# cloudflare/zkp-ecdsa

Hardware: NVIDIA H100
Metric: ZKAttest proofs/sec (higher is better)
Workload: dtype u256/u258 (32-bit limbs, Montgomery)

## Files before the change

zkp_ecdsa_b200/csrc/zk_curves.cuh:

```cuda
#pragma once
#include "zk_field.cuh"

namespace zk {

#define WEI_PT P256Pt
#define WEI_AFF P256Aff
#define WEI_JAC P256Jac
#define WEI_F P256p
#define WEI_FN(n) p256_##n
#define WEI_B_MONT ZK_P256_B_MONT
#define WEI_GX_MONT ZK_P256_GX_MONT
#define WEI_GY_MONT ZK_P256_GY_MONT
#include "zk_weier.inc"
#undef WEI_PT
#undef WEI_AFF
#undef WEI_JAC
#undef WEI_F
#undef WEI_FN
#undef WEI_B_MONT
#undef WEI_GX_MONT
#undef WEI_GY_MONT

#if defined(ZKA_PG_WAR256)
#define WEI_PT WarPt
#define WEI_AFF WarAff
#define WEI_JAC WarJac
#define WEI_F Warp
#define WEI_FN(n) war_##n
#define WEI_B_MONT ZK_WAR_B_MONT
#define WEI_GX_MONT ZK_WAR_GX_MONT
#define WEI_GY_MONT ZK_WAR_GY_MONT
#include "zk_weier.inc"
#undef WEI_PT
#undef WEI_AFF
#undef WEI_JAC
#undef WEI_F
#undef WEI_FN
#undef WEI_B_MONT
#undef WEI_GX_MONT
#undef WEI_GY_MONT

enum : int { PGL = 8 };
using PGp = Warp;
using FpPG = FpWar;
using TomPt = WarPt;
using TomPre = WarAff;
using TompMsm = Warp;
using TompCommit = Warp;
ZK_HD void tom_set_identity(TomPt& p) { war_set_identity(p); }
ZK_HD void tom_from_affine(TomPt& p, const uint32_t* x, const uint32_t* y) {
  copy_n<8>(p.x, x);
  copy_n<8>(p.y, y);
  Warp::set_one(p.z);
}
ZK_HD void tom_set_generator(TomPt& p) {
  WarAff g;
  war_set_generator(g);
  war_from_affine(p, g);
}
ZK_HD bool tom_on_curve(const uint32_t* x, const uint32_t* y) { return war_on_curve(x, y); }
ZK_HD void tom_add(TomPt& r, const TomPt& p, const TomPt& q) { war_add(r, p, q); }
template <bool kNeedT, class F = Warp>
ZK_HD void tom_madd(TomPt& r, const TomPt& p, const TomPre& q) { war_madd(r, p, q); }
ZK_HD void tom_dbl(TomPt& r, const TomPt& p) { war_dbl(r, p); }
ZK_HD void tom_neg(TomPt& r, const TomPt& p) {
  copy_n<8>(r.x, p.x);
  Warp::neg(r.y, p.y);
  copy_n<8>(r.z, p.z);
}
ZK_HD void pg_dbl_n(TomPt& p, int c) { war_dbl_n(p, c); }
ZK_HD void pg_pre_neg(TomPre& q) { Warp::neg(q.y, q.y); }
ZK_HD bool pg_is_identity(const TomPt& p) { return war_is_identity(p); }
ZK_HD void pg_fixed_to_msm(TomPt&) {}
#else
struct TomPt {
  uint32_t x[9], y[9], t[9], z[9];
};
struct TomPre {
  uint32_t x[9], y[9], k[9];
};

ZK_HD void tom_const(uint32_t* r, int which) {
  constexpr uint32_t sa[9] = ZK_TOM_SQRTA_MONT;
  constexpr uint32_t isa[9] = ZK_TOM_INVSQRTA_MONT;
  constexpr uint32_t d1[9] = ZK_TOM_D1_MONT;
  constexpr uint32_t gx[9] = ZK_TOM_GX1_MONT;
  constexpr uint32_t gy[9] = ZK_TOM_GY_MONT;
  constexpr uint32_t s2[9] = ZK_TOM_SQRTND1_MONT;
  constexpr uint32_t is2[9] = ZK_TOM_INVSQRTND1_MONT;
  constexpr uint32_t dd2[9] = ZK_TOM_2D2_MONT;
  constexpr uint32_t isd[9] = ZK_TOM_INVSQRTND_MONT;
#pragma unroll
  for (int i = 0; i < 9; i++)
    r[i] = which == 0 ? sa[i] : which == 1 ? isa[i] : which == 2 ? d1[i] : which == 3 ? gx[i] : which == 4 ? gy[i]
           : which == 5 ? s2[i] : which == 6 ? is2[i] : which == 7 ? dd2[i] : isd[i];
}
enum { TOM_SQRTA = 0, TOM_INVSQRTA = 1, TOM_D1 = 2, TOM_GX1 = 3, TOM_GY = 4, TOM_SQRTND1 = 5, TOM_INVSQRTND1 = 6,
       TOM_2D2 = 7, TOM_INVSQRTND = 8 };

struct TompInl : Tomp {
  ZK_HD static void mul(uint32_t* r, const uint32_t* a, const uint32_t* b) {
#if defined(__CUDA_ARCH__) && !defined(ZKA_NO_PTX_MUL)
    ptx::tom_mul_body(r, a, b);
#else
    Tomp::mul(r, a, b);
#endif
  }
  ZK_HD static void sqr(uint32_t* r, const uint32_t* a) { mul(r, a, a); }
};
#if defined(ZKA_COMMIT_INLINE)
using TompCommit = TompInl;
#else
using TompCommit = Tomp;
#endif
#if defined(ZKA_MSM_INLINE)
using TompMsm = TompInl;
#else
using TompMsm = Tomp;
#endif

template <bool kNeedT, class F = Tomp>
ZK_HD void tom2_madd(TomPt& r, const TomPt& p, const TomPre& q) {
  uint32_t A[9], B[9], C[9], D[9], E[9], Fv[9], G[9], H[9];
  F::sub(A, p.y, p.x);
  F::mul(A, A, q.x);
  F::add(B, p.y, p.x);
  F::mul(B, B, q.y);
  F::mul(C, p.t, q.k);
  F::add(D, p.z, p.z);
  F::sub(E, B, A);
  F::sub(Fv, D, C);
  F::add(G, D, C);
  F::add(H, B, A);
  F::mul(r.x, E, Fv);
  F::mul(r.y, G, H);
  if (kNeedT) F::mul(r.t, E, H);
  F::mul(r.z, Fv, G);
}

ZK_HD void tom_set_identity(TomPt& p) {
  zero_n<9>(p.x);
  Tomp::set_one(p.y);
  zero_n<9>(p.t);
  Tomp::set_one(p.z);
}
ZK_HD void tom_from_affine(TomPt& p, const uint32_t* x1, const uint32_t* y) {
  copy_n<9>(p.x, x1);
  copy_n<9>(p.y, y);
  Tomp::mul(p.t, x1, y);
  Tomp::set_one(p.z);
}
ZK_HD void tom_set_generator(TomPt& p) {
  uint32_t gx[9], gy[9];
  tom_const(gx, TOM_GX1);
  tom_const(gy, TOM_GY);
  tom_from_affine(p, gx, gy);
}
ZK_HD bool tom_on_curve(const uint32_t* x1, const uint32_t* y) {
  using F = Tomp;
  uint32_t xx[9], yy[9], l[9], r[9], d1[9], one[9];
  F::sqr(xx, x1);
  F::sqr(yy, y);
  F::add(l, xx, yy);
  F::mul(r, xx, yy);
  tom_const(d1, TOM_D1);
  F::mul(r, r, d1);
  F::set_one(one);
  F::add(r, r, one);
  uint32_t d[9], o[9];
  F::sub(d, l, r);
  zero_n<9>(o);
  o[0] = 1;
  F::mul(d, d, o);
  uint32_t nz = 0, np = 0;
#pragma unroll
  for (int i = 0; i < 9; i++) { nz |= d[i]; np |= d[i] ^ FpTom::p(i); }
  return nz == 0 || np == 0;
}

ZK_HD void tom_add(TomPt& r, const TomPt& p, const TomPt& q) {
  using F = Tomp;
  uint32_t A[9], B[9], C[9], D[9], E[9], Fv[9], G[9], H[9], d1[9];
  tom_const(d1, TOM_D1);
  F::mul(A, p.x, q.x);
  F::mul(B, p.y, q.y);
  F::mul(C, p.t, q.t);
  F::mul(C, C, d1);
  F::mul(D, p.z, q.z);
  F::add(E, p.x, p.y);
  F::add(H, q.x, q.y);
  F::mul(E, E, H);
  F::sub(E, E, A);
  F::sub(E, E, B);
  F::sub(Fv, D, C);
  F::add(G, D, C);
  F::sub(H, B, A);
  F::mul(r.x, E, Fv);
  F::mul(r.y, G, H);
  F::mul(r.t, E, H);
  F::mul(r.z, Fv, G);
}
template <bool kNeedT, class F = Tomp>
ZK_HD void tom_madd(TomPt& r, const TomPt& p, const TomPre& q) {
  uint32_t A[9], B[9], C[9], E[9], Fv[9], G[9], H[9];
  F::mul(A, p.x, q.x);
  F::mul(B, p.y, q.y);
  F::mul(C, p.t, q.k);
  F::add(E, p.x, p.y);
  F::add(H, q.x, q.y);
  F::mul(E, E, H);
  F::sub(E, E, A);
  F::sub(E, E, B);
  F::sub(Fv, p.z, C);
  F::add(G, p.z, C);
  F::sub(H, B, A);
  F::mul(r.x, E, Fv);
  F::mul(r.y, G, H);
  if (kNeedT) F::mul(r.t, E, H);
  F::mul(r.z, Fv, G);
}
ZK_HD void tom_dbl(TomPt& r, const TomPt& p) {
  using F = Tomp;
  uint32_t A[9], B[9], C[9], E[9], G[9], Fv[9], H[9];
  F::sqr(A, p.x);
  F::sqr(B, p.y);
  F::sqr(C, p.z);
  F::add(C, C, C);
  F::add(E, p.x, p.y);
  F::sqr(E, E);
  F::sub(E, E, A);
  F::sub(E, E, B);
  F::add(G, A, B);
  F::sub(Fv, G, C);
  F::sub(H, A, B);
  F::mul(r.x, E, Fv);
  F::mul(r.y, G, H);
  F::mul(r.t, E, H);
  F::mul(r.z, Fv, G);
}
ZK_HD void tom_neg(TomPt& r, const TomPt& p) {
  Tomp::neg(r.x, p.x);
  copy_n<9>(r.y, p.y);
  Tomp::neg(r.t, p.t);
  copy_n<9>(r.z, p.z);
}


enum : int { PGL = 9 };
using PGp = Tomp;
using FpPG = FpTom;
ZK_HD void pg_dbl_n(TomPt& p, int c) {
  for (int i = 0; i < c; i++) tom_dbl(p, p);
}
ZK_HD void pg_pre_neg(TomPre& q) {
  Tomp::neg(q.x, q.x);
  Tomp::neg(q.k, q.k);
}
ZK_HD bool pg_is_identity(const TomPt& p) { return Tomp::is_zero(p.x) && Tomp::eq(p.y, p.z); }
ZK_HD void pg_fixed_to_msm(TomPt& f) {
  uint32_t cw[9], X[9], Y[9], Tt[9], Zp[9], c1[9];
  tom_const(c1, TOM_INVSQRTND1);
  Tomp::mul(cw, f.x, c1);
  Tomp::mul(X, cw, f.y);
  Tomp::sqr(Y, f.z);
  Tomp::mul(Tt, cw, f.z);
  Tomp::mul(Zp, f.z, f.y);
  copy_n<9>(f.x, X); copy_n<9>(f.y, Y); copy_n<9>(f.t, Tt); copy_n<9>(f.z, Zp);
}
#endif

}
```

zkp_ecdsa_b200/csrc/zk_ops.cuh:

```cuda
#pragma once
#include "zk_curves.cuh"
#include "zk_layout.h"
#include "zk_sha256.cuh"

namespace zk {

#if defined(__CUDA_ARCH__)
#define ZK_SET_STATUS(ptr, code) atomicCAS((int*)(ptr), 0, (int)(code))
#define ZK_SET_STATUS_OVER(ptr, code, over) \
  do {                                      \
    atomicCAS((int*)(ptr), 0, (int)(code)); \
    atomicCAS((int*)(ptr), (int)(over), (int)(code)); \
  } while (0)
#else
#define ZK_SET_STATUS_OVER(ptr, code, over)              \
  do {                                                   \
    if (*(ptr) == 0 || *(ptr) == (over)) *(ptr) = (code); \
  } while (0)
#define ZK_SET_STATUS(ptr, code) \
  do {                           \
    if (*(ptr) == 0) *(ptr) = (code); \
  } while (0)
#endif

template <int N>
ZK_HD void ld(uint32_t* r, const uint32_t* p) {
#pragma unroll
  for (int i = 0; i < N; i++) r[i] = p[i];
}
template <int N>
ZK_HD void st(uint32_t* p, const uint32_t* r) {
#pragma unroll
  for (int i = 0; i < N; i++) p[i] = r[i];
}

enum : int {
  P256_PROJ_WORDS = 24,
  P256_AFF_WORDS = 16,
#if defined(ZKA_PG_WAR256)
  TOM_PROJ_WORDS = 24,
  TOM_AFF_WORDS = 16,
  TOM_PRE_WORDS = 16,
#else
  TOM_PROJ_WORDS = 28,
  TOM_AFF_WORDS = 18,
  TOM_PRE_WORDS = 32,
#endif
  NORM_CHUNK_MAX = 64,
};


#if defined(ZKA_PG_WAR256)
ZK_HD void tom_st_xyz(uint32_t* m, const uint32_t* x, const uint32_t* y, const uint32_t* z) {
  st<8>(m, x); st<8>(m + 8, y); st<8>(m + 16, z);
}
ZK_HD void tom_ld_xyz(uint32_t* x, uint32_t* y, uint32_t* z, const uint32_t* m) {
  ld<8>(x, m); ld<8>(y, m + 8); ld<8>(z, m + 16);
}
ZK_HD void tom_ld_pre(TomPre& q, const uint32_t* m) { ld<8>(q.x, m); ld<8>(q.y, m + 8); }
#else
ZK_HD void tom_st_xyz(uint32_t* m, const uint32_t* x, const uint32_t* y, const uint32_t* z) {
  uint32_t w[28];
#pragma unroll
  for (int i = 0; i < 9; i++) { w[i] = x[i]; w[9 + i] = y[i]; w[18 + i] = z[i]; }
  w[27] = 0;
#if defined(__CUDA_ARCH__)
  uint4* v = reinterpret_cast<uint4*>(m);
#pragma unroll
  for (int i = 0; i < 7; i++) v[i] = make_uint4(w[4 * i], w[4 * i + 1], w[4 * i + 2], w[4 * i + 3]);
#else
  for (int i = 0; i < 28; i++) m[i] = w[i];
#endif
}
ZK_HD void tom_ld_xyz(uint32_t* x, uint32_t* y, uint32_t* z, const uint32_t* m) {
  uint32_t w[28];
#if defined(__CUDA_ARCH__)
  const uint4* v = reinterpret_cast<const uint4*>(m);
#pragma unroll
  for (int i = 0; i < 7; i++) {
    const uint4 u = v[i];
    w[4 * i] = u.x; w[4 * i + 1] = u.y; w[4 * i + 2] = u.z; w[4 * i + 3] = u.w;
  }
#else
  for (int i = 0; i < 28; i++) w[i] = m[i];
#endif
#pragma unroll
  for (int i = 0; i < 9; i++) { x[i] = w[i]; y[i] = w[9 + i]; z[i] = w[18 + i]; }
}

ZK_HD void tom2_pre_neg(TomPre& q, bool neg) {
  uint32_t nk[9];
  Tomp::neg(nk, q.k);
#pragma unroll
  for (int i = 0; i < 9; i++) {
    const uint32_t a = q.x[i], b = q.y[i];
    q.x[i] = neg ? b : a;
    q.y[i] = neg ? a : b;
    q.k[i] = neg ? nk[i] : q.k[i];
  }
}
ZK_HD void tom_ld_pre(TomPre& q, const uint32_t* m) {
#if defined(__CUDA_ARCH__)
  const uint4* v = reinterpret_cast<const uint4*>(m);
  uint32_t w[32];
#pragma unroll
  for (int i = 0; i < 7; i++) {
    uint4 u = __ldg(v + i);
    w[4 * i] = u.x; w[4 * i + 1] = u.y; w[4 * i + 2] = u.z; w[4 * i + 3] = u.w;
  }
#pragma unroll
  for (int i = 0; i < 9; i++) { q.x[i] = w[i]; q.y[i] = w[9 + i]; q.k[i] = w[18 + i]; }
#else
  ld<9>(q.x, m); ld<9>(q.y, m + 9); ld<9>(q.k, m + 18);
#endif
}

#endif

ZK_HD void ld4(uint32_t* w, const void* p) {
#if defined(__CUDA_ARCH__)
  const uint4 u = *reinterpret_cast<const uint4*>(p);
  w[0] = u.x; w[1] = u.y; w[2] = u.z; w[3] = u.w;
#else
  const uint32_t* q = reinterpret_cast<const uint32_t*>(p);
  for (int i = 0; i < 4; i++) w[i] = q[i];
#endif
}
ZK_HD void st4(void* p, const uint32_t* w) {
#if defined(__CUDA_ARCH__)
  *reinterpret_cast<uint4*>(p) = make_uint4(w[0], w[1], w[2], w[3]);
#else
  uint32_t* q = reinterpret_cast<uint32_t*>(p);
  for (int i = 0; i < 4; i++) q[i] = w[i];
#endif
}
ZK_HD void ld8v(uint32_t* r, const uint32_t* p) { ld4(r, p); ld4(r + 4, p + 4); }
ZK_HD void st8v(uint32_t* p, const uint32_t* r) { st4(p, r); st4(p + 4, r + 4); }
ZK_HD bool aligned16(const void* p) { return ((size_t)p & 15) == 0; }

template <int N, int CB>
ZK_HD uint32_t enc_byte(int i, uint32_t tag, const uint32_t* x, const uint32_t* y) {
  if (i == 0) return tag;
  if (i >= 1 + 2 * CB) return 0u;
  const uint32_t* c = i <= CB ? x : y;
  const int pos = CB - 1 - (i <= CB ? i - 1 : i - 1 - CB);
  return (pos >> 2) < N ? ((c[pos >> 2] >> (8 * (pos & 3))) & 0xffu) : 0u;
}
template <int N, int CB>
ZK_HD void store_point_words(uint8_t* o, uint32_t tag, const uint32_t* x, const uint32_t* y) {
  uint32_t w[BSTRIDE / 4];
#pragma unroll
  for (int j = 0; j < BSTRIDE / 4; j++)
    w[j] = enc_byte<N, CB>(4 * j, tag, x, y) | (enc_byte<N, CB>(4 * j + 1, tag, x, y) << 8) |
           (enc_byte<N, CB>(4 * j + 2, tag, x, y) << 16) | (enc_byte<N, CB>(4 * j + 3, tag, x, y) << 24);
  if (aligned16(o)) {
#pragma unroll
    for (int j = 0; j < BSTRIDE / 16; j++) st4(o + 16 * j, w + 4 * j);
  } else {
    uint32_t* ow = reinterpret_cast<uint32_t*>(o);
#pragma unroll
    for (int j = 0; j < BSTRIDE / 4; j++) ow[j] = w[j];
  }
}

ZK_HD uint32_t digit4(const uint32_t* k, int j) { return (k[j >> 3] >> (4 * (j & 7))) & 15u; }
ZK_HD uint32_t digit8(const uint32_t* k, int j) { return (k[j >> 2] >> (8 * (j & 3))) & 255u; }
ZK_HD uint32_t digit_w(const uint32_t* k, int pos, int w) {
  int wi = pos >> 5, sh = pos & 31;
  uint64_t v = k[wi];
  if (wi + 1 < 8) v |= (uint64_t)k[wi + 1] << 32;
  return (uint32_t)(v >> sh) & ((1u << w) - 1u);
}

ZK_HD int fb_entries(int w) { return (1 << (w - 1)) + 1; }
ZK_HD int fb_windows(int w) { return (256 + w) / w; }
ZK_HD uint32_t signed_digit(const uint32_t* k, int j, int w, uint32_t& carry, bool& neg) {
  const int pos = j * w;
  uint32_t d = carry;
  if (pos < 256) d += digit_w(k, pos, (256 - pos) < w ? (256 - pos) : w);
  const uint32_t half = 1u << (w - 1);
  neg = d > half;
  carry = neg ? 1u : 0u;
  return neg ? (1u << w) - d : d;
}

ZK_HD uint32_t bswap32(uint32_t x) {
#if defined(__CUDA_ARCH__)
  return __byte_perm(x, 0u, 0x0123);
#else
  return (x >> 24) | ((x >> 8) & 0xff00u) | ((x << 8) & 0xff0000u) | (x << 24);
#endif
}
ZK_HD void tape_draw(uint32_t* r, const uint8_t* tape, int draw) {
  const uint8_t* p = tape + 32 * (size_t)draw;
#if defined(__CUDA_ARCH__)
  if (aligned16(p)) {
    const uint4 a = __ldg(reinterpret_cast<const uint4*>(p)), b = __ldg(reinterpret_cast<const uint4*>(p) + 1);
    r[7] = bswap32(a.x); r[6] = bswap32(a.y); r[5] = bswap32(a.z); r[4] = bswap32(a.w);
    r[3] = bswap32(b.x); r[2] = bswap32(b.y); r[1] = bswap32(b.z); r[0] = bswap32(b.w);
    return;
  }
#endif
#pragma unroll
  for (int i = 0; i < 8; i++) {
    const uint8_t* q = p + 28 - 4 * i;
    r[i] = ((uint32_t)q[0] << 24) | ((uint32_t)q[1] << 16) | ((uint32_t)q[2] << 8) | (uint32_t)q[3];
  }
}

#define WEI_PT P256Pt
#define WEI_AFF P256Aff
#define WEI_JAC P256Jac
#define WEI_F P256p
#define WEI_FN(n) p256_##n
#define WEI_T(n) P256##n
#include "zk_weier_ops.inc"
#undef WEI_PT
#undef WEI_AFF
#undef WEI_JAC
#undef WEI_F
#undef WEI_FN
#undef WEI_T

enum : int { KEY_W_MIN = 5, KEY_W_MAX = 8, KEY_CAP = 52 * 17 };
ZK_HD int key_window_bits(uint32_t count, uint32_t B, uint32_t uses) {
  int best = KEY_W_MIN;
  uint64_t best_cost = ~0ull;
  for (int w = KEY_W_MIN; w <= KEY_W_MAX; w++) {
    const uint64_t nwin = (uint64_t)fb_windows(w), ne = (uint64_t)fb_entries(w);
    if (w > KEY_W_MIN && (uint64_t)count * nwin * ne > (uint64_t)B * KEY_CAP) break;
    const uint64_t cost = nwin * ((uint64_t)count * (ne - 1) * 2 + (uint64_t)B * uses);
    if (cost < best_cost) { best_cost = cost; best = w; }
  }
  return best;
}
ZK_HD size_t key_table_words(int w) { return (size_t)fb_windows(w) * fb_entries(w) * P256_AFF_WORDS; }

enum : int { RT_W = 5, RT_NWIN = 52, RT_ROW = 16, RT_ENTRIES = RT_NWIN * RT_ROW };
struct P256RowsSignedTask {
  const uint32_t* pows;
// ... 35 lines not shown
ZK_HD int item_gpart_of_job(int j) {
  if (j < 6) return j;
  if (j < 30) {
    const int m = (j - 6) / 6, u = (j - 6) % 6;
    return 6 + 5 * m + (u < 4 ? u : u - 1);
  }
  return 26 + ((j - 30) >> 1);
}
ZK_HD int item_job_of_gpart(int g) {
  if (g < 6) return g;
  if (g < 26) {
    const int m = (g - 6) / 5, u = (g - 6) % 5;
    return 6 + 6 * m + (u < 4 ? u : 5);
  }
  return 30 + 2 * (g - 26);
}
#if defined(ZKA_PG_WAR256)
#include "zk_ops_war.cuh"
#else
struct TomPowsTask {
  const uint32_t* base_aff;
  uint32_t* pows;
  int nbase, nwin, w;
  ZK_HD void operator()(int t) const {
    uint32_t x[9], y[9];
    ld<9>(x, base_aff + (size_t)t * TOM_AFF_WORDS);
    ld<9>(y, base_aff + (size_t)t * TOM_AFF_WORDS + 9);
    TomPt p;
    tom_from_affine(p, x, y);
    for (int j = 0; j < nwin; j++) {
      uint32_t* o = pows + ((size_t)t * nwin + j) * 36;
      st<9>(o, p.x); st<9>(o + 9, p.y); st<9>(o + 18, p.t); st<9>(o + 27, p.z);
      for (int k = 0; k < w; k++) tom_dbl(p, p);
    }
  }
};
struct TomRowsTask {
  const uint32_t* pows;
  uint32_t* rows;
  int w;
  ZK_HD void operator()(int t) const {
    TomPt p, acc;
    const uint32_t* s = pows + (size_t)t * 36;
    ld<9>(p.x, s); ld<9>(p.y, s + 9); ld<9>(p.t, s + 18); ld<9>(p.z, s + 27);
    tom_set_identity(acc);
    const int ne = fb_entries(w);
    uint32_t* out = rows + (size_t)t * ne * TOM_PROJ_WORDS;
    for (int d = 0; d < ne; d++) {
      uint32_t* o = out + (size_t)d * TOM_PROJ_WORDS;
      tom_st_xyz(o, acc.x, acc.y, acc.z);
      tom_add(acc, acc, p);
    }
  }
};
struct TomRowsHiTask {
  const uint32_t* pows;
  uint32_t* hi;
  uint32_t* rows;
  int w;
  ZK_HD void operator()(int t) const {
    TomPt p, acc;
    const uint32_t* s = pows + (size_t)t * 36;
    ld<9>(p.x, s); ld<9>(p.y, s + 9); ld<9>(p.t, s + 18); ld<9>(p.z, s + 27);
    for (int k = 0; k < 8; k++) tom_dbl(p, p);
    tom_set_identity(acc);
    const int nh = 1 << (w - 9);
    for (int m = 0; m < nh; m++) {
      uint32_t* o = hi + ((size_t)t * nh + m) * 36;
      st<9>(o, acc.x); st<9>(o + 9, acc.y); st<9>(o + 18, acc.t); st<9>(o + 27, acc.z);
      tom_add(acc, acc, p);
    }
    tom_st_xyz(rows + ((size_t)t * fb_entries(w) + ((size_t)1 << (w - 1))) * TOM_PROJ_WORDS, acc.x, acc.y, acc.z);
  }
};
struct TomRowsLoTask {
  const uint32_t* pows;
  const uint32_t* hi;
  uint32_t* rows;
  int w;
  ZK_HD void operator()(int t) const {
    const int nh = 1 << (w - 9);
    const int j = t / nh, m = t % nh;
    TomPt p, acc;
    const uint32_t* s = pows + (size_t)j * 36;
    ld<9>(p.x, s); ld<9>(p.y, s + 9); ld<9>(p.t, s + 18); ld<9>(p.z, s + 27);
    const uint32_t* h = hi + (size_t)t * 36;
    ld<9>(acc.x, h); ld<9>(acc.y, h + 9); ld<9>(acc.t, h + 18); ld<9>(acc.z, h + 27);
    uint32_t* out = rows + ((size_t)j * fb_entries(w) + ((size_t)m << 8)) * TOM_PROJ_WORDS;
    for (int d = 0; d < 256; d++) {
      uint32_t* o = out + (size_t)d * TOM_PROJ_WORDS;
      tom_st_xyz(o, acc.x, acc.y, acc.z);
      tom_add(acc, acc, p);
    }
  }
};
struct TomTabE2Task {
  const uint32_t* proj;
  uint32_t* pre;
  int count;
  ZK_HD void operator()(int t) const {
    using F = Tomp;
    constexpr int CH = 16;
    const int lo = t * CH;
    int n = count - lo;
    if (n > CH) n = CH;
    if (n <= 0) return;
    uint32_t pf[CH][9];
    uint32_t acc[9], y[9], z[9], den[9];
    F::set_one(acc);
    for (int k = 0; k < n; k++) {
      const uint32_t* src = proj + (size_t)(lo + k) * TOM_PROJ_WORDS;
      uint32_t xx[9];
      tom_ld_xyz(xx, y, z, src);
      F::mul(den, y, z);
      F::mul(acc, acc, den);
      copy_n<9>(pf[k], acc);
    }
    uint32_t inv[9], s2[9], dd2[9];
    F::inv(inv, acc);
    tom_const(s2, TOM_SQRTND1);
    tom_const(dd2, TOM_2D2);
    for (int k = n - 1; k >= 0; k--) {
      const uint32_t* src = proj + (size_t)(lo + k) * TOM_PROJ_WORDS;
      uint32_t x[9], di[9], w[9], v[9], kk[9], ym[9], yp[9];
      tom_ld_xyz(x, y, z, src);
      F::mul(den, y, z);
      if (k > 0) F::mul(di, inv, pf[k - 1]); else copy_n<9>(di, inv);
      F::mul(inv, inv, den);
      F::mul(w, x, y);
      F::mul(w, w, di);
      F::mul(w, w, s2);
      F::sqr(v, z);
      F::mul(v, v, di);
      F::mul(kk, w, v);
      F::mul(kk, kk, dd2);
      F::sub(ym, v, w);
      F::add(yp, v, w);
      F::reduce(ym); F::reduce(yp); F::reduce(kk);
      uint32_t* o = pre + (size_t)(lo + k) * TOM_PRE_WORDS;
      st<9>(o, ym); st<9>(o + 9, yp); st<9>(o + 18, kk);
      for (int i = 27; i < 32; i++) o[i] = 0;
    }
  }
};

struct TomNormTask {
  const uint32_t* proj;
  uint32_t* aff;
  uint8_t* bytes;
  int count;
  int chunk;
  int e2;
  int aff_mod, aff_lim;
  ZK_HD static void canon2p(uint32_t* r) {
    uint32_t t[9], p2[9];
#pragma unroll
    for (int i = 0; i < 9; i++) p2[i] = (FpTom::p(i) << 1) | (i > 0 ? (FpTom::p(i - 1) >> 31) : 0u);
    uint32_t br = sub_n<9>(t, r, p2);
    csel_n<9>(r, br == 0, t, r);
    br = sub_p<FpTom>(t, r);
    csel_n<9>(r, br == 0, t, r);
  }
  ZK_HD void operator()(int t) const {
    using F = Tomp;
    const int lo = t * chunk;
    int n = count - lo;
    if (n > chunk) n = chunk;
    if (n <= 0) return;
    uint32_t pre[NORM_CHUNK_MAX][9];
    uint32_t acc[9], z[9], v[9], den[9];
    F::set_one(acc);
    for (int k = 0; k < n; k++) {
      const uint32_t* src = proj + (size_t)(lo + k) * TOM_PROJ_WORDS;
      uint32_t xx[9];
      tom_ld_xyz(xx, v, z, src);
      if (e2) F::mul(den, z, v); else copy_n<9>(den, z);
      F::mul(acc, acc, den);
      copy_n<9>(pre[k], acc);
    }
    uint32_t inv[9], isa[9], is2[9], isd[9], one_plain[9];
    F::inv(inv, acc);
    tom_const(isa, TOM_INVSQRTA);
    tom_const(is2, TOM_INVSQRTND1);
    tom_const(isd, TOM_INVSQRTND);
    zero_n<9>(one_plain);
    one_plain[0] = 1;
    for (int k = n - 1; k >= 0; k--) {
      const uint32_t* src = proj + (size_t)(lo + k) * TOM_PROJ_WORDS;
      uint32_t X[9], Y[9], di[9];
      tom_ld_xyz(X, Y, z, src);
      if (e2) F::mul(den, z, Y); else copy_n<9>(den, z);
      if (k > 0) F::mul(di, inv, pre[k - 1]); else copy_n<9>(di, inv);
      F::mul(inv, inv, den);
      if (bytes) {
        uint32_t Dp[9], cx[9], cy[9];
        F::mul(Dp, di, one_plain);
        if (e2) {
          F::mul(cx, X, Y);
          F::mul(cx, cx, isd);
          F::mul(cx, cx, Dp);
          F::sqr(cy, z);
          F::mul(cy, cy, Dp);
        } else {
          F::mul(cx, X, isa);
          F::mul(cx, cx, Dp);
          F::mul(cy, Y, Dp);
        }
        canon2p(cx);
        canon2p(cy);
        store_point_words<9, 33>(bytes + (size_t)(lo + k) * BSTRIDE, 0x04u, cx, cy);
      }
      if (aff && ((lo + k) % aff_mod) < aff_lim) {
        uint32_t x[9], y[9];
        if (e2) {
          uint32_t zi[9], vi[9];
          F::mul(zi, di, Y);
          F::mul(vi, di, z);
          F::mul(x, X, zi);
          F::mul(x, x, is2);
          F::mul(y, z, vi);
        } else {
          F::mul(x, X, di);
          F::mul(y, Y, di);
        }
        uint32_t* a = aff + (size_t)(lo + k) * TOM_AFF_WORDS;
        st<9>(a, x);
        st<9>(a + 9, y);
      }
    }
  }
};

struct TomCommitTask {
  const uint32_t* jv;
  const uint32_t* jr;
  const uint32_t* gtab;
  const uint32_t* htab;
  uint32_t* proj;
  int w, nwin;
  ZK_HD void operator()(int t) const {
    uint32_t v[8], r[8];
    ld<8>(v, jv + (size_t)t * 8);
    ld<8>(r, jr + (size_t)t * 8);
    TomPt acc;
    tom_set_identity(acc);
    const size_t ne = (size_t)fb_entries(w);
    uint32_t cv = 0, cr = 0;
    for (int j = 0; j < nwin; j++) {
      TomPre q;
      bool nv, nr;
      const uint32_t dv = signed_digit(v, j, w, cv, nv), dr = signed_digit(r, j, w, cr, nr);
      tom_ld_pre(q, gtab + ((size_t)j * ne + dv) * TOM_PRE_WORDS);
      tom2_pre_neg(q, nv);
      tom2_madd<true>(acc, acc, q);
      tom_ld_pre(q, htab + ((size_t)j * ne + dr) * TOM_PRE_WORDS);
      tom2_pre_neg(q, nr);
      tom2_madd<true>(acc, acc, q);
    }
    uint32_t* o = proj + (size_t)t * TOM_PROJ_WORDS;
    tom_st_xyz(o, acc.x, acc.y, acc.z);
  }
};

struct TomCommitGTask {
  const uint32_t* jv;
  const uint32_t* gtab;
  uint32_t* ext;
  int w, nwin;
  ZK_HD void operator()(int t) const {
    const int item = t / GJOBS_PER_ITEM, g = t % GJOBS_PER_ITEM;
    uint32_t v[8];
    ld<8>(v, jv + ((size_t)item * JOBS_PER_ITEM + item_job_of_gpart(g)) * 8);
    TomPt acc;
    tom_set_identity(acc);
    const size_t ne = (size_t)fb_entries(w);
    uint32_t carry = 0;
#pragma unroll 1
    for (int j = 0; j < nwin; j++) {
      TomPre q;
      bool neg;
      const uint32_t d = signed_digit(v, j, w, carry, neg);
      tom_ld_pre(q, gtab + ((size_t)j * ne + d) * TOM_PRE_WORDS);
      tom2_pre_neg(q, neg);
      tom2_madd<true, TompCommit>(acc, acc, q);
    }
    uint32_t* o = ext + (size_t)t * TOM_EXT_WORDS;
    st<9>(o, acc.x); st<9>(o + 9, acc.y); st<9>(o + 18, acc.t); st<9>(o + 27, acc.z);
  }
};
struct TomCommitHTask {
  const uint32_t* jr;
  const uint32_t* htab;
  const uint32_t* ext;
  uint32_t* proj;
  int w, nwin;
  ZK_HD void operator()(int t) const {
    const int item = t / JOBS_PER_ITEM, jb = t % JOBS_PER_ITEM;
    uint32_t r[8];
    ld<8>(r, jr + (size_t)t * 8);
    TomPt acc;
    const uint32_t* s = ext + ((size_t)item * GJOBS_PER_ITEM + item_gpart_of_job(jb)) * TOM_EXT_WORDS;
    ld<9>(acc.x, s); ld<9>(acc.y, s + 9); ld<9>(acc.t, s + 18); ld<9>(acc.z, s + 27);
    const size_t ne = (size_t)fb_entries(w);
    uint32_t carry = 0;
#pragma unroll 1
    for (int j = 0; j < nwin; j++) {
      TomPre q;
      bool neg;
      const uint32_t d = signed_digit(r, j, w, carry, neg);
      tom_ld_pre(q, htab + ((size_t)j * ne + d) * TOM_PRE_WORDS);
      tom2_pre_neg(q, neg);
      tom2_madd<true, TompCommit>(acc, acc, q);
    }
    tom_st_xyz(proj + (size_t)t * TOM_PROJ_WORDS, acc.x, acc.y, acc.z);
  }
};

#if !defined(ZKA_HOSTSIM) && defined(ZKA_COMMIT_MINBLOCKS)
template <> struct TaskMinBlocks<TomCommitHTask> { static constexpr int value = ZKA_COMMIT_MINBLOCKS; };
template <> struct TaskMinBlocks<TomCommitGTask> { static constexpr int value = ZKA_COMMIT_MINBLOCKS; };
template <> struct TaskMinBlocks<TomCommitTask> { static constexpr int value = ZKA_COMMIT_MINBLOCKS; };
#endif

#endif

enum : int { GK_BLOCK_BITS = 10 };
ZK_HD int gk_block_bits(int n) { return n < GK_BLOCK_BITS ? n : GK_BLOCK_BITS; }
ZK_HD void gk_block_sum(uint32_t* acc, const uint32_t* ring_m, const uint32_t (*fz)[8], const uint32_t (*fo)[8], int n,
                        int k, uint32_t blk, const uint32_t* vw) {
  using F = Tomq;
  uint32_t P[21][8];
  F::set_one(P[n]);
  for (int j = n - 1; j >= k; j--) F::mul(P[j], P[j + 1], ((blk >> (j - k)) & 1u) ? fo[j] : fz[j]);
  for (int j = k - 1; j >= 0; j--) F::mul(P[j], P[j + 1], fz[j]);
  zero_n<8>(acc);
  const size_t base = (size_t)blk << k;
  const uint32_t cnt = 1u << k;
  for (uint32_t l = 0;;) {
    uint32_t vi[8], term[8];
    ld<8>(vi, ring_m + (base + l) * 8);
    if (vw) F::sub(vi, vw, vi);
    F::mul(term, vi, P[0]);
    F::add(acc, acc, term);
    l++;
    if (l == cnt) break;
    int tz = 0;
    while (!((l >> tz) & 1u)) tz++;
    F::mul(P[tz], P[tz + 1], fo[tz]);
    for (int j = tz - 1; j >= 0; j--) F::mul(P[j], P[j + 1], fz[j]);
  }
}

ZK_HD bool hash_pt_fetch(uint32_t* t, const uint8_t* p, int len) {
  if (((size_t)p & 3) || len < 64 || len > 68) return false;
  if (aligned16(p)) {
#pragma unroll
    for (int j = 0; j < 4; j++) ld4(t + 4 * j, p + 16 * j);
    t[16] = len > 64 ? *reinterpret_cast<const uint32_t*>(p + 64) : 0u;
    return true;
  }
  const uint32_t* q = reinterpret_cast<const uint32_t*>(p);
#pragma unroll
  for (int j = 0; j < 17; j++) t[j] = (4 * j < len) ? q[j] : 0u;
  return true;
}
template <class Src>
ZK_HD void hash_points80(uint32_t* c3, const Src& src, int npts) {
  Sha256 h;
  h.init();
  uint32_t nx[17], cu[17];
  int nlen = 0;
  const uint8_t* np = npts > 0 ? src(0, nlen) : nullptr;
  bool nfast = npts > 0 && hash_pt_fetch(nx, np, nlen);
  for (int i = 0; i < npts; i++) {
    const uint8_t* p = np;
    const int len = nlen;
    const bool fast = nfast;
#pragma unroll
    for (int j = 0; j < 17; j++) cu[j] = nx[j];
    if (i + 1 < npts) {
      np = src(i + 1, nlen);
      nfast = hash_pt_fetch(nx, np, nlen);
    }
    if (fast) h.feed17(cu, len);
    else h.update(p, len);
  }
  h.final80(c3);
}

ZK_HD void challenge_to_limbs(uint32_t* r, const uint32_t* c3) {
  zero_n<8>(r);
  r[0] = c3[0]; r[1] = c3[1]; r[2] = c3[2];
}

template <int N>
ZK_HD void load_point(uint32_t* w, const uint8_t* src) {
  if (aligned16(src)) {
#pragma unroll
    for (int j = 0; j < BSTRIDE / 16; j++) ld4(w + 4 * j, src + 16 * j);
  } else if (((size_t)src & 3) == 0) {
    const uint32_t* sw = reinterpret_cast<const uint32_t*>(src);
#pragma unroll
    for (int j = 0; j < BSTRIDE / 4; j++) w[j] = 4 * j < N ? sw[j] : 0u;
  } else {
#pragma unroll
    for (int j = 0; j < BSTRIDE / 4; j++) {
      uint32_t v = 0;
#pragma unroll
      for (int t = 0; t < 4; t++)
        if (4 * j + t < N) v |= (uint32_t)src[4 * j + t] << (8 * t);
      w[j] = v;
    }
  }
}

struct ByteWriter {
  uint8_t* blk;
  uint32_t q[4];
  int fill;
  int lead;
  ZK_HD explicit ByteWriter(uint8_t* dst) : blk(dst - ((size_t)dst & 15)), fill((int)((size_t)dst & 15)), lead(fill) {
    q[0] = q[1] = q[2] = q[3] = 0;
  }
  ZK_HD static uint32_t funnel(uint32_t lo, uint32_t hi, int sh) {
#if defined(__CUDA_ARCH__)
    return __funnelshift_l(lo, hi, sh);
#else
    return (uint32_t)((((uint64_t)hi << 32) | lo) >> (32 - sh));
#endif
  }
  ZK_HD void store_part(int lo, int hi) const {
#pragma unroll
    for (int w = 0; w < 4; w++) {
      if (lo <= 4 * w && 4 * w + 4 <= hi) {
        *reinterpret_cast<uint32_t*>(blk + 4 * w) = q[w];
      } else {
#pragma unroll
        for (int t = 0; t < 4; t++)
          if (lo <= 4 * w + t && 4 * w + t < hi) blk[4 * w + t] = (uint8_t)(q[w] >> (8 * t));
      }
    }
  }
  ZK_HD void chunk(const uint32_t* c, int nb) {
    uint32_t m[4];
#pragma unroll
    for (int i = 0; i < 4; i++) {
      const int k = nb - 4 * i;
      m[i] = k >= 4 ? c[i] : k <= 0 ? 0u : c[i] & ((1u << (8 * k)) - 1u);
    }
    const int sh = 8 * (fill & 3), ws = fill >> 2;
    uint32_t d[5];
    d[0] = sh ? m[0] << sh : m[0];
#pragma unroll
    for (int i = 1; i < 4; i++) d[i] = funnel(m[i - 1], m[i], sh);
    d[4] = sh ? m[3] >> (32 - sh) : 0u;
    uint32_t e[8];
#pragma unroll
    for (int k = 0; k < 8; k++) {
      uint32_t v = 0;
#pragma unroll
      for (int s = 0; s < 4; s++)
        if (k - s >= 0 && k - s <= 4) v = ws == s ? d[k - s] : v;
      e[k] = v;
    }
#pragma unroll
    for (int k = 0; k < 4; k++) q[k] |= e[k];
    fill += nb;
// ... 52 lines not shown
```

zkp_ecdsa_b200/csrc/zk_ops_war.cuh:

```cuda
#pragma once

#define WEI_PT WarPt
#define WEI_AFF WarAff
#define WEI_JAC WarJac
#define WEI_F Warp
#define WEI_FN(n) war_##n
#define WEI_T(n) War##n
#include "zk_weier_ops.inc"
#undef WEI_PT
#undef WEI_AFF
#undef WEI_JAC
#undef WEI_F
#undef WEI_FN
#undef WEI_T

struct TomNormTask {
  const uint32_t* proj;
  uint32_t* aff;
  uint8_t* bytes;
  int count;
  int chunk;
  int e2;
  int aff_mod, aff_lim;
  ZK_HD void operator()(int t) const {
    using F = Warp;
    const int lo = t * chunk;
    int n = count - lo;
    if (n > chunk) n = chunk;
    if (n <= 0) return;
    uint32_t pre[NORM_CHUNK_MAX][8];
    uint32_t acc[8], z[8], one[8];
    F::set_one(one);
    copy_n<8>(acc, one);
    for (int k = 0; k < n; k++) {
      ld<8>(z, proj + (size_t)(lo + k) * TOM_PROJ_WORDS + 16);
      if (is_zero_n<8>(z)) copy_n<8>(z, one);
      F::mul(acc, acc, z);
      copy_n<8>(pre[k], acc);
    }
    uint32_t inv[8];
    F::inv(inv, acc);
    for (int k = n - 1; k >= 0; k--) {
      const uint32_t* src = proj + (size_t)(lo + k) * TOM_PROJ_WORDS;
      ld<8>(z, src + 16);
      const bool isinf = is_zero_n<8>(z);
      if (isinf) copy_n<8>(z, one);
      uint32_t zi[8];
      if (k > 0) F::mul(zi, inv, pre[k - 1]); else copy_n<8>(zi, inv);
      F::mul(inv, inv, z);
      uint32_t X[8], Y[8], x[8], y[8];
      ld<8>(X, src);
      ld<8>(Y, src + 8);
      F::mul(x, X, zi);
      F::mul(y, Y, zi);
      if (aff && ((lo + k) % aff_mod) < aff_lim) {
        uint32_t* a = aff + (size_t)(lo + k) * TOM_AFF_WORDS;
        st<8>(a, x);
        st<8>(a + 8, y);
      }
      if (bytes) {
        uint32_t cx[8], cy[8];
        F::from_mont(cx, x);
        F::from_mont(cy, y);
        if (isinf) { zero_n<8>(cx); zero_n<8>(cy); }
        store_point_words<8, 32>(bytes + (size_t)(lo + k) * BSTRIDE, isinf ? 0x00u : 0x04u, cx, cy);
      }
    }
  }
};

struct TomCommitTask {
  const uint32_t* jv;
  const uint32_t* jr;
  const uint32_t* gtab;
  const uint32_t* htab;
  uint32_t* proj;
  int w, nwin;
  ZK_HD void operator()(int t) const {
    uint32_t v[8], r[8];
    ld<8>(v, jv + (size_t)t * 8);
    ld<8>(r, jr + (size_t)t * 8);
    WarPt acc;
    war_set_identity(acc);
    war_accum_fixed(acc, gtab, v, w);
    war_accum_fixed(acc, htab, r, w);
    war_st_proj(proj + (size_t)t * TOM_PROJ_WORDS, acc);
  }
};
struct TomCommitGTask {
  const uint32_t* jv;
  const uint32_t* gtab;
  uint32_t* ext;
  int w, nwin;
  ZK_HD void operator()(int t) const {
    const int item = t / GJOBS_PER_ITEM, g = t % GJOBS_PER_ITEM;
    uint32_t v[8];
    ld<8>(v, jv + ((size_t)item * JOBS_PER_ITEM + item_job_of_gpart(g)) * 8);
    WarPt acc;
    war_set_identity(acc);
    war_accum_fixed(acc, gtab, v, w);
    war_st_proj(ext + (size_t)t * TOM_EXT_WORDS, acc);
  }
};
struct TomCommitHTask {
  const uint32_t* jr;
  const uint32_t* htab;
  const uint32_t* ext;
  uint32_t* proj;
  int w, nwin;
  ZK_HD void operator()(int t) const {
    const int item = t / JOBS_PER_ITEM, jb = t % JOBS_PER_ITEM;
    uint32_t r[8];
    ld<8>(r, jr + (size_t)t * 8);
    WarPt acc;
    war_ld_proj(acc, ext + ((size_t)item * GJOBS_PER_ITEM + item_gpart_of_job(jb)) * TOM_EXT_WORDS);
    war_accum_fixed(acc, htab, r, w);
    war_st_proj(proj + (size_t)t * TOM_PROJ_WORDS, acc);
  }
};
```

zkp_ecdsa_b200/csrc/zk_prove.cuh:

```cuda
#pragma once
#include "zk_sigma.cuh"

namespace zk {

struct ProveCtx {
  int B;
  int S;
  int N;
  int n;
  int M;
  int tom_w, tom_nwin;
  int mode;
  int head_len;
  const uint8_t* base;
  const uint8_t* s_in;
  const uint8_t* q_in;
  uint32_t* base_aff;
  const uint8_t* msg_hash;
  const uint8_t* sig;
  const uint8_t* pk;
  const uint32_t* which;
  uint32_t* which_s;
  const uint8_t* tape;
  size_t tape_stride;
// ... 447 lines not shown
    if (n > ITEM_INV_CHUNK) n = ITEM_INV_CHUNK;
    uint32_t d[ITEM_INV_CHUNK][8], pre[ITEM_INV_CHUNK][8], acc[8];
    bool z[ITEM_INV_CHUNK];
    F::set_one(acc);
#pragma unroll
    for (int k = 0; k < ITEM_INV_CHUNK; k++) {
      if (k < n) {
        const int it = lo + k;
        uint32_t x1[8], x2[8], one[8];
        ld<8>(x1, c.pb_T1_aff + (size_t)it * 16);
        ld<8>(x2, c.pk_aff + (size_t)c.item_b[it] * 16);
        F::sub(d[k], x2, x1);
        z[k] = is_zero_n<8>(d[k]);
        F::set_one(one);
        csel_n<8>(d[k], z[k], one, d[k]);
        F::mul(acc, acc, d[k]);
        copy_n<8>(pre[k], acc);
      }
    }
    uint32_t inv[8];
    F::inv(inv, acc);
#pragma unroll
    for (int k = ITEM_INV_CHUNK - 1; k >= 0; k--) {
      if (k < n) {
        uint32_t r[8], zero[8];
        if (k > 0) F::mul(r, inv, pre[k - 1]); else copy_n<8>(r, inv);
        F::mul(inv, inv, d[k]);
        zero_n<8>(zero);
        csel_n<8>(r, z[k], zero, r);
        st<8>(c.item_inv + (size_t)(lo + k) * 8, r);
      }
    }
  }
};

struct ItemScalarsTask {
  ProveCtx c;
  ZK_HD void job(size_t item, int j, const uint32_t* v_mont, const uint32_t* r_canon) const {
    uint32_t v[8];
    Tomq::from_mont(v, v_mont);
    st8v(c.s2_jv + c.s2_job(item, j) * 8, v);
    st8v(c.s2_jr + c.s2_job(item, j) * 8, r_canon);
  }
  ZK_HD void job_raw(size_t item, int j, const uint32_t* v, const uint32_t* r) const {
    st8v(c.s2_jv + c.s2_job(item, j) * 8, v);
    st8v(c.s2_jr + c.s2_job(item, j) * 8, r);
  }
  ZK_HD void operator()(int it) const {
    using F = Tomq;
    const int b = c.item_b[it], i = c.item_i[it], k = c.item_k[it];
    if (c.pb_T1_inf[it]) ZK_SET_STATUS(c.status + b, ZKA_ERR_T1_INFINITY);
    const int d0 = draws_before_items(c.S) + DRAWS_PER_ITEM * k;
    uint32_t x1[8], y1[8], x2[8], y2[8], x3[8];
    ld8v(x1, c.pb_T1_aff + (size_t)it * 16);
    ld8v(y1, c.pb_T1_aff + (size_t)it * 16 + 8);
    ld8v(x2, c.pk_aff + (size_t)b * 16);
    ld8v(y2, c.pk_aff + (size_t)b * 16 + 8);
    ld8v(x3, c.pa_T_aff + ((size_t)b * (c.S + 1) + i) * 16);
    uint32_t rT1x[8], rT1y[8], rPkx[8], rPky[8], rTx[8], rTy[8];
    draw_checked<FpP256>(rT1x, c, b, d0 + IT_T1X_R);
    draw_checked<FpP256>(rT1y, c, b, d0 + IT_T1Y_R);
    draw_checked<FpP256>(rPkx, c, b, DRAW_PKX_R);
    draw_checked<FpP256>(rPky, c, b, DRAW_PKY_R);
    draw_checked<FpP256>(rTx, c, b, DRAW_REP0 + DRAWS_PER_REP * i + 2);
    draw_checked<FpP256>(rTy, c, b, DRAW_REP0 + DRAWS_PER_REP * i + 3);
    uint32_t mT1x[8], mT1y[8], mPkx[8], mPky[8], mTx[8], mTy[8];
    F::to_mont(mT1x, rT1x); F::to_mont(mT1y, rT1y);
    F::to_mont(mPkx, rPkx); F::to_mont(mPky, rPky);
    F::to_mont(mTx, rTx);   F::to_mont(mTy, rTy);
    uint32_t i7[8], i8[8], i9[8], i10[8], i11[8], i12[8], i13[8];
    F::sub(i7, x2, x1);
    ld8v(i8, c.item_inv + (size_t)it * 8);
    F::sub(i9, y2, y1);
    F::mul(i10, i8, i9);
    F::sqr(i11, i10);
    F::sub(i12, x1, x3);
    F::mul(i13, i10, i12);
    uint32_t r7[8], r9[8], r12[8], rcx[8], rcy[8];
    F::sub(r7, mPkx, mT1x);
    F::sub(r9, mPky, mT1y);
    F::sub(r12, mT1x, mTx);
    F::add(rcx, mTx, mT1x); F::add(rcx, rcx, mPkx);
    F::add(rcy, mTy, mT1y);
    uint32_t r8[8], r10[8], r11[8], r13[8], m8[8], m10[8], m11[8], m13[8];
    draw_checked<FpP256>(r8, c, b, d0 + IT_C8_R);
    draw_checked<FpP256>(r10, c, b, d0 + IT_C10_R);
    draw_checked<FpP256>(r11, c, b, d0 + IT_C11_R);
    draw_checked<FpP256>(r13, c, b, d0 + IT_C13_R);
    F::to_mont(m8, r8); F::to_mont(m10, r10); F::to_mont(m11, r11); F::to_mont(m13, r13);
    job(it, JOB_T1X, x1, rT1x);
    job(it, JOB_T1Y, y1, rT1y);
    job(it, JOB_C8, i8, r8);
    job(it, JOB_C10, i10, r10);
    job(it, JOB_C11, i11, r11);
    job(it, JOB_C13, i13, r13);
    uint32_t one[8], zero[8];
    F::set_one(one);
    zero_n<8>(zero);
    uint32_t* sec = c.secrets + (size_t)it * SECRETS_PER_ITEM * 8;
    for (int m = 0; m < 4; m++) {
      const uint32_t *x, *y, *z, *rx, *ry, *rz;
      if (m == 0)      { x = i7;  y = i8;  z = one; rx = r7;  ry = m8;  rz = zero; }
      else if (m == 1) { x = i8;  y = i9;  z = i10; rx = m8;  ry = r9;  rz = m10; }
      else if (m == 2) { x = i10; y = i10; z = i11; rx = m10; ry = m10; rz = m11; }
      else             { x = i10; y = i12; z = i13; rx = m10; ry = r12; rz = m13; }
      const int dm = d0 + item_mult_draw(m);
      uint32_t kx[8], ky[8], kz[8], ra[8], mkx[8], t[8], u[8], r4[8];
      draw_checked<FpP256>(kx, c, b, dm + 0);
      draw_checked<FpP256>(ky, c, b, dm + 1);
      draw_checked<FpP256>(kz, c, b, dm + 2);
      F::to_mont(mkx, kx);
      const int j0 = JOB_MULT0 + 6 * m;
      F::mul(t, x, y);
      F::mul(r4, x, ry);
      F::from_mont(u, r4);
      job(it, j0 + 0, t, u);
      draw_checked<FpP256>(ra, c, b, dm + 3);
      job_raw(it, j0 + 1, kx, ra);
      draw_checked<FpP256>(ra, c, b, dm + 4);
      job_raw(it, j0 + 2, ky, ra);
      draw_checked<FpP256>(ra, c, b, dm + 5);
      job_raw(it, j0 + 3, kz, ra);
      draw_checked<FpP256>(ra, c, b, dm + 6);
      job_raw(it, j0 + 4, kz, ra);
      F::mul(t, mkx, y);
      F::mul(u, mkx, ry);
      F::from_mont(u, u);
      job(it, j0 + 5, t, u);
      uint32_t* sm = sec + (size_t)m * 7 * 8;
      st8v(sm, x); st8v(sm + 8, y); st8v(sm + 16, z);
      st8v(sm + 24, rx); st8v(sm + 32, ry); st8v(sm + 40, rz); st8v(sm + 48, r4);
    }
    for (int e = 0; e < 2; e++) {
      const int de = d0 + (e == 0 ? IT_EQ0 : IT_EQ1);
      uint32_t kk[8], ra[8];
      draw_checked<FpP256>(kk, c, b, de + 0);
      draw_checked<FpP256>(ra, c, b, de + 1);
      job_raw(it, JOB_EQ0 + 2 * e, kk, ra);
      draw_checked<FpP256>(ra, c, b, de + 2);
      job_raw(it, JOB_EQ0 + 2 * e + 1, kk, ra);
      uint32_t* se = sec + (size_t)(28 + 3 * e) * 8;
      st8v(se, e == 0 ? i11 : i13);
      st8v(se + 8, e == 0 ? m11 : m13);
      st8v(se + 16, e == 0 ? rcx : rcy);
    }
  }
};

struct DerivedTask {
  ProveCtx c;
  struct Store {
    const ProveCtx& c;
    int it;
    ZK_HD void operator()(int d, const TomPt& p) const { tom_st_xyz(c.s2_proj + c.s2_der(it, d) * TOM_PROJ_WORDS, p.x, p.y, p.z); }
  };
  ZK_HD void ldaff(TomPt& p, const uint32_t* aff, size_t idx) const {
    uint32_t x[PGL], y[PGL];
    ld<PGL>(x, aff + idx * TOM_AFF_WORDS);
    ld<PGL>(y, aff + idx * TOM_AFF_WORDS + PGL);
    tom_from_affine(p, x, y);
  }
  ZK_HD void operator()(int it) const {
    const int b = c.item_b[it], i = c.item_i[it];
    TomPt pkX, pkY, Tx, Ty, T1x, T1y;
    ldaff(pkX, c.s1_aff, c.s1_pt(b, 0));
    ldaff(pkY, c.s1_aff, c.s1_pt(b, 1));
    ldaff(Tx, c.s1_aff, c.s1_pt(b, 2 + 2 * i));
    ldaff(Ty, c.s1_aff, c.s1_pt(b, 3 + 2 * i));
    ldaff(T1x, c.s2_aff, c.s2_job(it, JOB_T1X));
    ldaff(T1y, c.s2_aff, c.s2_job(it, JOB_T1Y));
    point_add_derived(Store{c, it}, T1x, pkX, Tx, T1y, pkY, Ty);
  }
};

struct ItemHashTask {
  ProveCtx c;
  struct Src {
    const ProveCtx* c;
    size_t it;
    int h;
    ZK_HD const uint8_t* pt(size_t idx) const { return c->s2_bytes + idx * BSTRIDE; }
    ZK_HD const uint8_t* operator()(int k, int& len) const {
      len = WP;
      const ProveCtx& C = *c;
      const int ns = h < PA_MULTS ? 3 : 2;
      if (k < ns) {
        const int com = h < PA_MULTS ? pa_mult_com(h, k) : pa_eq_com(h - PA_MULTS, k);
        return pa_com_bytes(com, pt(C.s2_der(it, 0)), C.tg_bytes, pt(C.s2_job(it, JOB_C8)), BSTRIDE);
      }
      return pt(C.s2_job(it, (h < PA_MULTS ? JOB_MULT0 + 6 * h : JOB_EQ0 + 2 * (h - PA_MULTS)) + (k - ns)));
    }
  };
  ZK_HD void operator()(int t) const {
    const size_t it = (size_t)t / HASHES_PER_ITEM;
    const int h = t % HASHES_PER_ITEM;
    uint32_t c3[3];
    Src src{&c, it, h};
    hash_points80(c3, src, h < 4 ? 9 : 4);
    st<3>(c.item_chal + (size_t)t * 3, c3);
  }
};

ZK_HD void response(uint32_t* t, const uint32_t* k_canon, const uint32_t* cc, const uint32_t* w_mont) {
  using F = Tomq;
  uint32_t cw[8];
  F::mul(cw, cc, w_mont);
  F::sub(t, k_canon, cw);
}

struct ItemEmitTask {
  ProveCtx c;
  ZK_HD void operator()(int t) const {
    const size_t it = (size_t)t / 7;
    const int part = t % 7;
    const int b = c.item_b[it], i = c.item_i[it], k = c.item_k[it];
    uint8_t* rep = c.proofs + (size_t)b * c.proof_stride + c.rep_off[(size_t)b * c.S + i];
    uint8_t* body = rep + REP_HEAD;
    uint8_t* pa = body + 2 * NS;
    const int d0 = draws_before_items(c.S) + DRAWS_PER_ITEM * k;
    const uint32_t* sec = c.secrets + it * SECRETS_PER_ITEM * 8;
    if (part < 4) {
      const int m = part;
      ByteWriter o(pa + 4 * WP + m * MULT_LEN);
#pragma unroll
      for (int p = 0; p < 6; p++) o.put_point<WP>(c.s2_bytes + c.s2_job(it, JOB_MULT0 + 6 * m + p) * BSTRIDE);
      uint32_t cc[8], c3[3], kk[8], w[8], r[8];
      ld<3>(c3, c.item_chal + (it * HASHES_PER_ITEM + m) * 3);
      challenge_to_limbs(cc, c3);
      const int dm = d0 + item_mult_draw(m);
      const uint32_t* sm = sec + (size_t)m * 7 * 8;
#pragma unroll
      for (int q = 0; q < 7; q++) {
        tape_draw(kk, c.tape_of(b), dm + q);
        reduce_once<FpP256>(kk);
        ld8v(w, sm + q * 8);
        response(r, kk, cc, w);
        o.put_scalar<WS>(r);
      }
      o.finish();
    } else if (part < 6) {
      const int e = part - 4;
      ByteWriter o(pa + 4 * WP + 4 * MULT_LEN + e * EQ_LEN);
      o.put_point<WP>(c.s2_bytes + c.s2_job(it, JOB_EQ0 + 2 * e) * BSTRIDE);
      o.put_point<WP>(c.s2_bytes + c.s2_job(it, JOB_EQ0 + 2 * e + 1) * BSTRIDE);
      uint32_t cc[8], c3[3], kk[8], w[8], r[8];
      ld<3>(c3, c.item_chal + (it * HASHES_PER_ITEM + 4 + e) * 3);
      challenge_to_limbs(cc, c3);
      const int de = d0 + (e == 0 ? IT_EQ0 : IT_EQ1);
      const uint32_t* se = sec + (size_t)(28 + 3 * e) * 8;
#pragma unroll
      for (int q = 0; q < 3; q++) {
        tape_draw(kk, c.tape_of(b), de + q);
        reduce_once<FpP256>(kk);
        ld8v(w, se + q * 8);
        response(r, kk, cc, w);
        o.put_scalar<WS>(r);
      }
      o.finish();
    } else {
      using Fn = P256n;
      uint32_t alpha[8], s1[8], ri[8], r0[8], z[8];
      tape_draw(alpha, c.tape_of(b), DRAW_REP0 + DRAWS_PER_REP * i); reduce_once<FnP256>(alpha);
      tape_draw(ri, c.tape_of(b), DRAW_REP0 + DRAWS_PER_REP * i + 1); reduce_once<FnP256>(ri);
      tape_draw(r0, c.tape_of(b), DRAW_COMS1_R); reduce_once<FnP256>(r0);
      ld<8>(s1, c.s1 + (size_t)b * 8);
      ByteWriter o(body);
      Fn::sub(z, alpha, s1);
      o.put_scalar<NS>(z);
      Fn::sub(z, ri, r0);
      o.put_scalar<NS>(z);
      o.put_point<WP>(c.s2_bytes + c.s2_job(it, JOB_C8) * BSTRIDE);
      o.put_point<WP>(c.s2_bytes + c.s2_job(it, JOB_C10) * BSTRIDE);
      o.put_point<WP>(c.s2_bytes + c.s2_job(it, JOB_C11) * BSTRIDE);
      o.put_point<WP>(c.s2_bytes + c.s2_job(it, JOB_C13) * BSTRIDE);
      o.finish();
      ByteWriter ot(pa + PA_LEN);
      uint32_t r[8];
      tape_draw(r, c.tape_of(b), d0 + IT_T1X_R); reduce_once<FpP256>(r);
      ot.put_scalar<WS>(r);
      tape_draw(r, c.tape_of(b), d0 + IT_T1Y_R); reduce_once<FpP256>(r);
      ot.put_scalar<WS>(r);
      ot.finish();
    }
  }
};

struct RepEmitTask {
  ProveCtx c;
  ZK_HD void operator()(int t) const {
    const int S1 = c.S + 1;
    const int b = t / S1, i = t % S1;
    uint8_t* proof = c.proofs + (size_t)b * c.proof_stride;
    if (i == c.S) {
      if (c.mode == 1) return;
      ByteWriter o(proof);
      o.put_point<NP>(c.r_bytes + (size_t)b * BSTRIDE);
      o.put_point<NP>(c.pa_A_bytes + ((size_t)b * S1 + c.S) * BSTRIDE);
      o.put_point<WP>(c.s1_bytes + c.s1_pt(b, 0) * BSTRIDE);
      o.put_point<WP>(c.s1_bytes + c.s1_pt(b, 1) * BSTRIDE);
      o.finish();
      if (c.pa_A_inf[(size_t)b * S1 + c.S]) ZK_SET_STATUS(c.status + b, ZKA_ERR_IDENTITY_ENC);
      return;
    }
    uint8_t* rep = proof + c.rep_off[(size_t)b * c.S + i];
    const uint32_t bit = (c.chal[(size_t)b * 3 + (i >> 5)] >> (i & 31)) & 1u;
    ByteWriter o(rep);
    o.put_byte(bit);
// ... 507 lines not shown
```

zkp_ecdsa_b200/csrc/zkattest.cu:

```cuda
#include "zkattest.h"

#include <math.h>
#include <stdio.h>

#include <algorithm>
#include <atomic>
#include <cmath>
#include <mutex>
#include <chrono>
#include <memory>
#include <thread>
#include <string>
#include <vector>

#include "zk_launch.cuh"
#include "zk_prove.cuh"
#include "zk_seed.cuh"
#include "zk_verify_agg.cuh"

namespace zk {
struct ParsePointsTask {
  const uint8_t* nist;
  const uint8_t* tom;
  uint32_t* nist_aff;
// ... 239 lines not shown
struct FixedTable {
  DevBuf buf;
  uint32_t* tab = nullptr;
};

}

struct Lane {
  Stream st;
  Stream cs_in, cs_out;
  Event ev_small[2], ev_tape[2], ev_done[2], ev_out[2];
  Stream aux[2];
  Event ev_fork, ev_join[2];
  DevBuf w[51];
  DevBuf in[2][10], out[2][3];
  DevBuf agg[8], agg_tom[5 + 2 * AGG_MAX_LEVELS], agg_nist[5 + 2 * AGG_MAX_LEVELS];
  std::string err;
  ~Lane() {
    for (int i = 0; i < 2; i++) {
      ev_destroy(ev_small[i]); ev_destroy(ev_tape[i]); ev_destroy(ev_done[i]); ev_destroy(ev_out[i]);
    }
    ev_destroy(ev_fork); ev_destroy(ev_join[0]); ev_destroy(ev_join[1]);
    stream_destroy(cs_in);
    stream_destroy(cs_out);
    stream_destroy(aux[0]);
    stream_destroy(aux[1]);
    stream_destroy(st);
  }
};

struct zka_ctx : Lane {
  int device = 0;
  std::vector<std::unique_ptr<Lane>> extra;
  int nlanes = 3;
  DevBuf ring_in, ring_m;
  Lane& lane(int i) { return i == 0 ? *this : *extra[i - 1]; }
  int tom_w = 22, tom_nwin = 12;
  int chunk = 4096;
  int host_chunk = 2048;
  volatile uint32_t* progress = nullptr;
  uint32_t progress_cap = 0;
  int agg = 1;
  int agg_c = 0;
  uint64_t agg_pass = 0, agg_fail = 0;
  std::mutex stat_mu;
  std::mutex copy_mu;
  int agg_c_last = 0;
  bool tape_split = true;
  int p256_hw = 20;
  FixedTable g8;
  FixedTable gw;
  FixedTable tg;
  DevBuf tg_bytes;
  DevBuf lag;
  int lag_n = -1;
};

struct zka_params {
  zka_ctx* ctx = nullptr;
  uint32_t sec_level = 80;
  FixedTable h8;
  int h_w = 20;
  FixedTable th;
  uint8_t h_nist[65];
  uint8_t h_proof[WP];
};

struct zka_rings {
  zka_ctx* ctx = nullptr;
  uint32_t R = 0;
  std::vector<uint32_t> size;
  std::vector<int> depth;
  DevBuf ring_m, ring_base, ring_size;
};

namespace {

int fail(zka_ctx* ctx, int code, const std::string& msg) {
  if (ctx) ctx->err = msg;
  return code;
}
template <class Fn>
int guarded(zka_ctx* ctx, Fn&& body) {
  try {
    return body();
  } catch (const std::exception& e) {
    return fail(ctx, ZKA_E_CUDA, e.what());
  }
}

template <class Src>
void agg_msm(Stream& st, Cursor A, const Src& src, const AggPlan& pl, const uint32_t* ctl, const uint32_t** rootA,
             const uint32_t** rootB) {
  const AggDigits& D = pl.D;
  const int nwin = D.nwin, nb = D.nb, nseg = (nb + 1 + AGG_SEG - 1) / AGG_SEG;
  const size_t cap = (size_t)src.slots();
  uint32_t* hist = A.take<uint32_t>((size_t)nwin * (nb + 1));
  uint32_t* bstart = A.take<uint32_t>((size_t)nwin * (nb + 2));
  uint32_t* segtot = A.take<uint32_t>((size_t)nwin * nseg);
  uint32_t* sorted = A.take<uint32_t>((size_t)nwin * cap);
  uint32_t* bsum = A.take<uint32_t>((size_t)nwin * nb * Src::PTW);
  dev_memset(st, hist, 0, (size_t)nwin * (nb + 1) * 4);
  launch(st, (long long)cap, AggHistTask<Src>{src, D, ctl, hist});
  launch(st, (long long)nwin * nseg, AggSegSumTask{ctl, hist, segtot, nb, nseg});
  launch(st, nwin, AggSegScanTask{ctl, segtot, nseg});
  launch(st, (long long)nwin * nseg, AggOffsetsTask{ctl, segtot, hist, bstart, nb, nseg});
  launch(st, (long long)cap, AggScatterTask<Src>{src, D, ctl, hist, sorted, cap});
  launch(st, (long long)nwin * nb, AggBucketTask<Src>{src, ctl, bstart, sorted, bsum, cap, nb});
  const uint32_t *inA = bsum, *inB = nullptr;
  int nin = nb, ll = 0;
  for (int lv = 0; lv < pl.levels; lv++) {
    const int nout = nin >> pl.lm[lv];
    uint32_t* oA = A.take<uint32_t>((size_t)nwin * nout * Src::PTW);
    uint32_t* oB = A.take<uint32_t>((size_t)nwin * nout * Src::PTW);
    launch(st, (long long)nwin * nout, AggLevelTask<Src>{ctl, inA, inB, oA, oB, nin, pl.lm[lv], ll, nwin, D.top_shift});
    inA = oA; inB = oB; nin = nout; ll += pl.lm[lv];
  }
  *rootA = inA;
  *rootB = inB;
}

int ceil_log2(uint32_t v) {
  int n = 0;
  while ((1ull << n) < v) n++;
  return n;
}


static int g_norm_slots = 132 * 4;
static bool g_norm_model = true;
inline int norm_chunk_for(long long count, int per_point = 11) {
  if (!g_norm_model) {
    long long c = count / 100000;
    if (c < 8) c = 8;
    if (c > NORM_CHUNK_MAX) c = NORM_CHUNK_MAX;
    return (int)c;
  }
  int best = 8;
  long long best_cost = -1;
  for (int c = 8; c <= NORM_CHUNK_MAX; c++) {
    const long long threads = (count + c - 1) / c, ctas = (threads + 127) / 128;
    const long long waves = (ctas + g_norm_slots - 1) / g_norm_slots;
    const long long cost = waves * ((long long)per_point * c + 70);
    if (best_cost < 0 || cost < best_cost) { best_cost = cost; best = c; }
  }
  return best;
}
inline void launch_p256_norm(Stream& st, const uint32_t* proj, uint32_t* aff, uint8_t* bytes, uint8_t* inf, long long count) {
  if (count <= 0) return;
  const int ch = norm_chunk_for(count, bytes ? 7 : 5);
  launch(st, (count + ch - 1) / ch, P256NormTask{proj, aff, bytes, inf, (int)count, ch});
}
inline void launch_tom_norm(Stream& st, const uint32_t* proj, uint32_t* aff, uint8_t* bytes, long long count, int e2,
                            int aff_mod = 1, int aff_lim = 1) {
  if (count <= 0) return;
  const int ch = norm_chunk_for(count);
  launch(st, (count + ch - 1) / ch, TomNormTask{proj, aff, bytes, (int)count, ch, e2, aff_mod, aff_lim});
}

void build_p256_tab(zka_ctx* ctx, const uint32_t* base_aff_dev, FixedTable& out, int w) {
  Stream& st = ctx->st;
  const int nwin = fb_windows(w);
  const size_t E = (size_t)fb_entries(w), count = (size_t)nwin * E;
  DevBuf pows, rows;
  uint32_t* d_pows = pows.get<uint32_t>((size_t)nwin * P256_PROJ_WORDS);
  uint32_t* d_rows = rows.get<uint32_t>(count * P256_PROJ_WORDS);
  out.tab = out.buf.get<uint32_t>(count * P256_AFF_WORDS);
  launch(st, 1, P256PowsTask{base_aff_dev, nullptr, d_pows, 1, nwin, w});
  if (w > 9) {
    DevBuf hi;
    const int nh = 1 << (w - 9);
    uint32_t* d_hi = hi.get<uint32_t>((size_t)nwin * nh * P256_PROJ_WORDS);
    launch(st, nwin, P256RowsHiTask{d_pows, d_hi, d_rows, w});
    launch(st, (long long)nwin * nh, P256RowsLoTask{d_pows, d_hi, d_rows, w});
    sync(st);
  } else {
    launch(st, nwin, P256RowsTask{d_pows, d_rows, w});
  }
  launch_p256_norm(st, d_rows, out.tab, nullptr, nullptr, (long long)(count));
  sync(st);
}
#if defined(ZKA_PG_WAR256)
void build_tom_tab(zka_ctx* ctx, const uint32_t* base_aff_dev, FixedTable& out) {
  Stream& st = ctx->st;
  const int w = ctx->tom_w, nwin = fb_windows(w);
  const size_t E = (size_t)fb_entries(w), count = (size_t)nwin * E;
  DevBuf pows, rows;
  uint32_t* d_pows = pows.get<uint32_t>((size_t)nwin * P256_PROJ_WORDS);
  uint32_t* d_rows = rows.get<uint32_t>(count * P256_PROJ_WORDS);
  out.tab = out.buf.get<uint32_t>(count * TOM_PRE_WORDS);
  launch(st, 1, WarPowsTask{base_aff_dev, nullptr, d_pows, 1, nwin, w});
  if (w > 9) {
    DevBuf hi;
    const int nh = 1 << (w - 9);
    uint32_t* d_hi = hi.get<uint32_t>((size_t)nwin * nh * P256_PROJ_WORDS);
    launch(st, nwin, WarRowsHiTask{d_pows, d_hi, d_rows, w});
    launch(st, (long long)nwin * nh, WarRowsLoTask{d_pows, d_hi, d_rows, w});
    sync(st);
  } else {
    launch(st, nwin, WarRowsTask{d_pows, d_rows, w});
  }
  {
    const int ch = norm_chunk_for((long long)count, 5);
    launch(st, ((long long)count + ch - 1) / ch, WarNormTask{d_rows, out.tab, nullptr, nullptr, (int)count, ch});
  }
  sync(st);
}
#else
void build_tom_tab(zka_ctx* ctx, const uint32_t* base_aff_dev, FixedTable& out) {
  Stream& st = ctx->st;
  const int w = ctx->tom_w, nwin = ctx->tom_nwin;
  const size_t ne = (size_t)fb_entries(w), count = (size_t)nwin * ne;
  DevBuf pows, rows;
  uint32_t* d_pows = pows.get<uint32_t>((size_t)nwin * 36);
  uint32_t* d_rows = rows.get<uint32_t>(count * TOM_PROJ_WORDS);
  out.tab = out.buf.get<uint32_t>(count * TOM_PRE_WORDS);
  launch(st, 1, TomPowsTask{base_aff_dev, d_pows, 1, nwin, w});
  if (w > 9) {
    DevBuf hi;
    const int nh = 1 << (w - 9);
    uint32_t* d_hi = hi.get<uint32_t>((size_t)nwin * nh * 36);
    launch(st, nwin, TomRowsHiTask{d_pows, d_hi, d_rows, w});
    launch(st, (long long)nwin * nh, TomRowsLoTask{d_pows, d_hi, d_rows, w});
    sync(st);
  } else {
    launch(st, nwin, TomRowsTask{d_pows, d_rows, w});
  }
  launch(st, (long long)(count + 15) / 16, TomTabE2Task{d_rows, out.tab, (int)count});
  sync(st);
}

#endif

template <class T>
const T* stage_in(Stream& st, DevBuf& buf, const T* p, size_t count) {
  if (!p || count == 0) return p;
  if (is_device_ptr(p)) return p;
  T* d = buf.get<T>(count);
  copy_h2d(st, d, p, count * sizeof(T));
  return d;
}

template <class T>
struct Output {
  T* dst;
  size_t width;
  bool dev;
  Output(T* p, size_t width) : dst(p), width(width), dev(is_device_ptr(p)) {}
  T* rows(DevBuf& stage, uint32_t b0, size_t rows) const { return dev ? dst + b0 * width : stage.get<T>(rows * width); }
  void copy_back(Stream& st, uint32_t b0, const T* d, size_t rows) const {
    if (!dev) copy_d2h(st, dst + b0 * width, d, rows * width * sizeof(T));
  }
  void copy_back_2d(Stream& st, uint32_t b0, const T* d, size_t rows, size_t bytes) const {
    if (!dev) copy_d2h_2d(st, dst + b0 * width, width * sizeof(T), d, width * sizeof(T), bytes, rows);
  }
};

std::vector<uint32_t> chunk_schedule(uint32_t B, uint32_t cmax, int lanes, bool taper) {
  std::vector<uint32_t> off{0};
  auto r32 = [](uint32_t v) { return v < 32 ? std::max<uint32_t>(v, 1) : ((v + 31) & ~31u); };
  if (lanes > 1) {
    uint32_t per = r32((B + (uint32_t)lanes - 1) / (uint32_t)lanes);
    cmax = std::min(cmax, std::max<uint32_t>(per, 256));
  }
  uint32_t done = 0;
  auto push = [&](uint32_t n) { n = std::min(n, B - done); if (n) { done += n; off.push_back(done); } };
  if (taper && cmax >= 1024 && B >= 3 * cmax) {
    const uint32_t q = r32(cmax / 4), h = r32(cmax / 2);
    push(q);
    push(h);
    const uint32_t mid = B - done - (h + q);
    const uint32_t nm = (mid + cmax - 1) / cmax;
    const uint32_t each = r32((mid + nm - 1) / nm);
    for (uint32_t i = 0; i + 1 < nm; i++) push(each);
    push(B - done - (h + q));
    push(h);
    push(q);
  } else {
    const uint32_t nk = (B + cmax - 1) / cmax;
    const uint32_t each = r32((B + nk - 1) / nk);
    while (done < B) push(each);
  }
  return off;
}

#if !defined(ZKA_HOSTSIM)
void CUDART_CB progress_cb(void* p) { *reinterpret_cast<volatile uint32_t*>(p) = 1u; }
void notify_progress(Stream& st, volatile uint32_t* flag) { ZK_CUDA_CHECK(cudaLaunchHostFunc(st.s, progress_cb, (void*)flag)); }
#else
void notify_progress(Stream&, volatile uint32_t* flag) { *flag = 1u; }
#endif

template <class Fn>
void run_lanes(zka_ctx* ctx, int used, Fn fn) {
  if (used <= 1) { fn(0); return; }
  std::vector<std::thread> th;
  std::vector<std::exception_ptr> errs((size_t)used);
  for (int li = 1; li < used; li++)
    th.emplace_back([&, li] {
      try {
#if !defined(ZKA_HOSTSIM)
        ZK_CUDA_CHECK(cudaSetDevice(ctx->device));
#endif
        fn(li);
      } catch (...) {
        errs[(size_t)li] = std::current_exception();
      }
    });
  try { fn(0); } catch (...) { errs[0] = std::current_exception(); }
  for (auto& t : th) t.join();
  for (auto& e : errs)
    if (e) std::rethrow_exception(e);
}

void prep_lagrange(zka_ctx* ctx, Stream& st, int n) {
  if (ctx->lag_n != n) {
    launch(st, 1, GkLagrangeTask{ctx->lag.get<uint32_t>((size_t)n * n * 8), n});
    ctx->lag_n = n;
  }
}
const uint32_t* prep_ring(zka_ctx* ctx, Stream& st, const uint8_t* ring, uint32_t N, int n, bool lagrange) {
  const uint8_t* d_ring = stage_in(st, ctx->ring_in, ring, (size_t)N * 32);
  uint32_t* ring_m = ctx->ring_m.get<uint32_t>(((size_t)1 << n) * 8);
  launch(st, 1ll << n, RingPrepTask{d_ring, ring_m, (int)N});
  if (lagrange) prep_lagrange(ctx, st, n);
  return ring_m;
}

struct RingPass {
  const zka_rings* set;
  const uint32_t* ring_of;
  int n;
};
struct RingRuns {
  std::vector<uint32_t> start;
  std::vector<int> depth;
  int nmax = 0;
};
int ring_runs(zka_ctx* ctx, const zka_rings* set, const uint32_t* ring_of, uint32_t B, RingRuns& rr) {
  std::vector<uint32_t> h(B);
  if (is_device_ptr(ring_of)) {
    copy_d2h(ctx->st, h.data(), ring_of, (size_t)B * 4);
    sync(ctx->st);
  } else {
    memcpy(h.data(), ring_of, (size_t)B * 4);
  }
  for (uint32_t b = 0; b < B; b++)
    if (h[b] >= set->R) return fail(ctx, ZKA_E_ARG, "ring_of[i] >= number of rings in the set");
  for (uint32_t b = 0; b < B; b++) {
    const int n = set->depth[h[b]];
    if (b == 0 || n != rr.depth.back()) { rr.start.push_back(b); rr.depth.push_back(n); }
    rr.nmax = std::max(rr.nmax, n);
  }
  rr.start.push_back(B);
  return 0;
}

int gk_blocks(int n) { return 1 << (n - gk_block_bits(n)); }

ProveCtx prove_ctx(const zka_ctx* ctx, const zka_params* P, int B, int S, int N, int n) {
  ProveCtx c;
  memset(&c, 0, sizeof(c));
  c.B = B; c.S = S; c.N = N; c.n = n;
  c.tom_w = ctx->tom_w; c.tom_nwin = ctx->tom_nwin;
  c.g_tab8 = ctx->g8.tab; c.h_tab8 = P->h8.tab; c.h_w = P->h_w;
  c.g_tabw = ctx->gw.tab; c.g_w = ctx->p256_hw;
  c.tg_tab = ctx->tg.tab; c.th_tab = P->th.tab;
  c.tg_bytes = (const uint8_t*)ctx->tg_bytes.p;
  c.gk_lag = (uint32_t*)ctx->lag.p;
  return c;
}
VerifyCtx verify_ctx(const zka_ctx* ctx, const zka_params* P, int B, int S, int N, int n, int K, int mode) {
  VerifyCtx c;
  memset(&c, 0, sizeof(c));
  c.B = B; c.S = S; c.N = N; c.n = n; c.K = K; c.mode = mode;
  c.tom_w = ctx->tom_w; c.tom_nwin = ctx->tom_nwin;
  c.g_tab8 = ctx->g8.tab; c.h_tab8 = P->h8.tab; c.h_w = P->h_w;
  c.tg_tab = ctx->tg.tab; c.th_tab = P->th.tab;
  c.tg_bytes = (const uint8_t*)ctx->tg_bytes.p;
  return c;
}

void prove_store1(Stream& st, const ProveCtx& c) {
  const long long n1 = (long long)c.B * (2 + 2 * c.S);
  launch(st, n1, JobsATask{c});
  launch(st, n1, TomCommitTask{c.s1_jv, c.s1_jr, c.tg_tab, c.th_tab, c.s1_proj, c.tom_w, c.tom_nwin});
  launch_tom_norm(st, c.s1_proj, c.s1_aff, c.s1_bytes, n1, 1);
}
void prove_items_gk(Stream& st, const ProveCtx& c, uint32_t* gext, bool items, bool gk) {
  const long long M = c.M, nj = M * JOBS_PER_ITEM, nd = M * DERS_PER_ITEM;
  const long long Bn = (long long)c.B * c.n, ng = 4 * Bn;
  const int nblk = gk_blocks(c.n);
  const size_t g0 = c.s2_gk(0, 0);
  if (items) {
    launch(st, (M + ITEM_INV_CHUNK - 1) / ITEM_INV_CHUNK, ItemInvTask{c});
    launch(st, M, ItemScalarsTask{c});
  }
  if (gk) {
    launch(st, Bn, GkJobsTask{c});
    launch(st, Bn * nblk, GkPolyTask{c});
    if (nblk > 1) launch(st, Bn, GkPolyReduceTask{c});
    launch(st, Bn, GkCdJobsTask{c});
  }
  if (items) {
    launch(st, M * GJOBS_PER_ITEM, TomCommitGTask{c.s2_jv, c.tg_tab, gext, c.tom_w, c.tom_nwin});
    launch(st, nj, TomCommitHTask{c.s2_jr, c.th_tab, gext, c.s2_proj, c.tom_w, c.tom_nwin});
  }
  if (gk)
    launch(st, ng, TomCommitTask{c.s2_jv + g0 * 8, c.s2_jr + g0 * 8, c.tg_tab, c.th_tab, c.s2_proj + g0 * TOM_PROJ_WORDS, c.tom_w,
                                 c.tom_nwin});
  if (items) {
    launch_tom_norm(st, c.s2_proj, c.s2_aff, c.s2_bytes, nj, 1, JOBS_PER_ITEM, 2);
    launch(st, M, DerivedTask{c});
    launch_tom_norm(st, c.s2_proj + nj * TOM_PROJ_WORDS, nullptr, c.s2_bytes + nj * BSTRIDE, nd, 0);
  }
  if (gk) launch_tom_norm(st, c.s2_proj + g0 * TOM_PROJ_WORDS, nullptr, c.s2_bytes + g0 * BSTRIDE, ng, 1);
  if (items) {
    launch(st, M * HASHES_PER_ITEM, ItemHashTask{c});
    launch(st, M * 7, ItemEmitTask{c});
  }
}
void verify_gk(Stream& st, const VerifyCtx& c, uint32_t* gk_offs) {
  const int nblk = gk_blocks(c.n), ngk = 4 * c.n + 1;
  if (nblk > 1) launch(st, (long long)c.B * nblk, VGkSumTask{c});
  launch(st, c.B, VGkTask{c});
  launch(st, (long long)c.B * ngk, VGkOffsetsTask{c, gk_offs});
}

}

extern "C" {

int zka_version(void) { return 1; }

const char* zka_last_error(const zka_ctx* ctx) { return ctx ? ctx->err.c_str() : "null context"; }

uint64_t zka_launch_count(const zka_ctx* ctx) {
  if (!ctx) return 0;
  uint64_t n = ctx->st.launches + ctx->aux[0].launches + ctx->aux[1].launches;
  for (const auto& l : ctx->extra) n += l->st.launches + l->aux[0].launches + l->aux[1].launches;
  return n;
}

void* zka_get_stream(zka_ctx* ctx) {
#if !defined(ZKA_HOSTSIM)
  return ctx ? (void*)ctx->st.s : nullptr;
#else
  return nullptr;
#endif
}
int zka_set_profiling(zka_ctx* ctx, int enable) {
  if (!ctx) return ZKA_E_ARG;
  try {
    for (int i = 0; i < 1 + (int)ctx->extra.size(); i++) { sync(ctx->lane(i).st); ctx->lane(i).st.profiling = enable != 0; }
  } catch (...) { return ZKA_E_CUDA; }
  return 0;
}
int zka_profile_reset(zka_ctx* ctx) {
  if (!ctx) return ZKA_E_ARG;
  try {
    for (int i = 0; i < 1 + (int)ctx->extra.size(); i++) { sync(ctx->lane(i).st); ctx->lane(i).st.prof.clear(); }
  } catch (...) { return ZKA_E_CUDA; }
  return 0;
}
int zka_set_option(zka_ctx* ctx, const char* key, long value) {
  if (!ctx || !key || value < 1) return ZKA_E_ARG;
  const std::string k(key);
  return guarded(ctx, [&]() -> int {
    if (k == "lanes") {
      if (value > 8) return ZKA_E_ARG;
      while ((int)ctx->extra.size() + 1 < value) {
        auto l = std::make_unique<Lane>();
        stream_create(l->st);
        stream_create(l->cs_in);
        stream_create(l->cs_out);
        stream_create(l->aux[0]);
        stream_create(l->aux[1]);
        l->st.profiling = ctx->st.profiling;
        ctx->extra.push_back(std::move(l));
      }
      ctx->nlanes = (int)value;
    } else if (k == "chunk") {
      ctx->chunk = (int)value;
    } else if (k == "host_chunk") {
      ctx->host_chunk = (int)value;
    } else if (k == "agg") {
      ctx->agg = (int)value - 1;
    } else if (k == "agg_c") {
      if (value < 4 || value > 16) return ZKA_E_ARG;
      ctx->agg_c = (int)value;
    } else {
      return ZKA_E_ARG;
    }
    return 0;
  });
}
long long zka_stat(zka_ctx* ctx, const char* key) {
  if (!ctx || !key) return -1;
  const std::string k(key);
  std::lock_guard<std::mutex> g(ctx->stat_mu);
  if (k == "agg_pass") return (long long)ctx->agg_pass;
  if (k == "agg_fail") return (long long)ctx->agg_fail;
  if (k == "agg_c") return (long long)ctx->agg_c_last;
  return -1;
}
size_t zka_profile_json(zka_ctx* ctx, char* buf, size_t cap) {
  if (!ctx) return 0;
  std::map<std::string, ProfEntry> all;
  try {
    for (int i = 0; i < 1 + (int)ctx->extra.size(); i++) {
      sync(ctx->lane(i).st);
      for (auto& kv : ctx->lane(i).st.prof) {
        ProfEntry& e = all[kv.first];
        e.launches += kv.second.launches; e.ms += kv.second.ms; e.items += kv.second.items;
      }
    }
  } catch (...) { return 0; }
  std::string j = "{";
  bool first = true;
  for (auto& kv : all) {
    char tmp[512];
    snprintf(tmp, sizeof tmp, "%s\"%s\": {\"launches\": %llu, \"ms\": %.6f, \"items\": %llu}", first ? "" : ", ",
             kv.first.c_str(), (unsigned long long)kv.second.launches, kv.second.ms,
             (unsigned long long)kv.second.items);
    j += tmp;
    first = false;
  }
  j += "}";
  if (buf && cap) {
    size_t n = std::min(cap - 1, j.size());
    memcpy(buf, j.data(), n);
    buf[n] = 0;
  }
  return j.size() + 1;
}
int zka_proof_group(char* name, size_t cap, int* point_bytes, int* scalar_bytes) {
#if defined(ZKA_PG_WAR256)
  const char* n = "war256";
#else
  const char* n = "tomEdwards256";
#endif
  if (name && cap) {
    strncpy(name, n, cap - 1);
    name[cap - 1] = 0;
  }
  if (point_bytes) *point_bytes = WP;
  if (scalar_bytes) *scalar_bytes = WS;
  return 0;
}
int zka_set_progress(zka_ctx* ctx, volatile uint32_t* flags, uint32_t cap) {
  if (!ctx) return ZKA_E_ARG;
  ctx->progress = flags;
  ctx->progress_cap = flags ? cap : 0;
  return 0;
}
int zka_chunk_schedule(zka_ctx* ctx, uint32_t B, int host_buffers, uint32_t* off, uint32_t cap) {
  if (!ctx || !off || cap == 0) return ZKA_E_ARG;
  const std::vector<uint32_t> v = chunk_schedule(B, (uint32_t)(host_buffers ? std::min(ctx->chunk, ctx->host_chunk) : ctx->chunk), ctx->nlanes,
                                                 host_buffers != 0);
  if (v.size() > cap) return ZKA_E_ARG;
  for (size_t i = 0; i < v.size(); i++) off[i] = v[i];
  return (int)v.size() - 1;
}
int zka_lanes(const zka_ctx* ctx) { return ctx ? ctx->nlanes : 0; }
int zka_config(const zka_ctx* ctx, int* tom_w, int* tom_nwin, int* chunk) {
  if (!ctx) return ZKA_E_ARG;
  if (tom_w) *tom_w = ctx->tom_w;
  if (tom_nwin) *tom_nwin = ctx->tom_nwin;
  if (chunk) *chunk = ctx->chunk;
// ... 36 lines not shown
#endif
    if (const char* e = getenv("ZKA_HOST_CHUNK")) {
      int c = atoi(e);
      if (c >= 1) ctx->host_chunk = c;
    }
    stream_create(ctx->cs_in);
    stream_create(ctx->cs_out);
    stream_create(ctx->aux[0]);
    stream_create(ctx->aux[1]);
    {
      int lanes = 3;
#if defined(ZKA_HOSTSIM)
      lanes = 1;
#endif
      if (const char* e = getenv("ZKA_LANES")) lanes = atoi(e);
      if (lanes < 1) lanes = 1;
      if (lanes > 8) lanes = 8;
      if (zka_set_option(ctx.get(), "lanes", lanes) != 0) throw std::runtime_error("lanes");
    }
    if (const char* e = getenv("ZKA_TAPE_SPLIT")) ctx->tape_split = atoi(e) != 0;
    if (const char* e = getenv("ZKA_AGG")) ctx->agg = atoi(e);
    if (const char* e = getenv("ZKA_AGG_C")) {
      int c = atoi(e);
      if (c >= 4 && c <= 16) ctx->agg_c = c;
    }
    if (const char* e = getenv("ZKA_P256_HW")) {
      int w = atoi(e);
      if (w >= 8 && w <= 24) ctx->p256_hw = w;
    }
    DevBuf gen;
    uint32_t* d_gen = gen.get<uint32_t>(16 + TOM_AFF_WORDS);
    launch(ctx->st, 1, GenAffTask{d_gen, d_gen + 16});
    build_p256_tab(ctx.get(), d_gen, ctx->g8, 8);
    build_p256_tab(ctx.get(), d_gen, ctx->gw, ctx->p256_hw);
    build_tom_tab(ctx.get(), d_gen + 16, ctx->tg);
    DevBuf proj, aff;
    uint32_t* d_proj = proj.get<uint32_t>(TOM_PROJ_WORDS);
    uint32_t* d_aff = aff.get<uint32_t>(TOM_AFF_WORDS);
    uint8_t* d_bytes = ctx->tg_bytes.get<uint8_t>(BSTRIDE);
    launch(ctx->st, 1, GProjTask{d_gen + 16, d_proj});
    launch_tom_norm(ctx->st, d_proj, d_aff, d_bytes, 1, 0);
    sync(ctx->st);
    return 0;
  });
  if (rc) {
    fprintf(stderr, "zka_init: %s\n", ctx->err.c_str());
    return rc;
  }
  *out = ctx.release();
  return 0;
}

void zka_shutdown(zka_ctx* ctx) { delete ctx; }

int zka_params_create(zka_ctx* ctx, const uint8_t h_nist[65], const uint8_t h_proof[67], uint32_t sec_level,
                      zka_params** out) {
  if (!ctx || !h_nist || !h_proof || !out) return ZKA_E_ARG;
  if (sec_level < 1 || sec_level > MAX_REPS) return fail(ctx, ZKA_E_ARG, "sec_level must be in [1,80]");
  return guarded(ctx, [&] {
    std::unique_ptr<zka_params> P(new zka_params());
    P->ctx = ctx;
    P->sec_level = sec_level;
    P->h_w = ctx->p256_hw;
    memcpy(P->h_nist, h_nist, 65);
    memcpy(P->h_proof, h_proof, WP);
    DevBuf bn, bt, an, at, bad, inf;
    uint8_t* d_bn = bn.get<uint8_t>(65);
    uint8_t* d_bt = bt.get<uint8_t>(WP);
    uint32_t* d_an = an.get<uint32_t>(16);
    uint32_t* d_at = at.get<uint32_t>(TOM_AFF_WORDS);
    uint8_t* d_bad = bad.get<uint8_t>(2);
    uint8_t* d_inf = inf.get<uint8_t>(1);
    copy_h2d(ctx->st, d_bn, h_nist, 65);
    copy_h2d(ctx->st, d_bt, h_proof, WP);
    launch(ctx->st, 1, ParsePointsTask{d_bn, nullptr, d_an, nullptr, d_bad, d_inf});
    launch(ctx->st, 1, ParsePointsTask{nullptr, d_bt, nullptr, d_at, d_bad + 1, nullptr});
    uint8_t hb[3];
    copy_d2h(ctx->st, hb, d_bad, 2);
    copy_d2h(ctx->st, hb + 2, d_inf, 1);
    sync(ctx->st);
    if (hb[0] || hb[1] || hb[2]) return fail(ctx, ZKA_E_ARG, "params: h point not on its group");
    build_p256_tab(ctx, d_an, P->h8, P->h_w);
    build_tom_tab(ctx, d_at, P->th);
    *out = P.release();
    return 0;
  });
}

void zka_params_destroy(zka_params* P) { delete P; }

int zka_rings_create(zka_ctx* ctx, uint32_t R, const uint32_t* sizes, const uint8_t* keys, zka_rings** out) {
  if (!ctx || !sizes || !keys || !out) return ZKA_E_ARG;
  *out = nullptr;
  if (R == 0) return fail(ctx, ZKA_E_ARG, "a ring set holds at least one ring");
  if (R > (1u << 23)) return fail(ctx, ZKA_E_ARG, "ring set exceeds 2^24 padded entries");
  std::unique_ptr<zka_rings> set(new zka_rings());
  set->ctx = ctx;
  set->R = R;
  std::vector<uint32_t> key_off(R), base(R);
  uint64_t nkeys = 0, total = 0;
  for (uint32_t r = 0; r < R; r++) {
    const uint32_t N = sizes[r];
    if (N < 2 || N > (1u << 20)) return fail(ctx, ZKA_E_ARG, "ring size must be in [2, 2^20]");
    const int n = ceil_log2(N);
    set->size.push_back(N);
    set->depth.push_back(n);
    key_off[r] = (uint32_t)nkeys;
    base[r] = (uint32_t)total;
    nkeys += N;
    total += 1ull << n;
    if (total > (1ull << 24)) return fail(ctx, ZKA_E_ARG, "ring set exceeds 2^24 padded entries");
  }
  return guarded(ctx, [&] {
    Stream& st = ctx->st;
    DevBuf kbuf, obuf;
    const uint8_t* d_keys = stage_in(st, kbuf, keys, (size_t)nkeys * 32);
    uint32_t* d_off = obuf.get<uint32_t>(R);
    uint32_t* d_base = set->ring_base.get<uint32_t>(R);
    uint32_t* d_size = set->ring_size.get<uint32_t>(R);
    uint32_t* ring_m = set->ring_m.get<uint32_t>((size_t)total * 8);
    copy_h2d(st, d_off, key_off.data(), (size_t)R * 4);
    copy_h2d(st, d_base, base.data(), (size_t)R * 4);
    copy_h2d(st, d_size, set->size.data(), (size_t)R * 4);
    launch(st, (long long)total, RingSetPrepTask{d_keys, d_off, d_base, d_size, ring_m, (int)R});
    sync(st);
    *out = set.release();
    return 0;
  });
}

void zka_rings_destroy(zka_rings* set) { delete set; }

size_t zka_proof_max_len(uint32_t ring_size, uint32_t sec_level) {
  return (size_t)proof_len((int)sec_level, ceil_log2(ring_size), (int)sec_level);
}
size_t zka_prove_tape_len(uint32_t ring_size, uint32_t sec_level) {
  return (size_t)32 * prove_draws((int)sec_level, ceil_log2(ring_size), (int)sec_level);
}
size_t zka_verify_tape_len(uint32_t ring_size, uint32_t sec_level) {
  return verify_tape_len(ceil_log2(ring_size), (int)sec_level);
}

int zka_tom_commit_batch(zka_ctx* ctx, const zka_params* P, uint32_t count, const uint8_t* v, const uint8_t* r,
                         uint8_t* out) {
  if (!ctx || !P || !v || !r || !out) return ZKA_E_ARG;
  if (count == 0) return 0;
  return guarded(ctx, [&] {
    Stream& st = ctx->st;
    Cursor in(ctx->in[0]), w(ctx->w), ob(ctx->out[0]);
    const uint8_t* dv = stage_in(st, in.next(), v, (size_t)count * 32);
    const uint8_t* dr = stage_in(st, in.next(), r, (size_t)count * 32);
    uint32_t* jv = w.take<uint32_t>((size_t)count * 8);
    uint32_t* jr = w.take<uint32_t>((size_t)count * 8);
    uint32_t* proj = w.take<uint32_t>((size_t)count * TOM_PROJ_WORDS);
    uint32_t* aff = w.take<uint32_t>((size_t)count * TOM_AFF_WORDS);
    uint8_t* bytes = w.take<uint8_t>((size_t)count * BSTRIDE);
    const Output<uint8_t> o(out, WP);
    uint8_t* packed = o.rows(ob.next(), 0, count);
    launch(st, count, CommitConvTask{dv, dr, jv, jr});
    launch(st, count, TomCommitTask{jv, jr, ctx->tg.tab, P->th.tab, proj, ctx->tom_w, ctx->tom_nwin});
    launch_tom_norm(st, proj, aff, bytes, (long long)(count), 1);
    launch(st, count, PackTomTask{bytes, packed});
    o.copy_back(st, 0, packed, count);
    sync(st);
    return 0;
  });
}

int zka_p256_mul_batch(zka_ctx* ctx, uint32_t count, const uint8_t* base, const uint8_t* k, uint8_t* out) {
  if (!ctx || !k || !out) return ZKA_E_ARG;
  if (count == 0) return 0;
  return guarded(ctx, [&] {
    Stream& st = ctx->st;
    Cursor in(ctx->in[0]), w(ctx->w), ob(ctx->out[0]);
    const uint8_t* dk = stage_in(st, in.next(), k, (size_t)count * 32);
    const uint8_t* db = stage_in(st, in.next(), base, (size_t)count * 65);
    uint32_t* proj = w.take<uint32_t>((size_t)count * P256_PROJ_WORDS);
    uint32_t* aff = w.take<uint32_t>((size_t)count * P256_AFF_WORDS);
    uint8_t* bytes = w.take<uint8_t>((size_t)count * BSTRIDE);
    uint8_t* inf = w.take<uint8_t>(count);
    const bool per_base = db != nullptr;
    uint32_t* baff = w.take_if<uint32_t>(per_base, (size_t)count * 16);
    uint8_t* bad = w.take_if<uint8_t>(per_base, count);
    uint8_t* binf = w.take_if<uint8_t>(per_base, count);
    uint32_t* pows = w.take_if<uint32_t>(per_base, (size_t)count * RT_NWIN * P256_PROJ_WORDS);
    uint32_t* rows = w.take_if<uint32_t>(per_base, (size_t)count * RT_ENTRIES * P256_PROJ_WORDS);
    uint32_t* rtab = w.take_if<uint32_t>(per_base, (size_t)count * RT_ENTRIES * P256_AFF_WORDS);
    const Output<uint8_t> o(out, NP);
    uint8_t* packed = o.rows(ob.next(), 0, count);
    if (per_base) {
      launch(st, count, ParsePointsTask{db, nullptr, baff, nullptr, bad, binf});
      launch(st, count, P256PowsTask{baff, binf, pows, (int)count, RT_NWIN, RT_W});
      launch(st, (long long)count * RT_NWIN, P256RowsSignedTask{pows, rows});
      const long long np = (long long)count * RT_ENTRIES;
      launch_p256_norm(st, rows, rtab, nullptr, nullptr, (long long)(np));
    }
    launch(st, count, P256MulTask{dk, ctx->g8.tab, rtab, binf, proj});
    launch_p256_norm(st, proj, aff, bytes, inf, (long long)(count));
    launch(st, count, PackP256Task{bytes, packed});
    o.copy_back(st, 0, packed, count);
    sync(st);
    return 0;
  });
}


int zka_field_op_batch(zka_ctx* ctx, int field, int op, uint32_t count, const uint8_t* a, const uint8_t* b,
                       uint8_t* out) {
  if (!ctx || !a || !out || field < 0 || field > 2 || op < 0 || op > 4 || (op < 3 && !b)) return ZKA_E_ARG;
  if (count == 0) return 0;
  return guarded(ctx, [&] {
    Stream& st = ctx->st;
    Cursor in(ctx->in[0]), ob(ctx->out[0]);
    const int nb = field == 2 ? WCB : 32;
    const uint8_t* da = stage_in(st, in.next(), a, (size_t)count * nb);
    const uint8_t* db = stage_in(st, in.next(), b, (size_t)count * nb);
    const Output<uint8_t> o(out, nb);
    uint8_t* dout = o.rows(ob.next(), 0, count);
    if (field == 0) launch(st, count, FieldOpTask<P256p, 32>{da, db, dout, op});
    else if (field == 1) launch(st, count, FieldOpTask<P256n, 32>{da, db, dout, op});
    else launch(st, count, FieldOpTask<PGp, WCB>{da, db, dout, op});
    o.copy_back(st, 0, dout, count);
    sync(st);
    return 0;
  });
}

int zka_hash80_batch(zka_ctx* ctx, uint32_t count, const uint8_t* msgs, size_t msg_stride, const uint32_t* len,
                     uint8_t* out) {
  if (!ctx || !msgs || !len || !out) return ZKA_E_ARG;
  if (count == 0) return 0;
  return guarded(ctx, [&] {
    Stream& st = ctx->st;
    Cursor in(ctx->in[0]), ob(ctx->out[0]);
    const uint8_t* dm = stage_in(st, in.next(), msgs, (size_t)count * msg_stride);
    const uint32_t* dl = stage_in(st, in.next(), len, (size_t)count);
    const Output<uint8_t> o(out, 10);
    uint8_t* dout = o.rows(ob.next(), 0, count);
    launch(st, count, Hash80Task{dm, msg_stride, dl, dout});
    o.copy_back(st, 0, dout, count);
    sync(st);
    return 0;
  });
}

int zka_params_generate(zka_ctx* ctx, const uint8_t rnd[64], uint8_t h_nist[65], uint8_t h_proof[67]) {
  if (!ctx || !rnd || !h_nist || !h_proof) return ZKA_E_ARG;
  return guarded(ctx, [&] {
    int rc = zka_p256_mul_batch(ctx, 1, nullptr, rnd, h_nist);
    if (rc) return rc;
    Stream& st = ctx->st;
    Cursor in(ctx->in[0]), w(ctx->w);
    uint32_t* jv = w.take<uint32_t>(8);
    uint32_t* jr = w.take<uint32_t>(8);
    uint32_t* proj = w.take<uint32_t>(TOM_PROJ_WORDS);
    uint32_t* aff = w.take<uint32_t>(TOM_AFF_WORDS);
    uint8_t* bytes = w.take<uint8_t>(BSTRIDE);
    uint8_t* d_rnd = in.take<uint8_t>(32);
    copy_h2d(st, d_rnd, rnd + 32, 32);
    launch(st, 1, GenConvTask{d_rnd, jv, jr});
    launch(st, 1, TomCommitTask{jv, jr, ctx->tg.tab, ctx->tg.tab, proj, ctx->tom_w, ctx->tom_nwin});
    launch_tom_norm(st, proj, aff, bytes, (long long)(1), 1);
    copy_d2h(st, h_proof, bytes, WP);
    sync(st);
    return 0;
  });
}

int zka_key_to_int(zka_ctx* ctx, uint32_t count, const uint8_t* pk, uint8_t* x_out, int32_t* status) {
  if (!ctx || !pk || !x_out) return ZKA_E_ARG;
  if (count == 0) return 0;
  return guarded(ctx, [&] {
    Stream& st = ctx->st;
    Cursor in(ctx->in[0]), w(ctx->w), ob(ctx->out[0]);
    const uint8_t* dp = stage_in(st, in.next(), pk, (size_t)count * 65);
    uint32_t* aff = w.take<uint32_t>((size_t)count * 16);
    uint8_t* bad = w.take<uint8_t>(count);
    uint8_t* inf = w.take<uint8_t>(count);
    const Output<uint8_t> xo(x_out, 32);
    const Output<int32_t> so(status, 1);
    uint8_t* dx = xo.rows(ob.next(), 0, count);
    int32_t* ds = so.rows(ob.next(), 0, count);
    launch(st, count, ParsePointsTask{dp, nullptr, aff, nullptr, bad, inf});
    launch(st, count, KeyToIntTask{aff, bad, inf, dx, ds});
    xo.copy_back(st, 0, dx, count);
    if (status) so.copy_back(st, 0, ds, count);
    sync(st);
    return 0;
  });
}

static int prove_impl(zka_ctx* ctx, const zka_params* P, uint32_t B, const uint8_t* msg_hash, const uint8_t* sig,
                      const uint8_t* pk, const uint32_t* which, const uint8_t* ring, uint32_t N, const uint8_t* tape,
                      size_t tape_stride, uint8_t* proofs, size_t proof_stride, uint32_t* proof_len_out,
                      int32_t* status, int mode, const uint8_t* base, const uint8_t* s_in, const uint8_t* q_in,
                      const uint8_t* seeds = nullptr, const RingPass* rp = nullptr) {
  if (!ctx || !P || !pk || (!tape && !seeds) || !proofs || !proof_len_out || !status) return ZKA_E_ARG;
  if (mode == 0 && (!msg_hash || !sig || !which || (!ring && !rp))) return ZKA_E_ARG;
  if (mode == 1 && (!base || !s_in)) return ZKA_E_ARG;
  if (B == 0) return 0;
  if (mode == 0 && !rp && (N < 2 || N > (1u << 20))) return fail(ctx, ZKA_E_ARG, "ring size must be in [2, 2^20]");
  const int S = (int)P->sec_level;
  const int n = rp ? rp->n : mode == 0 ? ceil_log2(N) : 0;
  if (proof_stride < (mode == 0 ? (size_t)proof_len(S, n, S) : (size_t)S * REP0_LEN)) return fail(ctx, ZKA_E_ARG, "proof_stride < zka_proof_max_len");
  const bool seeded = seeds != nullptr;
  if (!seeded && tape_stride < (size_t)32 * (mode == 0 ? prove_draws(0, n, S) : draws_before_items(S))) return fail(ctx, ZKA_E_ARG, "tape_stride too small");
  const int seed_draws = prove_draws(S, n, S);
  return guarded(ctx, [&] {
    const uint32_t* ring_m = nullptr;
    if (rp) {
      ring_m = (const uint32_t*)rp->set->ring_m.p;
      prep_lagrange(ctx, ctx->st, n);
      sync(ctx->st);
    } else if (mode == 0) {
      ring_m = prep_ring(ctx, ctx->st, ring, N, n, true);
      sync(ctx->st);
    }
    const Output<uint8_t> po(proofs, proof_stride);
    const Output<uint32_t> lo(proof_len_out, 1);
    const Output<int32_t> so(status, 1);
    const int lanes = ctx->nlanes;
    const size_t dev_tape_stride = (tape_stride + 15) & ~(size_t)15;
    const bool all_dev = po.dev && is_device_ptr(seeded ? seeds : tape);
    const std::vector<uint32_t> off = chunk_schedule(B, (uint32_t)(all_dev ? ctx->chunk : std::min(ctx->chunk, ctx->host_chunk)), lanes, !all_dev);
    const uint32_t nchunks = (uint32_t)off.size() - 1;
    const int used = (int)std::min<uint32_t>((uint32_t)lanes, nchunks);
    const bool trace = getenv("ZKA_TRACE") != nullptr;
    const auto t_call = std::chrono::steady_clock::now();
    auto ms_now = [&] { return std::chrono::duration<double, std::milli>(std::chrono::steady_clock::now() - t_call).count(); };
    std::atomic<uint32_t> next_chunk((uint32_t)used);
    auto run_lane = [&](int li) {
      Lane& ln = ctx->lane(li);
      Stream& st = ln.st;
      struct ChunkIn { const uint8_t *msg_hash, *sig, *pk, *tape, *base, *s_in, *q_in, *seeds; const uint32_t *which, *ring_of; } cin[2];
      auto issue_inputs = [&](uint32_t k, int slot) {
        const uint32_t b0 = off[k];
        const size_t Bc = off[k + 1] - b0;
        Stream& ci = ln.cs_in;
        Cursor in(ln.in[slot]);
        DevBuf& tape_buf = in.next();
        auto rows = [&](auto* p, size_t width) { return stage_in(ci, in.next(), p ? p + b0 * width : p, Bc * width); };
        ev_wait(ci, ln.ev_done[slot]);
        cin[slot].msg_hash = rows(msg_hash, 32);
        cin[slot].sig = rows(sig, 64);
        cin[slot].pk = rows(pk, 65);
        cin[slot].which = rows(which, 1);
        cin[slot].ring_of = rows(rp ? rp->ring_of : nullptr, 1);
        cin[slot].base = rows(base, 65);
        cin[slot].s_in = rows(s_in, 32);
        cin[slot].q_in = rows(q_in, 65);
        cin[slot].seeds = rows(seeds, 32);
        ev_record(ln.ev_small[slot], ci);
        if (seeded) {
          cin[slot].tape = tape_buf.get<uint8_t>(Bc * (size_t)32 * seed_draws);
        } else if (is_device_ptr(tape)) {
          cin[slot].tape = tape + (size_t)b0 * tape_stride;
        } else if (!ctx->tape_split && dev_tape_stride == tape_stride) {
          cin[slot].tape = stage_in(ci, tape_buf, tape + (size_t)b0 * tape_stride, Bc * tape_stride);
        } else {
          uint8_t* dt = tape_buf.get<uint8_t>(Bc * dev_tape_stride);
          const size_t width = ctx->tape_split ? std::min(tape_stride, (size_t)32 * draws_before_items(S)) : tape_stride;
          copy_d2h_2d(ci, dt, dev_tape_stride, tape + (size_t)b0 * tape_stride, tape_stride, width, Bc);
          cin[slot].tape = dt;
        }
        ev_record(ln.ev_tape[slot], ci);
      };
      uint32_t k = (uint32_t)li;
      int slot = 0;
      if (k < nchunks) issue_inputs(k, slot);
      for (; k < nchunks; slot ^= 1) {
        const uint32_t b0 = off[k];
        const int Bc = (int)(off[k + 1] - b0);
        const uint32_t k_this = k;
        const double t_begin = ms_now();
        ev_wait(st, ln.ev_small[slot]);
        ev_wait(st, ln.ev_out[slot]);
        ProveCtx c = prove_ctx(ctx, P, Bc, S, (int)N, n);
        c.mode = mode; c.head_len = mode == 0 ? HEAD_LEN : 0;
        c.base = cin[slot].base; c.s_in = cin[slot].s_in; c.q_in = cin[slot].q_in;
        c.msg_hash = cin[slot].msg_hash;
        c.sig = cin[slot].sig;
        c.pk = cin[slot].pk;
        c.which = cin[slot].which;
        c.tape = cin[slot].tape;
        c.tape_stride = seeded ? (size_t)32 * seed_draws : is_device_ptr(tape) ? tape_stride : dev_tape_stride;
        c.tape_draws = seeded ? (uint32_t)seed_draws : (uint32_t)(tape_stride / 32);
        c.ring_m = ring_m;
        if (rp) {
          c.ring_of = cin[slot].ring_of;
          c.ring_base = (const uint32_t*)rp->set->ring_base.p;
          c.ring_size = (const uint32_t*)rp->set->ring_size.p;
        }
        const size_t S1 = (size_t)S + 1;
        const size_t nA = (size_t)Bc * S1;
        const size_t n1 = (size_t)Bc * (2 + 2 * S);
        Cursor w(ln.w);
        c.s1 = w.take<uint32_t>((size_t)Bc * 8);
        c.pk_aff = w.take<uint32_t>((size_t)Bc * 16);
        c.q_aff = w.take<uint32_t>((size_t)Bc * 16);
        c.q_inf = w.take<uint8_t>(Bc);
        c.r_aff = w.take<uint32_t>((size_t)Bc * 16);
        c.r_bytes = w.take<uint8_t>((size_t)Bc * BSTRIDE);
        c.rpows = w.take<uint32_t>((size_t)Bc * RT_NWIN * P256_PROJ_WORDS);
        c.rrows = w.take<uint32_t>((size_t)Bc * KEY_CAP * P256_PROJ_WORDS);
        c.rtab = w.take<uint32_t>((size_t)Bc * KEY_CAP * P256_AFF_WORDS);
        c.pa_T = w.take<uint32_t>(nA * P256_PROJ_WORDS);
        c.pa_A = w.take<uint32_t>(nA * P256_PROJ_WORDS);
        c.pa_T_aff = w.take<uint32_t>(nA * 16);
        c.pa_T_inf = w.take<uint8_t>(nA);
        c.pa_A_aff = w.take<uint32_t>(nA * 16);
        c.pa_A_bytes = w.take<uint8_t>(nA * BSTRIDE);
        c.pa_A_inf = w.take<uint8_t>(nA);
        c.s1_jv = w.take<uint32_t>(n1 * 8);
        c.s1_jr = w.take<uint32_t>(n1 * 8);
        c.s1_proj = w.take<uint32_t>(n1 * TOM_PROJ_WORDS);
        c.s1_aff = w.take<uint32_t>(n1 * TOM_AFF_WORDS);
        c.s1_bytes = w.take<uint8_t>(n1 * BSTRIDE);
        c.chal = w.take<uint32_t>((size_t)Bc * 3);
        c.zcount = w.take<uint32_t>(Bc);
        c.item_base = w.take<uint32_t>(Bc);
        c.item_total = w.take<uint32_t>(2);
        c.rep_off = w.take<uint32_t>((size_t)Bc * S);
        c.gk_off = w.take<uint32_t>(Bc);
        c.gk_dv = w.take<uint32_t>((size_t)Bc * n * 8);
        c.gk_x = w.take<uint32_t>((size_t)Bc * 3);
        c.u12 = w.take<uint32_t>((size_t)Bc * 16);
        c.tab_of = w.take<uint32_t>(Bc);
        c.tab_rep = w.take<uint32_t>((size_t)Bc * 2);
        c.tab_count = w.take<uint32_t>(2);
        c.which_s = w.take<uint32_t>(Bc);
        uint32_t* base_aff = w.take_if<uint32_t>(mode == 1, (size_t)Bc * 16);
        c.base_aff = mode == 0 ? c.pk_aff : base_aff;
        c.proof_stride = proof_stride;
        Cursor ob(ln.out[slot]);
        c.proofs = po.rows(ob.next(), b0, Bc);
        c.proof_len = lo.rows(ob.next(), b0, Bc);
        c.status = so.rows(ob.next(), b0, Bc);
  
        launch(st, Bc, PreKeyTask{c});
        launch(st, Bc, KeyDedupTask{c});
        launch(st, Bc, KeyRankTask{c});
        launch(st, Bc, KeyAssignTask{c});
        {
          const int Bp = (Bc + 31) & ~31;
          launch(st, (long long)Bp + Bc,
                 PowsAndPreTask{P256PowsTask{c.base_aff, nullptr, c.rpows, Bc, RT_NWIN, RT_W, c.tab_rep, c.tab_count, c.tab_count + 1}, PreTask{c}, Bp});
        }
        launch(st, (long long)Bc * ((KEY_CAP + 15) / 16), P256RowsBlockTask{c.rpows, c.rrows, KEY_W_MIN, c.tab_count, c.tab_count + 1});
        {
          const long long np = (long long)Bc * KEY_CAP;
          const uint32_t kest = rp ? (uint32_t)Bc : std::min<uint32_t>(N, (uint32_t)Bc);
          const int west = key_window_bits(kest, (uint32_t)Bc, (uint32_t)S + 2);
          const int ch = norm_chunk_for((long long)kest * fb_windows(west) * fb_entries(west), 5);
          launch(st, (np + ch - 1) / ch, P256NormTask{c.rrows, c.rtab, nullptr, nullptr, (int)np, ch, c.tab_count, 0, c.tab_count + 1});
        }
        ev_wait(st, ln.ev_tape[slot]);
        if (seeded) {
          const int d1 = draws_before_items(S);
          launch(st, (long long)Bc * d1, SeedProveTapeTask{cin[slot].seeds, const_cast<uint8_t*>(c.tape), c.tape_stride, S, n, 0, d1, nullptr});
        }
        {
          const int nAp = (int)((nA + 31) & ~(size_t)31);
          launch(st, (long long)nAp + Bc, PhaseAAndRPointTask{PhaseAP256Task{c}, RPointTask{c}, (int)nA, nAp});
        }
        launch_p256_norm(st, c.pa_T, c.pa_T_aff, nullptr, c.pa_T_inf, (long long)(nA));
        launch_p256_norm(st, c.pa_A, c.pa_A_aff, c.pa_A_bytes, c.pa_A_inf, (long long)(nA));
        if (mode == 1) launch(st, Bc, ExpStatementTask{c});
        prove_store1(st, c);
        launch(st, Bc, ExpChallengeTask{c});
        launch(st, 1, ScanTask{c});
        uint32_t tot2[2] = {0, 0};
        copy_d2h(st, tot2, c.item_total, 8);
        const bool tape_host = !seeded && ctx->tape_split && !is_device_ptr(tape);
        sync(st);
        if (seeded) {
          const int d1 = draws_before_items(S), span = prove_draws((int)tot2[1], n, S) - d1;
          launch(st, (long long)Bc * span, SeedProveTapeTask{cin[slot].seeds, const_cast<uint8_t*>(c.tape), c.tape_stride, S, n, d1, span, c.zcount});
        } else if (tape_host) {
          const size_t o0 = (size_t)32 * draws_before_items(S);
          const size_t o1 = std::min(tape_stride, (size_t)32 * prove_draws((int)tot2[1], n, S));
          if (o1 > o0)
            copy_d2h_2d(st, const_cast<uint8_t*>(c.tape) + o0, c.tape_stride, tape + (size_t)b0 * tape_stride + o0, tape_stride, o1 - o0, Bc);
        }
        const double t_mid = ms_now();
        {
          const uint32_t kn = next_chunk.fetch_add(1);
          if (kn < nchunks) issue_inputs(kn, slot ^ 1);
          k = kn;
        }
        const uint32_t M = tot2[0];
        const size_t max_len = mode == 0 ? (size_t)proof_len((int)tot2[1], n, S)
                                         : (size_t)tot2[1] * REP0_LEN + (size_t)(S - (int)tot2[1]) * REP1_LEN;
        c.M = (int)M;
        c.item_b = w.take<uint32_t>(M);
        c.item_i = w.take<uint32_t>(M);
        c.item_k = w.take<uint32_t>(M);
        c.pb_T1 = w.take<uint32_t>((size_t)M * P256_PROJ_WORDS);
        c.pb_T1_aff = w.take<uint32_t>((size_t)M * 16);
        c.pb_T1_inf = w.take<uint8_t>(M);
        const size_t n2 = c.s2_count();
        c.s2_jv = w.take<uint32_t>(n2 * 8);
        c.s2_jr = w.take<uint32_t>(n2 * 8);
        c.s2_proj = w.take<uint32_t>(n2 * TOM_PROJ_WORDS);
        c.s2_aff = w.take<uint32_t>(n2 * TOM_AFF_WORDS);
        c.s2_bytes = w.take<uint8_t>(n2 * BSTRIDE);
        c.secrets = w.take<uint32_t>((size_t)M * SECRETS_PER_ITEM * 8);
        c.item_inv = w.take<uint32_t>((size_t)M * 8);
        c.item_chal = w.take<uint32_t>((size_t)M * HASHES_PER_ITEM * 3);
        c.gk_part = w.take_if<uint32_t>(gk_blocks(n) > 1, (size_t)Bc * n * gk_blocks(n) * 8);
        uint32_t* gext = w.take<uint32_t>((size_t)M * GJOBS_PER_ITEM * TOM_EXT_WORDS);
        launch(st, Bc, ItemsTask{c});
        launch(st, M, PhaseBP256Task{c});
        launch_p256_norm(st, c.pb_T1, c.pb_T1_aff, nullptr, c.pb_T1_inf, (long long)(M));
        prove_items_gk(st, c, gext, true, true);
        launch(st, (long long)nA, RepEmitTask{c});
        if (mode == 0) launch(st, Bc, GkEmitTask{c});
        launch(st, (long long)Bc * FIN_PARTS, FinalizeTask{c});
        ev_record(ln.ev_done[slot], st);
        if (ctx->progress && !rp && k_this < ctx->progress_cap) notify_progress(st, ctx->progress + k_this);
        if (!po.dev || !lo.dev || !so.dev) {
          Stream& co = ln.cs_out;
          ev_wait(co, ln.ev_done[slot]);
          po.copy_back_2d(co, b0, c.proofs, Bc, max_len);
          lo.copy_back(co, b0, c.proof_len, Bc);
          so.copy_back(co, b0, c.status, Bc);
          ev_record(ln.ev_out[slot], co);
        }
        if (trace) {
          const double t_enq = ms_now();
          sync(st);
          const double t_comp = ms_now();
          sync(ln.cs_out);
          fprintf(stderr, "TRACE lane %d chunk %u rows %d begin %.2f mid %.2f enqueued %.2f computed %.2f copied %.2f\n", li, k_this, Bc,
                  t_begin, t_mid, t_enq, t_comp, ms_now());
        }
      }
      sync(ln.cs_in);
      sync(ln.cs_out);
      sync(st);
    };
    run_lanes(ctx, used, run_lane);
    return 0;
  });
}

int zka_prove_batch(zka_ctx* ctx, const zka_params* P, uint32_t B, const uint8_t* msg_hash, const uint8_t* sig,
                    const uint8_t* pk, const uint32_t* which, const uint8_t* ring, uint32_t N, const uint8_t* tape,
                    size_t tape_stride, uint8_t* proofs, size_t proof_stride, uint32_t* proof_len_out,
                    int32_t* status) {
  return prove_impl(ctx, P, B, msg_hash, sig, pk, which, ring, N, tape, tape_stride, proofs, proof_stride, proof_len_out, status, 0,
                    nullptr, nullptr, nullptr);
}

int zka_prove_batch_seeded(zka_ctx* ctx, const zka_params* P, uint32_t B, const uint8_t* msg_hash, const uint8_t* sig,
                           const uint8_t* pk, const uint32_t* which, const uint8_t* ring, uint32_t N, const uint8_t* seeds,
                           uint8_t* proofs, size_t proof_stride, uint32_t* proof_len_out, int32_t* status) {
  if (!seeds) return ZKA_E_ARG;
  return prove_impl(ctx, P, B, msg_hash, sig, pk, which, ring, N, nullptr, 0, proofs, proof_stride, proof_len_out, status, 0,
                    nullptr, nullptr, nullptr, seeds);
}

static int prove_rings(zka_ctx* ctx, const zka_params* P, const zka_rings* set, const uint32_t* ring_of, uint32_t B,
                       const uint8_t* msg_hash, const uint8_t* sig, const uint8_t* pk, const uint32_t* which, const uint8_t* tape,
                       size_t tape_stride, const uint8_t* seeds, uint8_t* proofs, size_t proof_stride, uint32_t* proof_len_out,
                       int32_t* status) {
  if (!ctx || !P || !set || !ring_of || !msg_hash || !sig || !pk || !which || (!tape && !seeds) || !proofs || !proof_len_out || !status)
    return ZKA_E_ARG;
  if (set->ctx != ctx) return fail(ctx, ZKA_E_ARG, "ring set of another context");
  if (B == 0) return 0;
  return guarded(ctx, [&] {
    RingRuns rr;
    if (const int rc = ring_runs(ctx, set, ring_of, B, rr)) return rc;
    const int S = (int)P->sec_level;
    if (proof_stride < (size_t)proof_len(S, rr.nmax, S)) return fail(ctx, ZKA_E_ARG, "proof_stride < zka_proof_max_len");
    if (tape && tape_stride < (size_t)32 * prove_draws(0, rr.nmax, S)) return fail(ctx, ZKA_E_ARG, "tape_stride too small");
    for (size_t k = 0; k + 1 < rr.start.size(); k++) {
      const uint32_t r0 = rr.start[k], rows = rr.start[k + 1] - r0;
      const RingPass rp{set, ring_of + r0, rr.depth[k]};
      const int rc = prove_impl(ctx, P, rows, msg_hash + (size_t)r0 * 32, sig + (size_t)r0 * 64, pk + (size_t)r0 * 65, which + r0,
                                nullptr, 0, tape ? tape + (size_t)r0 * tape_stride : nullptr, tape_stride,
                                proofs + (size_t)r0 * proof_stride, proof_stride, proof_len_out + r0, status + r0, 0, nullptr, nullptr,
                                nullptr, seeds ? seeds + (size_t)r0 * 32 : nullptr, &rp);
      if (rc) return rc;
    }
    return 0;
  });
}

int zka_prove_batch_rings(zka_ctx* ctx, const zka_params* P, const zka_rings* rings, const uint32_t* ring_of, uint32_t B,
                          const uint8_t* msg_hash, const uint8_t* sig, const uint8_t* pk, const uint32_t* which, const uint8_t* tape,
                          size_t tape_stride, uint8_t* proofs, size_t proof_stride, uint32_t* proof_len_out, int32_t* status) {
  if (!tape) return ZKA_E_ARG;
  return prove_rings(ctx, P, rings, ring_of, B, msg_hash, sig, pk, which, tape, tape_stride, nullptr, proofs, proof_stride,
                     proof_len_out, status);
}

int zka_prove_batch_rings_seeded(zka_ctx* ctx, const zka_params* P, const zka_rings* rings, const uint32_t* ring_of, uint32_t B,
                                 const uint8_t* msg_hash, const uint8_t* sig, const uint8_t* pk, const uint32_t* which,
                                 const uint8_t* seeds, uint8_t* proofs, size_t proof_stride, uint32_t* proof_len_out, int32_t* status) {
  if (!seeds) return ZKA_E_ARG;
  return prove_rings(ctx, P, rings, ring_of, B, msg_hash, sig, pk, which, nullptr, 0, seeds, proofs, proof_stride, proof_len_out,
                     status);
}

int zka_seed_tape(zka_ctx* ctx, int kind, uint32_t B, const uint8_t* seeds, uint32_t ring_size, uint32_t sec_level,
                  uint32_t samples, uint8_t* tape, size_t tape_stride) {
  if (!ctx || !seeds || !tape || (kind != 0 && kind != 1)) return ZKA_E_ARG;
  if (B == 0) return 0;
  if (ring_size < 2 || ring_size > (1u << 20)) return fail(ctx, ZKA_E_ARG, "ring size must be in [2, 2^20]");
  if (sec_level < 1 || sec_level > MAX_REPS) return fail(ctx, ZKA_E_ARG, "sec_level must be in [1,80]");
  const int S = (int)sec_level, n = ceil_log2(ring_size), K = (int)samples;
  if (kind == 1 && K < 1) return fail(ctx, ZKA_E_ARG, "samples must be >= 1");
  if (kind == 1 && S < K) return fail(ctx, ZKA_E_ARG, "security level not achieved");
  const size_t len = kind == 0 ? (size_t)32 * prove_draws(S, n, S) : verify_tape_len(n, S, K);
  if (tape_stride < len) return fail(ctx, ZKA_E_ARG, kind == 0 ? "tape_stride < zka_prove_tape_len" : "tape_stride < zka_verify_tape_len");
  return guarded(ctx, [&] {
    Stream& st = ctx->st;
    const uint32_t rows = 1024;
    for (uint32_t b0 = 0; b0 < B; b0 += rows) {
      const uint32_t Bc = std::min(rows, B - b0);
      Cursor in(ctx->in[0]), w(ctx->w);
      const uint8_t* ds = stage_in(st, in.next(), seeds + (size_t)b0 * 32, (size_t)Bc * 32);
      uint8_t* dt = w.take<uint8_t>((size_t)Bc * len);
      if (kind == 0) {
        launch(st, (long long)Bc * prove_draws(S, n, S), SeedProveTapeTask{ds, dt, len, S, n, 0, prove_draws(S, n, S), nullptr});
      } else {
        const SeedVerifyTapeTask vt{ds, dt, len, n, S, K};
        launch(st, (long long)Bc * vt.slots(), vt);
      }
      copy_d2h_2d(st, tape + (size_t)b0 * tape_stride, tape_stride, dt, len, len, Bc);
      sync(st);
    }
    return 0;
  });
}

int zka_prove_exp_batch(zka_ctx* ctx, const zka_params* P, uint32_t B, const uint8_t* base, const uint8_t* s, const uint8_t* pk,
                        const uint8_t* q, const uint8_t* tape, size_t tape_stride, uint8_t* proofs, size_t proof_stride,
                        uint32_t* proof_len, int32_t* status) {
  return prove_impl(ctx, P, B, nullptr, nullptr, pk, nullptr, nullptr, 2, tape, tape_stride, proofs, proof_stride, proof_len, status, 1,
                    base, s, q);
}

int zka_prove_membership_batch(zka_ctx* ctx, const zka_params* P, uint32_t B, const uint8_t* com_r, const uint32_t* index,
                               const uint8_t* ring, uint32_t N, const uint8_t* tape, size_t tape_stride, uint8_t* proofs,
                               size_t proof_stride, uint32_t* proof_len, int32_t* status) {
  if (!ctx || !P || !com_r || !index || !ring || !tape || !proofs || !proof_len || !status) return ZKA_E_ARG;
  if (B == 0) return 0;
  if (N < 2 || N > (1u << 20)) return fail(ctx, ZKA_E_ARG, "ring size must be in [2, 2^20]");
  const int n = ceil_log2(N);
  if (proof_stride < (size_t)gk_len(n)) return fail(ctx, ZKA_E_ARG, "proof_stride < GK block length");
  if (tape_stride < (size_t)32 * 5 * n) return fail(ctx, ZKA_E_ARG, "tape_stride < 32 * 5n");
  return guarded(ctx, [&] {
    Stream& st = ctx->st;
    const uint32_t* ring_m = prep_ring(ctx, st, ring, N, n, true);
    const Output<uint8_t> po(proofs, proof_stride);
    const Output<uint32_t> lo(proof_len, 1);
    const Output<int32_t> so(status, 1);
    const size_t it_len = 96 + tape_stride, it_stride = (it_len + 15) & ~(size_t)15;
    const uint32_t chunk = 8192;
    for (uint32_t b0 = 0; b0 < B; b0 += chunk) {
      const int Bc = (int)std::min<uint32_t>(chunk, B - b0);
      Cursor in(ctx->in[0]), w(ctx->w), ob(ctx->out[0]);
      const uint8_t* d_cr = stage_in(st, in.next(), com_r + (size_t)b0 * 32, (size_t)Bc * 32);
      const uint32_t* d_idx = stage_in(st, in.next(), index + b0, (size_t)Bc);
      const uint8_t* d_tape = stage_in(st, in.next(), tape + (size_t)b0 * tape_stride, (size_t)Bc * tape_stride);
      ProveCtx c = prove_ctx(ctx, P, Bc, 0, (int)N, n);
      c.which = d_idx;
      c.ring_m = ring_m;
      uint8_t* itape = w.take<uint8_t>((size_t)Bc * it_stride);
      c.tape = itape; c.tape_stride = it_stride; c.tape_draws = (uint32_t)(it_len / 32);
      c.which_s = w.take<uint32_t>(Bc);
      c.zcount = w.take<uint32_t>(Bc);
      c.gk_off = w.take<uint32_t>(Bc);
      c.gk_dv = w.take<uint32_t>((size_t)Bc * n * 8);
      c.gk_x = w.take<uint32_t>((size_t)Bc * 3);
      const size_t ng = (size_t)Bc * 4 * n;
      c.s2_jv = w.take<uint32_t>(ng * 8);
      c.s2_jr = w.take<uint32_t>(ng * 8);
      c.s2_proj = w.take<uint32_t>(ng * TOM_PROJ_WORDS);
      c.s2_bytes = w.take<uint8_t>(ng * BSTRIDE);
      c.gk_part = w.take_if<uint32_t>(gk_blocks(n) > 1, (size_t)Bc * n * gk_blocks(n) * 8);
      c.proof_stride = proof_stride;
      c.proofs = po.rows(ob.next(), b0, Bc);
      c.proof_len = lo.rows(ob.next(), b0, Bc);
      c.status = so.rows(ob.next(), b0, Bc);
      launch(st, Bc, GkAloneSetupTask{c, d_cr, d_tape, tape_stride, itape});
      prove_items_gk(st, c, nullptr, false, true);
      launch(st, Bc, GkEmitTask{c});
      launch(st, (long long)Bc * FIN_PARTS, FinalizeTask{c});
      po.copy_back_2d(st, b0, c.proofs, Bc, (size_t)gk_len(n));
      lo.copy_back(st, b0, c.proof_len, Bc);
      so.copy_back(st, b0, c.status, Bc);
      sync(st);
    }
    return 0;
  });
}

static int prove_sub(zka_ctx* ctx, const zka_params* P, int kind, uint32_t B, const uint8_t* scalars, const uint8_t* tape,
                     size_t tape_stride, uint8_t* commitments, uint8_t* proofs, int32_t* status) {
  if (!ctx || !P || !scalars || !tape || !commitments || !proofs || !status) return ZKA_E_ARG;
  if (B == 0) return 0;
  const int ns = kind == 0 ? 3 : 6, nd = kind == 0 ? 3 : 7, J = kind == 0 ? SUBP_EQ_JOBS : SUBP_MULT_JOBS;
  const int nc = kind == 0 ? 2 : 3, plen = kind == 0 ? EQ_LEN : MULT_LEN;
  if (tape_stride < (size_t)32 * nd) return fail(ctx, ZKA_E_ARG, "tape_stride too small for this sub-proof");
  return guarded(ctx, [&] {
    Stream& st = ctx->st;
    const Output<uint8_t> co(commitments, (size_t)nc * WP), po(proofs, plen);
    const Output<int32_t> so(status, 1);
    const uint32_t chunk = 16384;
    for (uint32_t b0 = 0; b0 < B; b0 += chunk) {
      const int Bc = (int)std::min<uint32_t>(chunk, B - b0);
      Cursor in(ctx->in[0]), w(ctx->w), ob(ctx->out[0]);
      const uint8_t* d_sc = stage_in(st, in.next(), scalars + (size_t)b0 * ns * 32, (size_t)Bc * ns * 32);
      const uint8_t* d_tape = stage_in(st, in.next(), tape + (size_t)b0 * tape_stride, (size_t)Bc * tape_stride);
      const size_t nj = (size_t)Bc * J;
      uint32_t* jv = w.take<uint32_t>(nj * 8);
      uint32_t* jr = w.take<uint32_t>(nj * 8);
      uint32_t* proj = w.take<uint32_t>(nj * TOM_PROJ_WORDS);
      uint8_t* bytes = w.take<uint8_t>(nj * BSTRIDE);
      uint8_t* d_com = co.rows(ob.next(), b0, Bc);
      uint8_t* d_prf = po.rows(ob.next(), b0, Bc);
      int32_t* d_st = so.rows(ob.next(), b0, Bc);
      launch(st, Bc, SubProveJobsTask{kind, d_sc, d_tape, tape_stride, jv, jr, d_st});
      launch(st, (long long)nj, TomCommitTask{jv, jr, ctx->tg.tab, P->th.tab, proj, ctx->tom_w, ctx->tom_nwin});
      launch_tom_norm(st, proj, nullptr, bytes, (long long)nj, 1);
      launch(st, Bc, SubProveEmitTask{kind, d_sc, d_tape, tape_stride, jr, bytes, d_com, d_prf, d_st});
      co.copy_back(st, b0, d_com, Bc);
      po.copy_back(st, b0, d_prf, Bc);
      so.copy_back(st, b0, d_st, Bc);
      sync(st);
    }
    return 0;
  });
}
int zka_prove_equality_batch(zka_ctx* ctx, const zka_params* P, uint32_t B, const uint8_t* scalars, const uint8_t* tape,
                             size_t tape_stride, uint8_t* commitments, uint8_t* proofs, int32_t* status) {
  return prove_sub(ctx, P, 0, B, scalars, tape, tape_stride, commitments, proofs, status);
}
int zka_prove_mult_batch(zka_ctx* ctx, const zka_params* P, uint32_t B, const uint8_t* scalars, const uint8_t* tape,
                         size_t tape_stride, uint8_t* commitments, uint8_t* proofs, int32_t* status) {
  return prove_sub(ctx, P, 1, B, scalars, tape, tape_stride, commitments, proofs, status);
}

int zka_prove_pointadd_batch(zka_ctx* ctx, const zka_params* P, uint32_t B, const uint8_t* points, const uint8_t* blinders,
                             const uint8_t* tape, size_t tape_stride, uint8_t* commitments, uint8_t* proofs, int32_t* status) {
  if (!ctx || !P || !points || !blinders || !tape || !commitments || !proofs || !status) return ZKA_E_ARG;
  if (B == 0) return 0;
  if (tape_stride < (size_t)32 * 38) return fail(ctx, ZKA_E_ARG, "tape_stride < 32 * 38");
  return guarded(ctx, [&] {
    Stream& st = ctx->st;
    const size_t it_stride = (size_t)32 * (9 + 38);
    const size_t row_stride = REP0_LEN;
    const Output<uint8_t> co(commitments, 6 * WP), po(proofs, PA_LEN);
    const Output<int32_t> so(status, 1);
    const uint32_t chunk = 8192;
    for (uint32_t b0 = 0; b0 < B; b0 += chunk) {
      const int Bc = (int)std::min<uint32_t>(chunk, B - b0);
      Cursor in(ctx->in[0]), w(ctx->w), ob(ctx->out[0]);
      const uint8_t* d_pts = stage_in(st, in.next(), points + (size_t)b0 * 195, (size_t)Bc * 195);
      const uint8_t* d_bl = stage_in(st, in.next(), blinders + (size_t)b0 * 192, (size_t)Bc * 192);
      const uint8_t* d_tape = stage_in(st, in.next(), tape + (size_t)b0 * tape_stride, (size_t)Bc * tape_stride);
      ProveCtx c = prove_ctx(ctx, P, Bc, 1, 2, 0);
      c.M = Bc; c.mode = 1; c.head_len = 0;
      uint8_t* itape = w.take<uint8_t>((size_t)Bc * it_stride);
      c.tape = itape; c.tape_stride = it_stride; c.tape_draws = (uint32_t)(it_stride / 32);
      const size_t n1 = (size_t)Bc * 4, n2 = (size_t)Bc * (JOBS_PER_ITEM + DERS_PER_ITEM);
      c.s1 = w.take<uint32_t>((size_t)Bc * 8);
      c.pk_aff = w.take<uint32_t>((size_t)Bc * 16);
      c.pa_T_aff = w.take<uint32_t>((size_t)Bc * 2 * 16);
      c.pa_T_inf = w.take<uint8_t>((size_t)Bc * 2);
      c.pa_A_inf = w.take<uint8_t>((size_t)Bc * 2);
      c.pb_T1_aff = w.take<uint32_t>((size_t)Bc * 16);
      c.pb_T1_inf = w.take<uint8_t>(Bc);
      c.chal = w.take<uint32_t>((size_t)Bc * 3);
      c.zcount = w.take<uint32_t>(Bc);
      c.item_base = w.take<uint32_t>(Bc);
      c.item_b = w.take<uint32_t>(Bc);
      c.item_i = w.take<uint32_t>(Bc);
      c.item_k = w.take<uint32_t>(Bc);
      c.rep_off = w.take<uint32_t>(Bc);
      c.s1_jv = w.take<uint32_t>(n1 * 8);
      c.s1_jr = w.take<uint32_t>(n1 * 8);
      c.s1_proj = w.take<uint32_t>(n1 * TOM_PROJ_WORDS);
      c.s1_aff = w.take<uint32_t>(n1 * TOM_AFF_WORDS);
      c.s1_bytes = w.take<uint8_t>(n1 * BSTRIDE);
      c.s2_jv = w.take<uint32_t>(n2 * 8);
      c.s2_jr = w.take<uint32_t>(n2 * 8);
      c.s2_proj = w.take<uint32_t>(n2 * TOM_PROJ_WORDS);
      c.s2_aff = w.take<uint32_t>(n2 * TOM_AFF_WORDS);
      c.s2_bytes = w.take<uint8_t>(n2 * BSTRIDE);
      c.secrets = w.take<uint32_t>((size_t)Bc * SECRETS_PER_ITEM * 8);
      c.item_inv = w.take<uint32_t>((size_t)Bc * 8);
      c.item_chal = w.take<uint32_t>((size_t)Bc * HASHES_PER_ITEM * 3);
      uint32_t* gext = w.take<uint32_t>((size_t)Bc * GJOBS_PER_ITEM * TOM_EXT_WORDS);
      c.proof_stride = row_stride;
      c.proofs = w.take<uint8_t>((size_t)Bc * row_stride);
      c.proof_len = w.take<uint32_t>(Bc);
      uint8_t* d_com = co.rows(ob.next(), b0, Bc);
      uint8_t* d_prf = po.rows(ob.next(), b0, Bc);
      c.status = so.rows(ob.next(), b0, Bc);
      launch(st, Bc, PaddSetupTask{c, d_pts, d_bl, d_tape, tape_stride, itape});
      prove_store1(st, c);
      prove_items_gk(st, c, gext, true, false);
      launch(st, Bc, PaddExtractTask{c, d_com, d_prf});
      co.copy_back(st, b0, d_com, Bc);
      po.copy_back(st, b0, d_prf, Bc);
      so.copy_back(st, b0, c.status, Bc);
      sync(st);
    }
    return 0;
  });
}

size_t zka_verify_tape_len_ex(uint32_t ring_size, uint32_t sec_level, uint32_t samples) {
  return verify_tape_len(ceil_log2(ring_size), (int)sec_level, (int)samples);
}

int zka_verify_batch(zka_ctx* ctx, const zka_params* P, uint32_t B, const uint8_t* msg_hash, const uint8_t* ring,
                     uint32_t N, const uint8_t* proofs, size_t proof_stride, const uint32_t* proof_len,
                     const uint8_t* tape, size_t tape_stride, uint8_t* ok, int32_t* status) {
  return zka_verify_batch_ex(ctx, P, B, msg_hash, ring, N, proofs, proof_stride, proof_len, tape, tape_stride, ok, status, V_SAMPLES);
}

static int verify_impl(zka_ctx* ctx, const zka_params* P, uint32_t B, const uint8_t* msg_hash, const uint8_t* ring,
                       uint32_t N, const uint8_t* proofs, size_t proof_stride, const uint32_t* proof_len,
                       const uint8_t* tape, size_t tape_stride, uint8_t* ok, int32_t* status, uint32_t samples, int mode,
                       const uint8_t* q_ext, const uint8_t* seeds = nullptr, const RingPass* rp = nullptr);

int zka_verify_batch_ex(zka_ctx* ctx, const zka_params* P, uint32_t B, const uint8_t* msg_hash, const uint8_t* ring,
                        uint32_t N, const uint8_t* proofs, size_t proof_stride, const uint32_t* proof_len,
                        const uint8_t* tape, size_t tape_stride, uint8_t* ok, int32_t* status, uint32_t samples) {
  if (!msg_hash || !ring) return ZKA_E_ARG;
  return verify_impl(ctx, P, B, msg_hash, ring, N, proofs, proof_stride, proof_len, tape, tape_stride, ok, status, samples, 0, nullptr);
}

int zka_verify_batch_seeded(zka_ctx* ctx, const zka_params* P, uint32_t B, const uint8_t* msg_hash, const uint8_t* ring,
                            uint32_t N, const uint8_t* proofs, size_t proof_stride, const uint32_t* proof_len,
                            const uint8_t* seeds, uint32_t samples, uint8_t* ok, int32_t* status) {
  if (!msg_hash || !ring || !seeds) return ZKA_E_ARG;
  return verify_impl(ctx, P, B, msg_hash, ring, N, proofs, proof_stride, proof_len, nullptr, 0, ok, status, samples, 0, nullptr, seeds);
}

static int verify_rings(zka_ctx* ctx, const zka_params* P, const zka_rings* set, const uint32_t* ring_of, uint32_t B,
                        const uint8_t* msg_hash, const uint8_t* proofs, size_t proof_stride, const uint32_t* proof_len,
                        const uint8_t* tape, size_t tape_stride, const uint8_t* seeds, uint32_t samples, uint8_t* ok, int32_t* status) {
  if (!ctx || !P || !set || !ring_of || !msg_hash || !proofs || !proof_len || (!tape && !seeds) || !ok || !status) return ZKA_E_ARG;
  if (set->ctx != ctx) return fail(ctx, ZKA_E_ARG, "ring set of another context");
  if (B == 0) return 0;
  return guarded(ctx, [&] {
    RingRuns rr;
    if (const int rc = ring_runs(ctx, set, ring_of, B, rr)) return rc;
    const int S = (int)P->sec_level, K = (int)samples;
    if (K < 1) return fail(ctx, ZKA_E_ARG, "samples must be >= 1");
    if (S < K) return fail(ctx, ZKA_E_ARG, "security level not achieved");
    if (tape && tape_stride < verify_tape_len(rr.nmax, S, K)) return fail(ctx, ZKA_E_ARG, "tape_stride < zka_verify_tape_len");
    for (size_t k = 0; k + 1 < rr.start.size(); k++) {
      const uint32_t r0 = rr.start[k], rows = rr.start[k + 1] - r0;
      const RingPass rp{set, ring_of + r0, rr.depth[k]};
      const int rc = verify_impl(ctx, P, rows, msg_hash + (size_t)r0 * 32, nullptr, 0, proofs + (size_t)r0 * proof_stride, proof_stride,
                                 proof_len + r0, tape ? tape + (size_t)r0 * tape_stride : nullptr, tape_stride, ok + r0, status + r0,
                                 samples, 0, nullptr, seeds ? seeds + (size_t)r0 * 32 : nullptr, &rp);
      if (rc) return rc;
    }
    return 0;
  });
}

int zka_verify_batch_rings(zka_ctx* ctx, const zka_params* P, const zka_rings* rings, const uint32_t* ring_of, uint32_t B,
                           const uint8_t* msg_hash, const uint8_t* proofs, size_t proof_stride, const uint32_t* proof_len,
                           const uint8_t* tape, size_t tape_stride, uint32_t samples, uint8_t* ok, int32_t* status) {
  if (!tape) return ZKA_E_ARG;
  return verify_rings(ctx, P, rings, ring_of, B, msg_hash, proofs, proof_stride, proof_len, tape, tape_stride, nullptr, samples, ok,
                      status);
}

int zka_verify_batch_rings_seeded(zka_ctx* ctx, const zka_params* P, const zka_rings* rings, const uint32_t* ring_of, uint32_t B,
                                  const uint8_t* msg_hash, const uint8_t* proofs, size_t proof_stride, const uint32_t* proof_len,
                                  const uint8_t* seeds, uint32_t samples, uint8_t* ok, int32_t* status) {
  if (!seeds) return ZKA_E_ARG;
  return verify_rings(ctx, P, rings, ring_of, B, msg_hash, proofs, proof_stride, proof_len, nullptr, 0, seeds, samples, ok, status);
}

static int verify_impl(zka_ctx* ctx, const zka_params* P, uint32_t B, const uint8_t* msg_hash, const uint8_t* ring,
                       uint32_t N, const uint8_t* proofs, size_t proof_stride, const uint32_t* proof_len,
                       const uint8_t* tape, size_t tape_stride, uint8_t* ok, int32_t* status, uint32_t samples, int mode,
                       const uint8_t* q_ext, const uint8_t* seeds, const RingPass* rp) {
  if (!ctx || !P || !proofs || !proof_len || (!tape && !seeds) || !ok || !status) return ZKA_E_ARG;
  if (B == 0) return 0;
  if (!rp && (N < 2 || N > (1u << 20))) return fail(ctx, ZKA_E_ARG, "ring size must be in [2, 2^20]");
  const int S = (int)P->sec_level;
  const int K = (int)samples;
  if (K < 1) return fail(ctx, ZKA_E_ARG, "samples must be >= 1");
  if (S < K) return fail(ctx, ZKA_E_ARG, "security level not achieved");
  const int n = rp ? rp->n : ceil_log2(N);
  const bool seeded = seeds != nullptr;
  if (!seeded && tape_stride < (mode == 1 ? (size_t)V_IDX_PAD + (size_t)32 * 25 * K : verify_tape_len(n, S, K)))
    return fail(ctx, ZKA_E_ARG, "tape_stride < zka_verify_tape_len");
  const size_t seed_stride = verify_tape_len(n, S, K);
  return guarded(ctx, [&] {
    const uint32_t* ring_m = nullptr;
    if (rp) {
      ring_m = (const uint32_t*)rp->set->ring_m.p;
    } else if (mode == 0) {
      ring_m = prep_ring(ctx, ctx->st, ring, N, n, false);
      sync(ctx->st);
    }
    const Output<uint8_t> oo(ok, 1);
    const Output<int32_t> so(status, 1);
    const int lanes = ctx->nlanes;
    const bool all_dev = is_device_ptr(proofs) && is_device_ptr(seeded ? seeds : tape);
    const std::vector<uint32_t> off = chunk_schedule(B, (uint32_t)std::min(ctx->chunk, all_dev ? 4096 : std::min(4096, ctx->host_chunk)), lanes, !all_dev);
    const uint32_t nchunks = (uint32_t)off.size() - 1;
    const int used = (int)std::min<uint32_t>((uint32_t)lanes, nchunks);
    std::atomic<uint32_t> next_chunk((uint32_t)used);
    const bool trace = getenv("ZKA_TRACE") != nullptr;
    const auto t_call = std::chrono::steady_clock::now();
    auto ms_now = [&] { return std::chrono::duration<double, std::milli>(std::chrono::steady_clock::now() - t_call).count(); };
    struct VIn { const uint8_t* msg; const uint8_t* proofs; const uint32_t* plen; const uint8_t* tape; const uint8_t* seeds; const uint32_t* ring_of; };
    auto stage_chunk = [&](Lane& ln, int slot, uint32_t kk) {
      std::lock_guard<std::mutex> copy_lock(ctx->copy_mu);
      Stream& ci = ctx->cs_in;
      Cursor in(ln.in[slot]);
      DevBuf& rows_buf = in.next();
      const uint32_t b0 = off[kk];
      const size_t Bc = off[kk + 1] - b0;
      VIn v;
      v.msg = stage_in(ci, in.next(), msg_hash ? msg_hash + (size_t)b0 * 32 : nullptr, Bc * 32);
      if (is_device_ptr(proofs) || is_device_ptr(proof_len)) {
        v.proofs = stage_in(ci, rows_buf, proofs + (size_t)b0 * proof_stride, Bc * proof_stride);
      } else {
        size_t w = 0;
        for (size_t i = 0; i < Bc; i++) w = std::max<size_t>(w, proof_len[b0 + i]);
        w = std::min(proof_stride, (w + 15) & ~(size_t)15);
        uint8_t* dp = rows_buf.get<uint8_t>(Bc * proof_stride);
        copy_d2h_2d(ci, dp, proof_stride, proofs + (size_t)b0 * proof_stride, proof_stride, w, Bc);
        v.proofs = dp;
      }
      v.plen = stage_in(ci, in.next(), proof_len + b0, Bc);
      if (seeded) v.tape = in.next().get<uint8_t>(Bc * seed_stride);
      else v.tape = stage_in(ci, in.next(), tape + (size_t)b0 * tape_stride, Bc * tape_stride);
      v.seeds = stage_in(ci, in.next(), seeded ? seeds + (size_t)b0 * 32 : nullptr, Bc * 32);
      v.ring_of = stage_in(ci, in.next(), rp ? rp->ring_of + b0 : nullptr, Bc);
      ev_record(ln.ev_small[slot], ci);
      return v;
    };
    std::vector<VIn> first((size_t)used);
    for (int li = 0; li < used; li++) first[(size_t)li] = stage_chunk(ctx->lane(li), 0, (uint32_t)li);
    auto run_lane = [&](int li) {
      Lane& ln = ctx->lane(li);
      Stream& st = ln.st;
      uint32_t k = (uint32_t)li;
      if (k >= nchunks) return;
      int slot = 0;
      VIn cur = first[(size_t)li];
      for (;;) {
      const uint32_t kn = next_chunk.fetch_add(1);
      VIn nxt{};
      if (kn < nchunks) nxt = stage_chunk(ln, slot ^ 1, kn);
      ev_wait(st, ln.ev_small[slot]);
      const uint32_t b0 = off[k];
      const int Bc = (int)(off[k + 1] - b0);
      const double t_begin = trace ? ms_now() : 0.0;
      VerifyCtx c = verify_ctx(ctx, P, Bc, S, (int)N, n, K, mode);
      c.q_ext = q_ext ? q_ext + (size_t)b0 * NP : nullptr;
      c.msg_hash = cur.msg;
      c.proofs = cur.proofs;
      c.proof_stride = proof_stride;
      c.proof_len = cur.plen;
      c.tape = cur.tape;
      c.tape_stride = seeded ? seed_stride : tape_stride;
      c.ring_m = ring_m;
      if (rp) {
        c.ring_of = cur.ring_of;
        c.ring_base = (const uint32_t*)rp->set->ring_base.p;
      }
      if (seeded) {
        const SeedVerifyTapeTask vt{cur.seeds, const_cast<uint8_t*>(cur.tape), seed_stride, n, S, K};
        launch(st, (long long)Bc * vt.slots(), vt);
      }
      double t_in = 0.0;
      if (trace) { sync(st); t_in = ms_now(); }
      const size_t ns = (size_t)Bc * K;
      const int ET = c.ent_tom(), EN = c.ent_nist(), SG = c.segs();
      const int ngk = 4 * n + 1;
      Cursor w(ln.w);
      c.rep_off = w.take<uint32_t>((size_t)Bc * S);
      c.gk_off = w.take<uint32_t>(Bc);
      c.tagbits = w.take<uint32_t>((size_t)Bc * 3);
      c.chal = w.take<uint32_t>((size_t)Bc * 3);
      c.gk_ok_len = w.take<uint8_t>(Bc);
      c.r_aff = w.take<uint32_t>((size_t)Bc * 16);
      c.q_aff = w.take<uint32_t>((size_t)Bc * 16);
      c.q_inf = w.take<uint8_t>(Bc);
      c.rpows = w.take<uint32_t>((size_t)Bc * RT_NWIN * P256_PROJ_WORDS);
      c.rrows = w.take<uint32_t>((size_t)Bc * RT_ENTRIES * P256_PROJ_WORDS);
      c.rtab = w.take<uint32_t>((size_t)Bc * RT_ENTRIES * P256_AFF_WORDS);
      c.samp_idx = w.take<uint32_t>(ns);
      c.samp_draw = w.take<uint32_t>(ns);
      c.sp_T = w.take<uint32_t>(ns * P256_PROJ_WORDS);
      c.sp_T_aff = w.take<uint32_t>(ns * 16);
      c.sp_T_inf = w.take<uint8_t>(ns);
      c.ta_jv = w.take<uint32_t>(ns * 2 * 8);
      c.ta_jr = w.take<uint32_t>(ns * 2 * 8);
      c.ta_proj = w.take<uint32_t>(ns * 2 * TOM_PROJ_WORDS);
      c.ta_aff = w.take<uint32_t>(ns * 2 * TOM_AFF_WORDS);
      c.td_proj = w.take<uint32_t>(ns * DERS_PER_ITEM * TOM_PROJ_WORDS);
      c.td_aff = w.take<uint32_t>(ns * DERS_PER_ITEM * TOM_AFF_WORDS);
      c.td_bytes = w.take<uint8_t>(ns * DERS_PER_ITEM * BSTRIDE);
      c.item_chal = w.take<uint32_t>(ns * HASHES_PER_ITEM * 3);
      c.ent_scalar = w.take<uint32_t>((size_t)Bc * ET * 8);
      c.ent_off = w.take<uint32_t>((size_t)Bc * ET);
      c.ent_pre = w.take<uint32_t>((size_t)Bc * ET * TOM_PRE_WORDS);
      c.ent_cnt = w.take<uint32_t>(ns);
      c.part = w.take<uint32_t>(ns * V_PART_WORDS);
      c.fx_jv = w.take<uint32_t>((size_t)Bc * 2 * 8);
      c.fx_jr = w.take<uint32_t>((size_t)Bc * 2 * 8);
      c.fx_proj = w.take<uint32_t>((size_t)Bc * 2 * TOM_PROJ_WORDS);
      c.nfix = w.take<uint32_t>((size_t)Bc * P256_PROJ_WORDS);
      c.id_flags = w.take<uint8_t>((size_t)Bc * 3);
      c.gk_tape_bad = w.take_if<uint8_t>(mode == 0, Bc);
      c.nent_scalar = w.take<uint32_t>((size_t)Bc * EN * 8);
      c.nent_aff = w.take<uint32_t>((size_t)Bc * EN * 16);
      c.nent_skip = w.take<uint8_t>((size_t)Bc * EN);
      c.gk_scalar = w.take<uint32_t>((size_t)Bc * ngk * 8);
      c.gk_pre = w.take<uint32_t>((size_t)Bc * ngk * TOM_PRE_WORDS);
      uint32_t* gk_offs = w.take<uint32_t>((size_t)Bc * ngk);
      c.win_w = w.take<uint32_t>((size_t)Bc * SG * MSM_NWIN * 36);
      c.win_g = w.take<uint32_t>((size_t)Bc * MSM_NWIN * 36);
      c.win_n = w.take<uint32_t>((size_t)Bc * MSM_NWIN_N * P256_PROJ_WORDS);
      c.gk_part = w.take_if<uint32_t>(gk_blocks(n) > 1, (size_t)Bc * gk_blocks(n) * 8);
      Cursor ob(ln.out[0]);
      c.ok = oo.rows(ob.next(), b0, Bc);
      c.status = so.rows(ob.next(), b0, Bc);

      launch(st, Bc, VLayoutTask{c});
      launch(st, (long long)Bc * (S + 1), VValidateTask{c});
      {
        const bool fork = !st.profiling;
        Stream& sr = fork ? ln.aux[0] : st;
        if (fork) { ev_record(ln.ev_fork, st); ev_wait(sr, ln.ev_fork); }
        launch(sr, Bc, P256PowsTask{c.r_aff, nullptr, c.rpows, Bc, RT_NWIN, RT_W});
        launch(sr, (long long)Bc * RT_NWIN, P256RowsSignedTask{c.rpows, c.rrows});
        launch_p256_norm(sr, c.rrows, c.rtab, nullptr, nullptr, (long long)Bc * RT_ENTRIES);
        launch(st, Bc, VChallengeTask{c});
        if (fork) { ev_record(ln.ev_join[0], sr); ev_wait(st, ln.ev_join[0]); }
      }
      const bool gk_fork = mode == 0 && !st.profiling;
      if (gk_fork) {
        ev_record(ln.ev_fork, st);
        ev_wait(ln.aux[1], ln.ev_fork);
        verify_gk(ln.aux[1], c, gk_offs);
        ev_record(ln.ev_join[1], ln.aux[1]);
      }
      launch(st, (long long)ns, VSampleP256Task{c});
      launch_p256_norm(st, c.sp_T, c.sp_T_aff, nullptr, c.sp_T_inf, (long long)(ns));
      launch(st, (long long)ns, VSampleJobsTask{c});
      launch(st, (long long)ns * 2, TomCommitTask{c.ta_jv, c.ta_jr, c.tg_tab, c.th_tab, c.ta_proj, c.tom_w, c.tom_nwin});
      launch_tom_norm(st, c.ta_proj, c.ta_aff, nullptr, (long long)(ns * 2), 1);
      launch(st, (long long)ns, VDerivedTask{c});
      launch_tom_norm(st, c.td_proj, nullptr, c.td_bytes, (long long)(ns * DERS_PER_ITEM), 0);
      launch(st, (long long)ns * HASHES_PER_ITEM, VItemHashTask{c});
      dev_memset(st, c.ent_off, 0, (size_t)Bc * ET * 4);
      launch(st, (long long)ns, VRelationsTask{c});
      if (mode == 0) {
        if (gk_fork) ev_wait(st, ln.ev_join[1]);
        else verify_gk(st, c, gk_offs);
      }
      launch(st, Bc, VReduceTask{c});
      launch(st, (long long)Bc * ET, VParseEntriesTask{c.proofs, proof_stride, c.ent_off, c.ent_pre, ET});
      if (mode == 0) launch(st, (long long)Bc * ngk, VParseEntriesTask{c.proofs, proof_stride, gk_offs, c.gk_pre, ngk});
      launch(st, (long long)Bc * 2, TomCommitTask{c.fx_jv, c.fx_jr, c.tg_tab, c.th_tab, c.fx_proj, c.tom_w, c.tom_nwin});
      uint32_t* ctl = nullptr;
      if (ctx->agg && mode == 0) {
        Cursor A(ln.agg);
        const int fgroups = (Bc * 2 + 63) / 64, ngroups = (Bc + 31) / 32, ngroups2 = (ngroups + 31) / 32;
        ctl = A.take<uint32_t>(AGG_CTL_WORDS);
#if !defined(ZKA_PG_WAR256)
        uint32_t* tpart = A.take<uint32_t>((size_t)Bc * (K + 1) * 2 * PG_EXT_WORDS);
#endif
        uint32_t* fpart = A.take<uint32_t>((size_t)fgroups * 16);
        uint32_t* fjv = A.take<uint32_t>(8);
        uint32_t* fjr = A.take<uint32_t>(8);
        uint32_t* fproj = A.take<uint32_t>(TOM_PROJ_WORDS);
        uint32_t* npart = A.take<uint32_t>((size_t)ngroups * P256_PROJ_WORDS);
        uint32_t* npart2 = A.take_if<uint32_t>(ngroups > 32, (size_t)ngroups2 * P256_PROJ_WORDS);
        dev_memset(st, ctl, 0, AGG_CTL_WORDS * 4);
        launch(st, Bc, AggGateTask{c, ctl});
        const AggTomSrc tsrc{c.ent_scalar, c.ent_pre, c.ent_cnt, c.gk_scalar, c.gk_pre, Bc, ET, K, ngk};
        const AggNistSrc nsrc{c.nent_scalar, c.nent_aff, c.nent_skip, Bc, EN};
        const bool fork = !st.profiling;
        Stream& sa = fork ? ln.aux[0] : st;
        Stream& sb = fork ? ln.aux[1] : st;
        if (fork) {
          ev_record(ln.ev_fork, st);
          ev_wait(sa, ln.ev_fork);
          ev_wait(sb, ln.ev_fork);
        }
#if !defined(ZKA_PG_WAR256)
        launch(sa, (long long)Bc * (K + 1) * 2, AggTorsionPartTask{tsrc, ctl, tpart});
        launch(sa, Bc, AggTorsionTask{tpart, ctl, K});
#endif
        const AggPlan tp = agg_plan((double)Bc * (0.5 * K * V_ENT_PER_SAMPLE + 2 + ngk), ctx->agg_c);
        const AggPlan np = agg_plan((double)Bc * EN, 0);
        ctx->agg_c_last = tp.D.c;
        const uint32_t *tA, *tB, *nA, *nB;
        agg_msm(st, Cursor(ln.agg_tom), tsrc, tp, ctl, &tA, &tB);
        agg_msm(sb, Cursor(ln.agg_nist), nsrc, np, ctl, &nA, &nB);
        launch(st, fgroups, AggFixPartTask{ctl, c.fx_jv, c.fx_jr, fpart, Bc});
        launch(st, 1, AggFixSumTask{ctl, fpart, fjv, fjr, fgroups});
        launch(st, 1, TomCommitTask{fjv, fjr, c.tg_tab, c.th_tab, fproj, c.tom_w, c.tom_nwin});
        launch(sb, ngroups, AggNistFixPartTask{ctl, c.nfix, npart, Bc});
        int nleft = ngroups;
        const uint32_t* nsum = npart;
        if (nleft > 32) {
          launch(sb, ngroups2, AggNistFixPartTask{ctl, npart, npart2, nleft});
          nsum = npart2;
          nleft = ngroups2;
        }
        if (fork) {
          ev_record(ln.ev_join[0], sa);
          ev_record(ln.ev_join[1], sb);
          ev_wait(st, ln.ev_join[0]);
          ev_wait(st, ln.ev_join[1]);
        }
        launch(st, 33, AggFinalTask{ctl, tA, tB, fproj, tp.D.nwin, tp.D.c, nA, nB, nsum, np.D.nwin, np.D.c, nleft});
        c.agg_ctl = ctl;
      }
      {
        const int nW = Bc * SG * MSM_NWIN, nWp = (nW + 31) & ~31, nG = Bc * MSM_NWIN;
        launch(st, (long long)nWp + nG,
               MsmTomWindowBothTask{MsmTomWindowTask{c.ent_scalar, c.ent_pre, c.ent_cnt, ET, K, V_ENT_PER_SAMPLE, 2, V_SEG, SG, c.win_w},
                                    MsmTomWindowTask{c.gk_scalar, c.gk_pre, nullptr, ngk, 0, 0, mode == 0 ? ngk : 0, V_SEG, 1, c.win_g}, nW, nWp, nG, ctl});
      }
      launch(st, (long long)Bc * MSM_NWIN_N, MsmP256WindowTask{c.nent_scalar, c.nent_aff, c.nent_skip, c.win_n, EN, ctl});
      {
        const int Bp = (Bc + 31) & ~31;
        launch(st, 3ll * Bp, MsmCombineAllTask{MsmTomCombineTask{c.win_g, c.fx_proj, c.id_flags, 2, 0, 0},
                                               MsmTomCombineTask{c.win_w, c.fx_proj, c.id_flags, 2, 1, 1, SG},
                                               MsmP256CombineTask{c.win_n, c.nfix, c.id_flags}, Bc, Bp, ctl});
      }
      launch(st, Bc, VFinalTask{c});
      oo.copy_back(st, b0, c.ok, Bc);
      so.copy_back(st, b0, c.status, Bc);
      uint32_t hctl[AGG_CTL_WORDS] = {0, 0, 0, 0};
      if (ctl) copy_d2h(st, hctl, ctl, sizeof(hctl));
      const double t_enq = trace ? ms_now() : 0.0;
      sync(st);
      if (trace)
        fprintf(stderr, "VTRACE lane %d chunk %u rows %d begin %.2f inputs_on_device %.2f enqueued %.2f done %.2f\n", li, k, Bc, t_begin, t_in,
                t_enq, ms_now());
      if (ctl) {
        std::lock_guard<std::mutex> g(ctx->stat_mu);
        if (hctl[AGG_TOM_PASS] && hctl[AGG_NIST_PASS]) ctx->agg_pass++;
        else ctx->agg_fail++;
      }
      if (kn >= nchunks) break;
      k = kn;
      cur = nxt;
      slot ^= 1;
    }
    };
    run_lanes(ctx, used, run_lane);
    sync(ctx->cs_in);
    return 0;
  });
}

int zka_verify_exp_batch(zka_ctx* ctx, const zka_params* P, uint32_t B, const uint8_t* base, const uint8_t* com,
                         const uint8_t* px, const uint8_t* py, const uint8_t* q, const uint8_t* proofs, size_t proof_stride,
                         const uint32_t* proof_len, const uint8_t* tape, size_t tape_stride, uint32_t samples, uint8_t* ok,
                         int32_t* status) {
  if (!ctx || !P || !base || !com || !px || !py || !proofs || !proof_len || !tape || !ok || !status || proof_stride == 0) return ZKA_E_ARG;
  if (B == 0) return 0;
  return guarded(ctx, [&] {
    Stream& st = ctx->st;
    DevBuf bufs[10];
    Cursor in(bufs);
    const uint8_t* d_base = stage_in(st, in.next(), base, (size_t)B * NP);
    const uint8_t* d_com = stage_in(st, in.next(), com, (size_t)B * NP);
    const uint8_t* d_px = stage_in(st, in.next(), px, (size_t)B * WP);
    const uint8_t* d_py = stage_in(st, in.next(), py, (size_t)B * WP);
    const uint8_t* d_q = stage_in(st, in.next(), q, (size_t)B * NP);
    const uint8_t* d_body = stage_in(st, in.next(), proofs, (size_t)B * proof_stride);
    const uint32_t* d_len = stage_in(st, in.next(), proof_len, (size_t)B);
    const uint8_t* d_tape = stage_in(st, in.next(), tape, (size_t)B * tape_stride);
    const size_t row_stride = (HEAD_LEN + proof_stride + 15) & ~(size_t)15;
    uint8_t* d_rows = in.take<uint8_t>((size_t)B * row_stride);
    uint32_t* d_rlen = in.take<uint32_t>(B);
    const int pieces = (int)((row_stride + 63) / 64);
    launch(st, (long long)B * pieces, VAssembleTask{d_base, d_com, d_px, d_py, d_body, proof_stride, d_len, d_rows, row_stride, d_rlen, pieces});
    sync(st);
    return verify_impl(ctx, P, B, nullptr, nullptr, 2, d_rows, row_stride, d_rlen, d_tape, tape_stride, ok, status, samples, 1, d_q);
  });
}

int zka_verify_membership_batch(zka_ctx* ctx, const zka_params* P, uint32_t B, const uint8_t* com, const uint8_t* ring, uint32_t N,
                                const uint8_t* proofs, size_t proof_stride, const uint32_t* proof_len, const uint8_t* tape,
                                size_t tape_stride, uint8_t* ok, int32_t* status) {
  if (!ctx || !P || !com || !ring || !proofs || !proof_len || !tape || !ok || !status || proof_stride == 0) return ZKA_E_ARG;
  if (B == 0) return 0;
  if (N < 2 || N > (1u << 20)) return fail(ctx, ZKA_E_ARG, "ring size must be in [2, 2^20]");
  const int n = ceil_log2(N);
  if (tape_stride < (size_t)32 * (2 * n + 1)) return fail(ctx, ZKA_E_ARG, "tape_stride < 32 * (2n + 1)");
  return guarded(ctx, [&] {
    Stream& st = ctx->st;
    DevBuf bufs[4];
    const uint32_t* ring_m = prep_ring(ctx, st, ring, N, n, false);
    const Output<uint8_t> oo(ok, 1);
    const Output<int32_t> so(status, 1);
    const size_t row_stride = (HEAD_LEN + proof_stride + 15) & ~(size_t)15;
    const int pieces = (int)((row_stride + 63) / 64);
    const int ngk = 4 * n + 1;
    const uint32_t chunk = 4096;
    for (uint32_t b0 = 0; b0 < B; b0 += chunk) {
      const int Bc = (int)std::min<uint32_t>(chunk, B - b0);
      Cursor in(bufs), w(ctx->w), ob(ctx->out[0]);
      const uint8_t* d_com = stage_in(st, in.next(), com + (size_t)b0 * WP, (size_t)Bc * WP);
      const uint8_t* d_body = stage_in(st, in.next(), proofs + (size_t)b0 * proof_stride, (size_t)Bc * proof_stride);
      const uint32_t* d_len = stage_in(st, in.next(), proof_len + b0, (size_t)Bc);
      VerifyCtx c = verify_ctx(ctx, P, Bc, (int)P->sec_level, (int)N, n, 1, 2);
      c.tape = stage_in(st, in.next(), tape + (size_t)b0 * tape_stride, (size_t)Bc * tape_stride);
      c.tape_stride = tape_stride;
      c.ring_m = ring_m;
      uint8_t* d_rows = w.take<uint8_t>((size_t)Bc * row_stride);
      uint32_t* d_rlen = w.take<uint32_t>(Bc);
      c.proofs = d_rows; c.proof_stride = row_stride; c.proof_len = d_rlen;
      c.gk_off = w.take<uint32_t>(Bc);
      c.gk_ok_len = w.take<uint8_t>(Bc);
      c.gk_scalar = w.take<uint32_t>((size_t)Bc * ngk * 8);
      c.gk_pre = w.take<uint32_t>((size_t)Bc * ngk * TOM_PRE_WORDS);
      uint32_t* gk_offs = w.take<uint32_t>((size_t)Bc * ngk);
      c.fx_jv = w.take<uint32_t>((size_t)Bc * 2 * 8);
      c.fx_jr = w.take<uint32_t>((size_t)Bc * 2 * 8);
      c.fx_proj = w.take<uint32_t>((size_t)Bc * 2 * TOM_PROJ_WORDS);
      c.win_g = w.take<uint32_t>((size_t)Bc * MSM_NWIN * 36);
      c.id_flags = w.take<uint8_t>((size_t)Bc * 3);
      c.gk_part = w.take_if<uint32_t>(gk_blocks(n) > 1, (size_t)Bc * gk_blocks(n) * 8);
      c.ok = oo.rows(ob.next(), b0, Bc);
      c.status = so.rows(ob.next(), b0, Bc);
      launch(st, (long long)Bc * pieces, VAssembleTask{nullptr, nullptr, d_com, nullptr, d_body, proof_stride, d_len, d_rows, row_stride, d_rlen, pieces});
      launch(st, Bc, VGkOnlyLayoutTask{c});
      dev_memset(st, c.fx_jv, 0, (size_t)Bc * 2 * 8 * 4);
      dev_memset(st, c.fx_jr, 0, (size_t)Bc * 2 * 8 * 4);
      verify_gk(st, c, gk_offs);
      launch(st, (long long)Bc * ngk, VParseEntriesTask{c.proofs, row_stride, gk_offs, c.gk_pre, ngk});
      launch(st, (long long)Bc * 2, TomCommitTask{c.fx_jv, c.fx_jr, c.tg_tab, c.th_tab, c.fx_proj, c.tom_w, c.tom_nwin});
      launch(st, (long long)Bc * MSM_NWIN, MsmTomWindowTask{c.gk_scalar, c.gk_pre, nullptr, ngk, 0, 0, ngk, V_SEG, 1, c.win_g});
      launch(st, Bc, MsmTomCombineTask{c.win_g, c.fx_proj, c.id_flags, 2, 0, 0});
      launch(st, Bc, VGkOnlyFinalTask{c});
      oo.copy_back(st, b0, c.ok, Bc);
      so.copy_back(st, b0, c.status, Bc);
      sync(st);
    }
    return 0;
  });
}

static int verify_sub(zka_ctx* ctx, const zka_params* P, int kind, uint32_t B, const uint8_t* points, const uint8_t* proofs,
                      const uint8_t* tape, size_t tape_stride, uint8_t* ok, int32_t* status) {
  if (!ctx || !P || !points || !proofs || !tape || !ok || !status) return ZKA_E_ARG;
  if (B == 0) return 0;
  if (tape_stride < (size_t)32 * sub_draws(kind)) return fail(ctx, ZKA_E_ARG, "tape_stride too small for this sub-proof");
  return guarded(ctx, [&] {
    Stream& st = ctx->st;
    const int la = sub_points(kind) * WP, lc = sub_proof_len(kind), ne = sub_entries(kind);
    const size_t stride = (size_t)(la + lc + 15) & ~(size_t)15;
    const Output<uint8_t> oo(ok, 1);
    const Output<int32_t> so(status, 1);
    const uint32_t chunk = 8192;
    for (uint32_t b0 = 0; b0 < B; b0 += chunk) {
      const int Bc = (int)std::min<uint32_t>(chunk, B - b0);
      Cursor in(ctx->in[0]), w(ctx->w), ob(ctx->out[0]);
      const uint8_t* d_pts = stage_in(st, in.next(), points + (size_t)b0 * la, (size_t)Bc * la);
      const uint8_t* d_prf = stage_in(st, in.next(), proofs + (size_t)b0 * lc, (size_t)Bc * lc);
      const uint8_t* d_tape = stage_in(st, in.next(), tape + (size_t)b0 * tape_stride, (size_t)Bc * tape_stride);
      uint8_t* rows = w.take<uint8_t>((size_t)Bc * stride);
      uint32_t* ent_scalar = w.take<uint32_t>((size_t)Bc * SUB_ENT_MAX * 8);
      uint32_t* ent_off = w.take<uint32_t>((size_t)Bc * SUB_ENT_MAX);
      uint32_t* ent_pre = w.take<uint32_t>((size_t)Bc * SUB_ENT_MAX * TOM_PRE_WORDS);
      uint32_t* fx_jv = w.take<uint32_t>((size_t)Bc * 2 * 8);
      uint32_t* fx_jr = w.take<uint32_t>((size_t)Bc * 2 * 8);
      uint32_t* fx_proj = w.take<uint32_t>((size_t)Bc * 2 * TOM_PROJ_WORDS);
      uint32_t* win = w.take<uint32_t>((size_t)Bc * MSM_NWIN * 36);
      uint8_t* flags = w.take<uint8_t>((size_t)Bc * 3);
      uint8_t* d_ok = oo.rows(ob.next(), b0, Bc);
      int32_t* d_st = so.rows(ob.next(), b0, Bc);
      launch(st, (long long)Bc * (la + lc), VConcatTask{d_pts, d_prf, la, lc, rows, stride});
      launch(st, Bc, VSubProofTask{kind, rows, stride, d_tape, tape_stride, (const uint8_t*)ctx->tg_bytes.p, ent_scalar, ent_off,
                                   fx_jv, fx_jr, d_st, d_ok});
      launch(st, (long long)Bc * SUB_ENT_MAX, VParseEntriesTask{rows, stride, ent_off, ent_pre, SUB_ENT_MAX});
      launch(st, (long long)Bc * 2, TomCommitTask{fx_jv, fx_jr, ctx->tg.tab, P->th.tab, fx_proj, ctx->tom_w, ctx->tom_nwin});
      launch(st, (long long)Bc * MSM_NWIN, MsmTomWindowTask{ent_scalar, ent_pre, nullptr, SUB_ENT_MAX, 0, 0, ne, V_SEG, 1, win});
      launch(st, Bc, MsmTomCombineTask{win, fx_proj, flags, 2, 1, 1});
      launch(st, Bc, VSubFinalTask{d_st, flags, d_ok});
      oo.copy_back(st, b0, d_ok, Bc);
      so.copy_back(st, b0, d_st, Bc);
      sync(st);
    }
    return 0;
  });
}
int zka_verify_equality_batch(zka_ctx* ctx, const zka_params* P, uint32_t B, const uint8_t* points, const uint8_t* proofs,
                              const uint8_t* tape, size_t tape_stride, uint8_t* ok, int32_t* status) {
  return verify_sub(ctx, P, SUB_EQ, B, points, proofs, tape, tape_stride, ok, status);
}
int zka_verify_mult_batch(zka_ctx* ctx, const zka_params* P, uint32_t B, const uint8_t* points, const uint8_t* proofs,
                          const uint8_t* tape, size_t tape_stride, uint8_t* ok, int32_t* status) {
  return verify_sub(ctx, P, SUB_MULT, B, points, proofs, tape, tape_stride, ok, status);
}
int zka_verify_pointadd_batch(zka_ctx* ctx, const zka_params* P, uint32_t B, const uint8_t* points, const uint8_t* proofs,
                              const uint8_t* tape, size_t tape_stride, uint8_t* ok, int32_t* status) {
  return verify_sub(ctx, P, SUB_PADD, B, points, proofs, tape, tape_stride, ok, status);
}

namespace {
int pack_common(zka_ctx* ctx, uint32_t B, uint8_t* rows, size_t stride, const uint32_t* len, uint8_t* packed, size_t cap,
                uint64_t* offsets, void* stream, int dir) {
  if (!ctx || !rows || !len || !packed || !offsets || stride == 0) return ZKA_E_ARG;
  if (B == 0) return 0;
#if !defined(ZKA_HOSTSIM)
  if (!is_device_ptr(rows) || !is_device_ptr(len) || !is_device_ptr(packed) || !is_device_ptr(offsets))
    return fail(ctx, ZKA_E_ARG, "zka_proofs_pack/unpack take device pointers");
#endif
  return guarded(ctx, [&] {
    Stream tmp;
    Stream* st = &ctx->st;
#if !defined(ZKA_HOSTSIM)
    if (stream) { tmp.s = (cudaStream_t)stream; st = &tmp; }
#endif
    const int pieces = (int)((stride + 15) / 16);
    launch(*st, 1, PackScanTask{len, offsets, (int)B});
    const bool al = (stride % 16 == 0) && (((size_t)rows | (size_t)packed) % 16 == 0);
    if (al) launch(*st, (long long)B * pieces, PackCopy16Task{rows, stride, len, offsets, packed, cap, pieces, dir});
    else launch(*st, (long long)B * pieces, PackCopyTask{rows, stride, len, offsets, packed, cap, pieces, dir});
    if (st == &tmp) ctx->st.launches += tmp.launches; else sync(*st);
    return 0;
  });
}
}

int zka_proofs_pack(zka_ctx* ctx, uint32_t B, const uint8_t* proofs, size_t proof_stride, const uint32_t* proof_len,
                    uint8_t* packed, size_t cap, uint64_t* offsets, void* stream) {
  return pack_common(ctx, B, const_cast<uint8_t*>(proofs), proof_stride, proof_len, packed, cap, offsets, stream, 0);
}
int zka_proofs_unpack(zka_ctx* ctx, uint32_t B, const uint8_t* packed, size_t cap, const uint32_t* proof_len, uint8_t* proofs,
                      size_t proof_stride, uint64_t* offsets, void* stream) {
  return pack_common(ctx, B, proofs, proof_stride, proof_len, const_cast<uint8_t*>(packed), cap, offsets, stream, 1);
}

}
```

Baseline: 108,800.

## Skip identity start and defer final madd products into batched normalization

Fixed-base commitment loops now seed the accumulator directly from the first table entry instead of adding to the identity. They also stop the last mixed addition before its final multiplications, storing the E/F/G/H intermediates in a wider 36-word record. The batched-inversion normalization consumes these intermediates so the deferred products are folded into work it already does. In the Weierstrass build the accumulation moves to Jacobian coordinates. Commitment buffers grow to the wider stride, which adds memory traffic, and every stride change has to stay consistent with the consumers.

```diff
diff --git a/zkp_ecdsa_b200/csrc/zk_curves.cuh b/zkp_ecdsa_b200/csrc/zk_curves.cuh
--- a/zkp_ecdsa_b200/csrc/zk_curves.cuh
+++ b/zkp_ecdsa_b200/csrc/zk_curves.cuh
@@ -136,6 +136,38 @@
   F::mul(r.y, G, H);
   if (kNeedT) F::mul(r.t, E, H);
   F::mul(r.z, Fv, G);
+}
+template <class F = Tomp>
+ZK_HD void tom2_from_pre(TomPt& r, const TomPre& q) {
+  uint32_t E[9], H[9];
+#pragma unroll
+  for (int i = 0; i < 9; i++) E[i] = FpTom::p(i);
+  add_n<9>(E, E, q.y);
+  sub_n<9>(E, E, q.x);
+  F::add(H, q.y, q.x);
+  F::mul(r.t, E, H);
+  F::add(r.x, E, E);
+  F::add(r.y, H, H);
+  F::set_one(r.z);
+  F::add(r.z, r.z, r.z);
+  F::add(r.z, r.z, r.z);
+}
+struct TomEfgh {
+  uint32_t e[9], f[9], g[9], h[9];
+};
+template <class F = Tomp>
+ZK_HD void tom2_madd_end(TomEfgh& r, const TomPt& p, const TomPre& q) {
+  uint32_t A[9], B[9], C[9], D[9];
+  F::sub(A, p.y, p.x);
+  F::mul(A, A, q.x);
+  F::add(B, p.y, p.x);
+  F::mul(B, B, q.y);
+  F::mul(C, p.t, q.k);
+  F::add(D, p.z, p.z);
+  F::sub(r.e, B, A);
+  F::sub(r.f, D, C);
+  F::add(r.g, D, C);
+  F::add(r.h, B, A);
 }
 
 ZK_HD void tom_set_identity(TomPt& p) {
diff --git a/zkp_ecdsa_b200/csrc/zk_ops.cuh b/zkp_ecdsa_b200/csrc/zk_ops.cuh
--- a/zkp_ecdsa_b200/csrc/zk_ops.cuh
+++ b/zkp_ecdsa_b200/csrc/zk_ops.cuh
@@ -39,10 +39,12 @@
   P256_AFF_WORDS = 16,
 #if defined(ZKA_PG_WAR256)
   TOM_PROJ_WORDS = 24,
+  TOM_E2_WORDS = 24,
   TOM_AFF_WORDS = 16,
   TOM_PRE_WORDS = 16,
 #else
   TOM_PROJ_WORDS = 28,
+  TOM_E2_WORDS = 36,
   TOM_AFF_WORDS = 18,
   TOM_PRE_WORDS = 32,
 #endif
@@ -86,6 +88,33 @@
 #endif
 #pragma unroll
   for (int i = 0; i < 9; i++) { x[i] = w[i]; y[i] = w[9 + i]; z[i] = w[18 + i]; }
+}
+ZK_HD void tom_st_efgh(uint32_t* m, const TomEfgh& p) {
+  uint32_t w[36];
+#pragma unroll
+  for (int i = 0; i < 9; i++) { w[i] = p.e[i]; w[9 + i] = p.f[i]; w[18 + i] = p.g[i]; w[27 + i] = p.h[i]; }
+#if defined(__CUDA_ARCH__)
+  uint4* v = reinterpret_cast<uint4*>(m);
+#pragma unroll
+  for (int i = 0; i < 9; i++) v[i] = make_uint4(w[4 * i], w[4 * i + 1], w[4 * i + 2], w[4 * i + 3]);
+#else
+  for (int i = 0; i < 36; i++) m[i] = w[i];
+#endif
+}
+ZK_HD void tom_ld_efgh(uint32_t* e, uint32_t* f, uint32_t* g, uint32_t* h, const uint32_t* m) {
+  uint32_t w[36];
+#if defined(__CUDA_ARCH__)
+  const uint4* v = reinterpret_cast<const uint4*>(m);
+#pragma unroll
+  for (int i = 0; i < 9; i++) {
+    const uint4 u = v[i];
+    w[4 * i] = u.x; w[4 * i + 1] = u.y; w[4 * i + 2] = u.z; w[4 * i + 3] = u.w;
+  }
+#else
+  for (int i = 0; i < 36; i++) w[i] = m[i];
+#endif
+#pragma unroll
+  for (int i = 0; i < 9; i++) { e[i] = w[i]; f[i] = w[9 + i]; g[i] = w[18 + i]; h[i] = w[27 + i]; }
 }
 
 ZK_HD void tom2_pre_neg(TomPre& q, bool neg) {
@@ -427,6 +456,7 @@
   int chunk;
   int e2;
   int aff_mod, aff_lim;
+  int stride;
   ZK_HD static void canon2p(uint32_t* r) {
     uint32_t t[9], p2[9];
 #pragma unroll
@@ -443,61 +473,54 @@
     if (n > chunk) n = chunk;
     if (n <= 0) return;
     uint32_t pre[NORM_CHUNK_MAX][9];
-    uint32_t acc[9], z[9], v[9], den[9];
+    uint32_t acc[9], z[9], h[9], den[9];
     F::set_one(acc);
     for (int k = 0; k < n; k++) {
-      const uint32_t* src = proj + (size_t)(lo + k) * TOM_PROJ_WORDS;
-      uint32_t xx[9];
-      tom_ld_xyz(xx, v, z, src);
-      if (e2) F::mul(den, z, v); else copy_n<9>(den, z);
+      const uint32_t* src = proj + (size_t)(lo + k) * stride;
+      uint32_t xx[9], yy[9];
+      if (e2) {
+        tom_ld_efgh(xx, yy, z, h, src);
+        F::mul(den, z, h);
+      } else {
+        tom_ld_xyz(xx, yy, den, src);
+      }
       F::mul(acc, acc, den);
       copy_n<9>(pre[k], acc);
     }
-    uint32_t inv[9], isa[9], is2[9], isd[9], one_plain[9];
+    uint32_t inv[9], cxk[9], is2[9], one_plain[9];
     F::inv(inv, acc);
-    tom_const(isa, TOM_INVSQRTA);
+    tom_const(cxk, e2 ? TOM_INVSQRTND : TOM_INVSQRTA);
     tom_const(is2, TOM_INVSQRTND1);
-    tom_const(isd, TOM_INVSQRTND);
     zero_n<9>(one_plain);
     one_plain[0] = 1;
     for (int k = n - 1; k >= 0; k--) {
-      const uint32_t* src = proj + (size_t)(lo + k) * TOM_PROJ_WORDS;
+      const uint32_t* src = proj + (size_t)(lo + k) * stride;
       uint32_t X[9], Y[9], di[9];
-      tom_ld_xyz(X, Y, z, src);
-      if (e2) F::mul(den, z, Y); else copy_n<9>(den, z);
+      if (e2) {
+        tom_ld_efgh(X, Y, z, h, src);
+        F::mul(den, z, h);
+        F::mul(X, X, h);
+        F::mul(Y, Y, z);
+      } else {
+        tom_ld_xyz(X, Y, den, src);
+      }
       if (k > 0) F::mul(di, inv, pre[k - 1]); else copy_n<9>(di, inv);
       F::mul(inv, inv, den);
       if (bytes) {
         uint32_t Dp[9], cx[9], cy[9];
         F::mul(Dp, di, one_plain);
-        if (e2) {
-          F::mul(cx, X, Y);
-          F::mul(cx, cx, isd);
-          F::mul(cx, cx, Dp);
-          F::sqr(cy, z);
-          F::mul(cy, cy, Dp);
-        } else {
-          F::mul(cx, X, isa);
-          F::mul(cx, cx, Dp);
-          F::mul(cy, Y, Dp);
-        }
+        F::mul(cx, X, cxk);
+        F::mul(cx, cx, Dp);
+        F::mul(cy, Y, Dp);
         canon2p(cx);
         canon2p(cy);
         store_point_words<9, 33>(bytes + (size_t)(lo + k) * BSTRIDE, 0x04u, cx, cy);
       }
       if (aff && ((lo + k) % aff_mod) < aff_lim) {
         uint32_t x[9], y[9];
-        if (e2) {
-          uint32_t zi[9], vi[9];
-          F::mul(zi, di, Y);
-          F::mul(vi, di, z);
-          F::mul(x, X, zi);
-          F::mul(x, x, is2);
-          F::mul(y, z, vi);
-        } else {
-          F::mul(x, X, di);
-          F::mul(y, Y, di);
-        }
+        F::mul(x, X, di);
+        if (e2) F::mul(x, x, is2);
+        F::mul(y, Y, di);
         uint32_t* a = aff + (size_t)(lo + k) * TOM_AFF_WORDS;
         st<9>(a, x);
         st<9>(a + 9, y);
@@ -505,6 +528,11 @@
     }
   }
 };
+
+ZK_HD void tom2_ld_entry(TomPre& q, const uint32_t* tab, int j, size_t ne, uint32_t d, bool neg) {
+  tom_ld_pre(q, tab + ((size_t)j * ne + d) * TOM_PRE_WORDS);
+  tom2_pre_neg(q, neg);
+}
 
 struct TomCommitTask {
   const uint32_t* jv;
@@ -513,27 +541,36 @@
   const uint32_t* htab;
   uint32_t* proj;
   int w, nwin;
+  int xyz = 0;
   ZK_HD void operator()(int t) const {
     uint32_t v[8], r[8];
     ld<8>(v, jv + (size_t)t * 8);
     ld<8>(r, jr + (size_t)t * 8);
-    TomPt acc;
-    tom_set_identity(acc);
     const size_t ne = (size_t)fb_entries(w);
     uint32_t cv = 0, cr = 0;
-    for (int j = 0; j < nwin; j++) {
-      TomPre q;
-      bool nv, nr;
-      const uint32_t dv = signed_digit(v, j, w, cv, nv), dr = signed_digit(r, j, w, cr, nr);
-      tom_ld_pre(q, gtab + ((size_t)j * ne + dv) * TOM_PRE_WORDS);
-      tom2_pre_neg(q, nv);
+    bool nv, nr;
+    TomPre q;
+    uint32_t dv = signed_digit(v, 0, w, cv, nv);
+    tom2_ld_entry(q, gtab, 0, ne, dv, nv);
+    TomPt acc;
+    tom2_from_pre(acc, q);
+    for (int j = 0;; j++) {
+      const uint32_t dr = signed_digit(r, j, w, cr, nr);
+      tom2_ld_entry(q, htab, j, ne, dr, nr);
+      if (j == nwin - 1) break;
       tom2_madd<true>(acc, acc, q);
-      tom_ld_pre(q, htab + ((size_t)j * ne + dr) * TOM_PRE_WORDS);
-      tom2_pre_neg(q, nr);
+      dv = signed_digit(v, j + 1, w, cv, nv);
+      tom2_ld_entry(q, gtab, j + 1, ne, dv, nv);
       tom2_madd<true>(acc, acc, q);
     }
-    uint32_t* o = proj + (size_t)t * TOM_PROJ_WORDS;
-    tom_st_xyz(o, acc.x, acc.y, acc.z);
+    if (xyz) {
+      tom2_madd<false>(acc, acc, q);
+      tom_st_xyz(proj + (size_t)t * TOM_PROJ_WORDS, acc.x, acc.y, acc.z);
+    } else {
+      TomEfgh e;
+      tom2_madd_end(e, acc, q);
+      tom_st_efgh(proj + (size_t)t * TOM_E2_WORDS, e);
+    }
   }
 };
 
@@ -546,17 +583,18 @@
     const int item = t / GJOBS_PER_ITEM, g = t % GJOBS_PER_ITEM;
     uint32_t v[8];
     ld<8>(v, jv + ((size_t)item * JOBS_PER_ITEM + item_job_of_gpart(g)) * 8);
-    TomPt acc;
-    tom_set_identity(acc);
     const size_t ne = (size_t)fb_entries(w);
     uint32_t carry = 0;
+    bool neg;
+    TomPre q;
+    const uint32_t d0 = signed_digit(v, 0, w, carry, neg);
+    tom2_ld_entry(q, gtab, 0, ne, d0, neg);
+    TomPt acc;
+    tom2_from_pre<TompCommit>(acc, q);
 #pragma unroll 1
-    for (int j = 0; j < nwin; j++) {
-      TomPre q;
-      bool neg;
+    for (int j = 1; j < nwin; j++) {
       const uint32_t d = signed_digit(v, j, w, carry, neg);
-      tom_ld_pre(q, gtab + ((size_t)j * ne + d) * TOM_PRE_WORDS);
-      tom2_pre_neg(q, neg);
+      tom2_ld_entry(q, gtab, j, ne, d, neg);
       tom2_madd<true, TompCommit>(acc, acc, q);
     }
     uint32_t* o = ext + (size_t)t * TOM_EXT_WORDS;
@@ -578,16 +616,19 @@
     ld<9>(acc.x, s); ld<9>(acc.y, s + 9); ld<9>(acc.t, s + 18); ld<9>(acc.z, s + 27);
     const size_t ne = (size_t)fb_entries(w);
     uint32_t carry = 0;
+    bool neg;
+    TomPre q;
 #pragma unroll 1
-    for (int j = 0; j < nwin; j++) {
-      TomPre q;
-      bool neg;
+    for (int j = 0; j < nwin - 1; j++) {
       const uint32_t d = signed_digit(r, j, w, carry, neg);
-      tom_ld_pre(q, htab + ((size_t)j * ne + d) * TOM_PRE_WORDS);
-      tom2_pre_neg(q, neg);
+      tom2_ld_entry(q, htab, j, ne, d, neg);
       tom2_madd<true, TompCommit>(acc, acc, q);
     }
-    tom_st_xyz(proj + (size_t)t * TOM_PROJ_WORDS, acc.x, acc.y, acc.z);
+    const uint32_t d = signed_digit(r, nwin - 1, w, carry, neg);
+    tom2_ld_entry(q, htab, nwin - 1, ne, d, neg);
+    TomEfgh e;
+    tom2_madd_end<TompCommit>(e, acc, q);
+    tom_st_efgh(proj + (size_t)t * TOM_E2_WORDS, e);
   }
 };
 
diff --git a/zkp_ecdsa_b200/csrc/zk_ops_war.cuh b/zkp_ecdsa_b200/csrc/zk_ops_war.cuh
--- a/zkp_ecdsa_b200/csrc/zk_ops_war.cuh
+++ b/zkp_ecdsa_b200/csrc/zk_ops_war.cuh
@@ -22,6 +22,7 @@
   int chunk;
   int e2;
   int aff_mod, aff_lim;
+  int stride;
   ZK_HD void operator()(int t) const {
     using F = Warp;
     const int lo = t * chunk;
@@ -33,7 +34,7 @@
     F::set_one(one);
     copy_n<8>(acc, one);
     for (int k = 0; k < n; k++) {
-      ld<8>(z, proj + (size_t)(lo + k) * TOM_PROJ_WORDS + 16);
+      ld<8>(z, proj + (size_t)(lo + k) * stride + 16);
       if (is_zero_n<8>(z)) copy_n<8>(z, one);
       F::mul(acc, acc, z);
       copy_n<8>(pre[k], acc);
@@ -41,7 +42,7 @@
     uint32_t inv[8];
     F::inv(inv, acc);
     for (int k = n - 1; k >= 0; k--) {
-      const uint32_t* src = proj + (size_t)(lo + k) * TOM_PROJ_WORDS;
+      const uint32_t* src = proj + (size_t)(lo + k) * stride;
       ld<8>(z, src + 16);
       const bool isinf = is_zero_n<8>(z);
       if (isinf) copy_n<8>(z, one);
@@ -76,14 +77,17 @@
   const uint32_t* htab;
   uint32_t* proj;
   int w, nwin;
+  int xyz = 0;
   ZK_HD void operator()(int t) const {
     uint32_t v[8], r[8];
     ld<8>(v, jv + (size_t)t * 8);
     ld<8>(r, jr + (size_t)t * 8);
+    WarJac aj;
+    war_set_identity_jac(aj);
+    war_accum_fixed_jac(aj, gtab, v, w);
+    war_accum_fixed_jac(aj, htab, r, w);
     WarPt acc;
-    war_set_identity(acc);
-    war_accum_fixed(acc, gtab, v, w);
-    war_accum_fixed(acc, htab, r, w);
+    war_jac_to_hom(acc, aj);
     war_st_proj(proj + (size_t)t * TOM_PROJ_WORDS, acc);
   }
 };
@@ -96,9 +100,11 @@
     const int item = t / GJOBS_PER_ITEM, g = t % GJOBS_PER_ITEM;
     uint32_t v[8];
     ld<8>(v, jv + ((size_t)item * JOBS_PER_ITEM + item_job_of_gpart(g)) * 8);
+    WarJac aj;
+    war_set_identity_jac(aj);
+    war_accum_fixed_jac(aj, gtab, v, w);
     WarPt acc;
-    war_set_identity(acc);
-    war_accum_fixed(acc, gtab, v, w);
+    war_jac_to_hom(acc, aj);
     war_st_proj(ext + (size_t)t * TOM_EXT_WORDS, acc);
   }
 };
diff --git a/zkp_ecdsa_b200/csrc/zk_prove.cuh b/zkp_ecdsa_b200/csrc/zk_prove.cuh
--- a/zkp_ecdsa_b200/csrc/zk_prove.cuh
+++ b/zkp_ecdsa_b200/csrc/zk_prove.cuh
@@ -623,7 +623,7 @@
   struct Store {
     const ProveCtx& c;
     int it;
-    ZK_HD void operator()(int d, const TomPt& p) const { tom_st_xyz(c.s2_proj + c.s2_der(it, d) * TOM_PROJ_WORDS, p.x, p.y, p.z); }
+    ZK_HD void operator()(int d, const TomPt& p) const { tom_st_xyz(c.s2_proj + c.s2_der(it, d) * TOM_E2_WORDS, p.x, p.y, p.z); }
   };
   ZK_HD void ldaff(TomPt& p, const uint32_t* aff, size_t idx) const {
     uint32_t x[PGL], y[PGL];
diff --git a/zkp_ecdsa_b200/csrc/zkattest.cu b/zkp_ecdsa_b200/csrc/zkattest.cu
--- a/zkp_ecdsa_b200/csrc/zkattest.cu
+++ b/zkp_ecdsa_b200/csrc/zkattest.cu
@@ -415,10 +415,11 @@
   launch(st, (count + ch - 1) / ch, P256NormTask{proj, aff, bytes, inf, (int)count, ch});
 }
 inline void launch_tom_norm(Stream& st, const uint32_t* proj, uint32_t* aff, uint8_t* bytes, long long count, int e2,
-                            int aff_mod = 1, int aff_lim = 1) {
+                            int aff_mod = 1, int aff_lim = 1, int stride = 0) {
   if (count <= 0) return;
   const int ch = norm_chunk_for(count);
-  launch(st, (count + ch - 1) / ch, TomNormTask{proj, aff, bytes, (int)count, ch, e2, aff_mod, aff_lim});
+  if (stride == 0) stride = e2 ? TOM_E2_WORDS : TOM_PROJ_WORDS;
+  launch(st, (count + ch - 1) / ch, TomNormTask{proj, aff, bytes, (int)count, ch, e2, aff_mod, aff_lim, stride});
 }
 
 void build_p256_tab(zka_ctx* ctx, const uint32_t* base_aff_dev, FixedTable& out, int w) {
@@ -670,14 +671,14 @@
     launch(st, nj, TomCommitHTask{c.s2_jr, c.th_tab, gext, c.s2_proj, c.tom_w, c.tom_nwin});
   }
   if (gk)
-    launch(st, ng, TomCommitTask{c.s2_jv + g0 * 8, c.s2_jr + g0 * 8, c.tg_tab, c.th_tab, c.s2_proj + g0 * TOM_PROJ_WORDS, c.tom_w,
+    launch(st, ng, TomCommitTask{c.s2_jv + g0 * 8, c.s2_jr + g0 * 8, c.tg_tab, c.th_tab, c.s2_proj + g0 * TOM_E2_WORDS, c.tom_w,
                                  c.tom_nwin});
   if (items) {
     launch_tom_norm(st, c.s2_proj, c.s2_aff, c.s2_bytes, nj, 1, JOBS_PER_ITEM, 2);
     launch(st, M, DerivedTask{c});
-    launch_tom_norm(st, c.s2_proj + nj * TOM_PROJ_WORDS, nullptr, c.s2_bytes + nj * BSTRIDE, nd, 0);
-  }
-  if (gk) launch_tom_norm(st, c.s2_proj + g0 * TOM_PROJ_WORDS, nullptr, c.s2_bytes + g0 * BSTRIDE, ng, 1);
+    launch_tom_norm(st, c.s2_proj + nj * TOM_E2_WORDS, nullptr, c.s2_bytes + nj * BSTRIDE, nd, 0, 1, 1, TOM_E2_WORDS);
+  }
+  if (gk) launch_tom_norm(st, c.s2_proj + g0 * TOM_E2_WORDS, nullptr, c.s2_bytes + g0 * BSTRIDE, ng, 1);
   if (items) {
     launch(st, M * HASHES_PER_ITEM, ItemHashTask{c});
     launch(st, M * 7, ItemEmitTask{c});
@@ -1020,7 +1021,7 @@
     const uint8_t* dr = stage_in(st, in.next(), r, (size_t)count * 32);
     uint32_t* jv = w.take<uint32_t>((size_t)count * 8);
     uint32_t* jr = w.take<uint32_t>((size_t)count * 8);
-    uint32_t* proj = w.take<uint32_t>((size_t)count * TOM_PROJ_WORDS);
+    uint32_t* proj = w.take<uint32_t>((size_t)count * TOM_E2_WORDS);
     uint32_t* aff = w.take<uint32_t>((size_t)count * TOM_AFF_WORDS);
     uint8_t* bytes = w.take<uint8_t>((size_t)count * BSTRIDE);
     const Output<uint8_t> o(out, WP);
@@ -1121,7 +1122,7 @@
     Cursor in(ctx->in[0]), w(ctx->w);
     uint32_t* jv = w.take<uint32_t>(8);
     uint32_t* jr = w.take<uint32_t>(8);
-    uint32_t* proj = w.take<uint32_t>(TOM_PROJ_WORDS);
+    uint32_t* proj = w.take<uint32_t>(TOM_E2_WORDS);
     uint32_t* aff = w.take<uint32_t>(TOM_AFF_WORDS);
     uint8_t* bytes = w.take<uint8_t>(BSTRIDE);
     uint8_t* d_rnd = in.take<uint8_t>(32);
@@ -1281,7 +1282,7 @@
         c.pa_A_inf = w.take<uint8_t>(nA);
         c.s1_jv = w.take<uint32_t>(n1 * 8);
         c.s1_jr = w.take<uint32_t>(n1 * 8);
-        c.s1_proj = w.take<uint32_t>(n1 * TOM_PROJ_WORDS);
+        c.s1_proj = w.take<uint32_t>(n1 * TOM_E2_WORDS);
         c.s1_aff = w.take<uint32_t>(n1 * TOM_AFF_WORDS);
         c.s1_bytes = w.take<uint8_t>(n1 * BSTRIDE);
         c.chal = w.take<uint32_t>((size_t)Bc * 3);
@@ -1369,7 +1370,7 @@
         const size_t n2 = c.s2_count();
         c.s2_jv = w.take<uint32_t>(n2 * 8);
         c.s2_jr = w.take<uint32_t>(n2 * 8);
-        c.s2_proj = w.take<uint32_t>(n2 * TOM_PROJ_WORDS);
+        c.s2_proj = w.take<uint32_t>(n2 * TOM_E2_WORDS);
         c.s2_aff = w.take<uint32_t>(n2 * TOM_AFF_WORDS);
         c.s2_bytes = w.take<uint8_t>(n2 * BSTRIDE);
         c.secrets = w.take<uint32_t>((size_t)M * SECRETS_PER_ITEM * 8);
@@ -1546,7 +1547,7 @@
       const size_t ng = (size_t)Bc * 4 * n;
       c.s2_jv = w.take<uint32_t>(ng * 8);
       c.s2_jr = w.take<uint32_t>(ng * 8);
-      c.s2_proj = w.take<uint32_t>(ng * TOM_PROJ_WORDS);
+      c.s2_proj = w.take<uint32_t>(ng * TOM_E2_WORDS);
       c.s2_bytes = w.take<uint8_t>(ng * BSTRIDE);
       c.gk_part = w.take_if<uint32_t>(gk_blocks(n) > 1, (size_t)Bc * n * gk_blocks(n) * 8);
       c.proof_stride = proof_stride;
@@ -1586,7 +1587,7 @@
       const size_t nj = (size_t)Bc * J;
       uint32_t* jv = w.take<uint32_t>(nj * 8);
       uint32_t* jr = w.take<uint32_t>(nj * 8);
-      uint32_t* proj = w.take<uint32_t>(nj * TOM_PROJ_WORDS);
+      uint32_t* proj = w.take<uint32_t>(nj * TOM_E2_WORDS);
       uint8_t* bytes = w.take<uint8_t>(nj * BSTRIDE);
       uint8_t* d_com = co.rows(ob.next(), b0, Bc);
       uint8_t* d_prf = po.rows(ob.next(), b0, Bc);
@@ -1651,12 +1652,12 @@
       c.rep_off = w.take<uint32_t>(Bc);
       c.s1_jv = w.take<uint32_t>(n1 * 8);
       c.s1_jr = w.take<uint32_t>(n1 * 8);
-      c.s1_proj = w.take<uint32_t>(n1 * TOM_PROJ_WORDS);
+      c.s1_proj = w.take<uint32_t>(n1 * TOM_E2_WORDS);
       c.s1_aff = w.take<uint32_t>(n1 * TOM_AFF_WORDS);
       c.s1_bytes = w.take<uint8_t>(n1 * BSTRIDE);
       c.s2_jv = w.take<uint32_t>(n2 * 8);
       c.s2_jr = w.take<uint32_t>(n2 * 8);
-      c.s2_proj = w.take<uint32_t>(n2 * TOM_PROJ_WORDS);
+      c.s2_proj = w.take<uint32_t>(n2 * TOM_E2_WORDS);
       c.s2_aff = w.take<uint32_t>(n2 * TOM_AFF_WORDS);
       c.s2_bytes = w.take<uint8_t>(n2 * BSTRIDE);
       c.secrets = w.take<uint32_t>((size_t)Bc * SECRETS_PER_ITEM * 8);
@@ -1872,7 +1873,7 @@
       c.sp_T_inf = w.take<uint8_t>(ns);
       c.ta_jv = w.take<uint32_t>(ns * 2 * 8);
       c.ta_jr = w.take<uint32_t>(ns * 2 * 8);
-      c.ta_proj = w.take<uint32_t>(ns * 2 * TOM_PROJ_WORDS);
+      c.ta_proj = w.take<uint32_t>(ns * 2 * TOM_E2_WORDS);
       c.ta_aff = w.take<uint32_t>(ns * 2 * TOM_AFF_WORDS);
       c.td_proj = w.take<uint32_t>(ns * DERS_PER_ITEM * TOM_PROJ_WORDS);
       c.td_aff = w.take<uint32_t>(ns * DERS_PER_ITEM * TOM_AFF_WORDS);
@@ -1939,7 +1940,7 @@
       launch(st, Bc, VReduceTask{c});
       launch(st, (long long)Bc * ET, VParseEntriesTask{c.proofs, proof_stride, c.ent_off, c.ent_pre, ET});
       if (mode == 0) launch(st, (long long)Bc * ngk, VParseEntriesTask{c.proofs, proof_stride, gk_offs, c.gk_pre, ngk});
-      launch(st, (long long)Bc * 2, TomCommitTask{c.fx_jv, c.fx_jr, c.tg_tab, c.th_tab, c.fx_proj, c.tom_w, c.tom_nwin});
+      launch(st, (long long)Bc * 2, TomCommitTask{c.fx_jv, c.fx_jr, c.tg_tab, c.th_tab, c.fx_proj, c.tom_w, c.tom_nwin, 1});
       uint32_t* ctl = nullptr;
       if (ctx->agg && mode == 0) {
         Cursor A(ln.agg);
@@ -1978,7 +1979,7 @@
         agg_msm(sb, Cursor(ln.agg_nist), nsrc, np, ctl, &nA, &nB);
         launch(st, fgroups, AggFixPartTask{ctl, c.fx_jv, c.fx_jr, fpart, Bc});
         launch(st, 1, AggFixSumTask{ctl, fpart, fjv, fjr, fgroups});
-        launch(st, 1, TomCommitTask{fjv, fjr, c.tg_tab, c.th_tab, fproj, c.tom_w, c.tom_nwin});
+        launch(st, 1, TomCommitTask{fjv, fjr, c.tg_tab, c.th_tab, fproj, c.tom_w, c.tom_nwin, 1});
         launch(sb, ngroups, AggNistFixPartTask{ctl, c.nfix, npart, Bc});
         int nleft = ngroups;
         const uint32_t* nsum = npart;
@@ -2114,7 +2115,7 @@
       dev_memset(st, c.fx_jr, 0, (size_t)Bc * 2 * 8 * 4);
       verify_gk(st, c, gk_offs);
       launch(st, (long long)Bc * ngk, VParseEntriesTask{c.proofs, row_stride, gk_offs, c.gk_pre, ngk});
-      launch(st, (long long)Bc * 2, TomCommitTask{c.fx_jv, c.fx_jr, c.tg_tab, c.th_tab, c.fx_proj, c.tom_w, c.tom_nwin});
+      launch(st, (long long)Bc * 2, TomCommitTask{c.fx_jv, c.fx_jr, c.tg_tab, c.th_tab, c.fx_proj, c.tom_w, c.tom_nwin, 1});
       launch(st, (long long)Bc * MSM_NWIN, MsmTomWindowTask{c.gk_scalar, c.gk_pre, nullptr, ngk, 0, 0, ngk, V_SEG, 1, c.win_g});
       launch(st, Bc, MsmTomCombineTask{c.win_g, c.fx_proj, c.id_flags, 2, 0, 0});
       launch(st, Bc, VGkOnlyFinalTask{c});
@@ -2159,7 +2160,7 @@
       launch(st, Bc, VSubProofTask{kind, rows, stride, d_tape, tape_stride, (const uint8_t*)ctx->tg_bytes.p, ent_scalar, ent_off,
                                    fx_jv, fx_jr, d_st, d_ok});
       launch(st, (long long)Bc * SUB_ENT_MAX, VParseEntriesTask{rows, stride, ent_off, ent_pre, SUB_ENT_MAX});
-      launch(st, (long long)Bc * 2, TomCommitTask{fx_jv, fx_jr, ctx->tg.tab, P->th.tab, fx_proj, ctx->tom_w, ctx->tom_nwin});
+      launch(st, (long long)Bc * 2, TomCommitTask{fx_jv, fx_jr, ctx->tg.tab, P->th.tab, fx_proj, ctx->tom_w, ctx->tom_nwin, 1});
       launch(st, (long long)Bc * MSM_NWIN, MsmTomWindowTask{ent_scalar, ent_pre, nullptr, SUB_ENT_MAX, 0, 0, ne, V_SEG, 1, win});
       launch(st, Bc, MsmTomCombineTask{win, fx_proj, flags, 2, 1, 1});
       launch(st, Bc, VSubFinalTask{d_st, flags, d_ok});
```

Result: faster. 113,700, median of 6 (+4.5%).
